# liangfu/dspnet

Hardware: AMD Instinct MI355X
Metric: training images/sec at 512x512 multitask (higher is better)
Workload: dtype f32; 1 GPU; resnet-50 multitask (det+depth+seg) 512x512, 8 det classes, 19 seg classes, N=6132 anchors, forward+backward+SGD; batch_per_gpu=32, global_batch=32, parallelism=dp1, f16x2_fallback_calls=0

## Files before the change

dspnet_amd/csrc/conv.hip:

```cpp
#include "dspn_common.h"
#include "bn_final_job.h"
#include "dspn_store.h"
#include "dspn_pieces.h"
#include "conv_geom.h"
#include <cstdlib>
#include "../../include/dspn_nn.h"

using dspn::st_t;
using dspn::kHalf;
using dspn::u32x4_t;

namespace {

using dspn::conv::f32x16;
using dspn::conv::bf16x8;
using dspn::pieces::bf16x4;
typedef __attribute__((address_space(3))) bf16x4 lds_bf16x4;

constexpr int kLdsRowH = kHalf ? 72 : 40;
__device__ __forceinline__ bf16x4 to_bf16x4(const float4 v) {
  bf16x4 r = {(__bf16)v.x, (__bf16)v.y, (__bf16)v.z, (__bf16)v.w};
  return r;
}

// ... 1563 lines not shown
    if (g.bn_sums) return DSPN_NT_(true, 3, false, 6);
    return g.stats ? DSPN_NT_(true, 3, false, 5) : DSPN_NT_(true, 3, false, 4);
  }
#endif
  if (g.bn_sums) return DSPN_NT_UB_(false, 2);
  if (g.in_scale) return g.stats ? DSPN_NT_UB_(true, 1) : DSPN_NT_UB_(true, 0);
  return g.stats ? DSPN_NT_UB_(false, 1) : DSPN_NT_UB_(false, 0);
#undef DSPN_NT_UB_
#undef DSPN_NT_
}

#ifdef DSPN_ABLATE
int g_debug_bits = 0;
#else
constexpr int g_debug_bits = 0;
#endif
static const int kNtBm[5] = {128, 128, 64, 256, 128}, kNtBn[5] = {128, 64, 64, 32, 256};
int nt_config(long long M, int Cout) {
  auto tiles = [&](int bm, int bn) { return ((M + bm - 1) / bm) * ((Cout + bn - 1) / bn); };
  int cfg;
  static const long long min_tiles = [] { const char *e = getenv("DSPN_NT_MINTILES"); return e ? atoll(e) : 256ll; }();
  if (Cout <= 32) cfg = tiles(256, 32) >= min_tiles ? 3 : 2;
  else cfg = (Cout > 64 && tiles(128, 128) >= min_tiles) ? 0 : 2;
  if (cfg == 0 && (Cout + 63) / 64 * 64 < (Cout + 127) / 128 * 128) cfg = 1;
  static const int cfg64 = [] { const char *e = getenv("DSPN_NT_CFG64"); return e ? atoi(e) : -1; }();
  if (cfg64 >= 0 && Cout > 32 && Cout <= 64 && tiles(kNtBm[cfg64], kNtBn[cfg64]) >= min_tiles) cfg = cfg64;
  if ((g_debug_bits >> 8) & 7) cfg = ((g_debug_bits >> 8) & 7) - 1;
  return cfg;
}
int dispatch_nt_impl(const st_t *in, const st_t *w, const float *bias, st_t *out, const ConvGeom &g_in,
                     hipStream_t s, SplitWs ws, const st_t *residual, bool *wide_used);
int dispatch_nt(const st_t *in, const st_t *w, const float *bias, st_t *out, const ConvGeom &g_in,
                hipStream_t s, SplitWs ws, const st_t *residual = nullptr) {
  bool wide = false;
  const int rc = dispatch_nt_impl(in, w, bias, out, g_in, s, ws, residual, &wide);
#ifndef DSPN_HALF
  if (!rc && g_in.bn_dy_absmax && !g_in.bn_sums && !wide) {
    if (!(g_in.dense && g_in.obs == (long long)g_in.Hg * g_in.Wg * g_in.ldc && g_in.ldc % 4 == 0))
      return dspn::fail(DSPN_ERR_ARG_, "conv2d_forward: the output magnitude block needs a dense output with ldc %% 4 == 0");
    return dspn_absmax_f32(out, (long long)g_in.N * g_in.Hg * g_in.Wg, g_in.ldc, nullptr, nullptr, 0,
                           reinterpret_cast<float *>(g_in.bn_dy_absmax), s);
  }
#endif
  return rc;
}
int dispatch_nt_impl(const st_t *in, const st_t *w, const float *bias, st_t *out, const ConvGeom &g_in,
                     hipStream_t s, SplitWs ws, const st_t *residual, bool *wide_used) {
  ConvGeom g = g_in;
  g.dbg = g_debug_bits;
  constexpr uintptr_t amask = 4 * sizeof(st_t) - 1;
  if (g.ldc % 4 == 0 && g.obs % 4 == 0 && (reinterpret_cast<uintptr_t>(out) & amask) == 0 &&
      (!residual || (reinterpret_cast<uintptr_t>(residual) & amask) == 0))
    g.flags |= 16;
  {
    const long long ib = (long long)sizeof(st_t) * g.N * g.Hin * g.Win * g.Cin,
                    wb = (long long)sizeof(st_t) * g.Cout * g.WTAPS * g.Cin;
    if (ib >= (1ll << 31) || wb >= (1ll << 31))
      return dspn::fail(DSPN_ERR_ARG_, "conv: tensors of 2 GiB or more are not supported by the buffer-addressed kernel");
    g.in_bytes = (unsigned)ib; g.w_bytes = (unsigned)wb;
  }
  const long long M = (long long)g.N * g.Hg * g.Wg;
  if (M <= 0) return 0;
  const bool pre = !kHalf && g.bf16 >= 2 && ((g.Cin / kEPC) & 7) == 0;
  if (pre) {
    if (!g.w_planes)
      return dspn::fail(DSPN_ERR_ARG_, "conv: the split math modes with a multiple of 32 input channels (%d) need the weight operand as piece planes (dspn_conv2d_weight_planes_f32)", g.Cin);
    w = static_cast<const st_t *>(g.w_planes);
    g.w_bytes = (unsigned)((g.bf16 == 3 ? 4ll : 6ll) * g.Cout * g.WTAPS * g.Cin);
  }
  auto tiles = [&](int bm, int bn) { return ((M + bm - 1) / bm) * ((g.Cout + bn - 1) / bn); };
  const int cfg = nt_config(M, g.Cout);
  const int *bm_ = kNtBm, *bn_ = kNtBn;
  const long long nblk = tiles(bm_[cfg], bn_[cfg]);
  const int nk = (g.TR * g.TS * (g.Cin / kEPC) + 7) >> 3;
  int splits = 1, per = nk;
  if (g.a_planes && !(pre && g.bf16 == 3 && !g.in_scale))
    return dspn::fail(DSPN_ERR_ARG_, "conv: a piece-plane operand needs DSPN_MATH_F32_F16X2, a multiple of 32 channels (%d) and no input affine", g.Cin);
  if (g.stats && (!g.dense || !(g.flags & 16) || g.Cout % 4 != 0))
    return dspn::fail(DSPN_ERR_ARG_, "conv2d_forward: output statistics need a dense, 16-byte aligned output with Cout %% 4 == 0");
  if (g.bn_sums && (g.in_scale || g.stats))
    return dspn::fail(DSPN_ERR_ARG_, "conv: BatchNorm-backward sums cannot be combined with an input affine or output statistics");
  if (g.bn_sums && (!(g.flags & 16) || g.Cout % 4 != 0))
    return dspn::fail(DSPN_ERR_ARG_, "conv2d_dgrad: BatchNorm sums need a 16-byte aligned dx with Cin %% 4 == 0");
  if (g.dense && nblk < 192 && nk >= 16 && ws.ptr && !g.stats && !g.bn_sums) {
    splits = (int)std::min<long long>((384 + nblk - 1) / nblk, nk / 8);
    splits = std::max(1, std::min(splits, 32));
    while (splits > 1 && sizeof(float) * (size_t)splits * M * g.Cout > ws.bytes) --splits;
    per = (nk + splits - 1) / splits;
    splits = (nk + per - 1) / per;
  }
  static const char *eight_env = getenv("DSPN_NT_8WAVE");
  const int eight_mode = eight_env ? atoi(eight_env) : -1;
  const bool one_tap = g.TR * g.TS == 1;
  const bool eight = eight_mode == 0 ? false : eight_mode == 1 ? true : (kHalf || g.bf16 >= 2) ? true
                     : ((!g.stats && !g.bn_sums) || (eight_mode == 2 && one_tap && g.bn_sums) || (eight_mode == 3 && one_tap));
  {
    bool wide_ok = splits == 1 && (cfg == 0 || (cfg == 2 && g.Cout > 32 && g.Cout <= 64)) && (g.flags & 16) && g.Cout % 4 == 0 &&
                   g.TR * g.TS > 0;
    if (kHalf) wide_ok = wide_ok && !g.in_scale && g.Cin % 64 == 0 && dspn::wide_tiles_mode() >= 2;
    else wide_ok = wide_ok && pre && g.bf16 == 3;
    if (wide_ok) {
      int shape = dspn::conv::wide_tile_choice(M, g.Cout, nk, (g.stats || g.bn_sums) ? 1 : 0);
      if (shape && !kHalf && !g.a_planes) shape = 10 + (shape == 1 ? 3 : shape);
      if (shape) { *wide_used = true; return dspn::conv::launch_wide(shape, in, w, bias, out, g, s, residual); }
    }
  }
  if (cfg == 0 && eight) return launch_nt<4, 2, 1, 2>(in, w, bias, out, g, s, splits, per, ws.ptr, residual);
  switch (cfg) {
    case 0: return launch_nt<2, 2, 2, 2>(in, w, bias, out, g, s, splits, per, ws.ptr, residual);
    case 1: return launch_nt<2, 2, 2, 1>(in, w, bias, out, g, s, splits, per, ws.ptr, residual);
    case 2: return launch_nt<2, 2, 1, 1>(in, w, bias, out, g, s, splits, per, ws.ptr, residual);
    default: return launch_nt<4, 1, 2, 1>(in, w, bias, out, g, s, splits, per, ws.ptr, residual);
  }
}

struct WgradPlan { int bm; int bn; int splits; int pps; };
constexpr int kPlanPK = 64;
static_assert(kPlanPK % kPK == 0, "split sizes must be whole k-steps");
WgradPlan wgrad_plan(long long P, int Cout, int J, long long x_bytes = 0, long long max_splits = 1 << 30) {
  WgradPlan p;
  p.bm = Cout <= 32 ? 32 : (Cout <= 64 ? 64 : 128);
  if (p.bm == 128 && (Cout + 63) / 64 * 64 < (Cout + 127) / 128 * 128) p.bm = 64;
  p.bn = (J <= 64 && p.bm == 128) ? 64 : 128;
  if (const char *e = getenv("DSPN_WG_TILE")) {
    const int t = atoi(e);
    p.bm = t == 0 ? 32 : (t == 1 ? 64 : 128);
    p.bn = t == 2 ? 64 : 128;
  }
  const long long tiles = (long long)((Cout + p.bm - 1) / p.bm) * ((J + p.bn - 1) / p.bn);
  const long long lds = 4ll * std::max(2 * kPK * (p.bm + p.bn), p.bm * (p.bn + 4));
  const long long slots = 256 * std::min<long long>(8, (160ll << 10) / lds);
  long long s_min = 1;
  if (x_bytes > 0) s_min = (x_bytes + (32ll << 20) - 1) / (32ll << 20);
  const long long s_max = std::max<long long>(1, std::min<long long>(std::min<long long>(P / 128, 1024), max_splits));
  s_min = std::min(s_min, s_max);
  const double flop_per_pix = 2.0 * p.bm * p.bn, slot_rate = 120e12 / (double)slots, ovh_pix = 160;
  double best = 1e30;
  long long splits = s_min;
  for (long long sp = s_min; sp <= s_max; ++sp) {
    const long long pps = ((P + sp - 1) / sp + kPlanPK - 1) / kPlanPK * kPlanPK;
    const long long real = (P + pps - 1) / pps;
    const long long rounds = (tiles * real + slots - 1) / slots;
    const double t = (double)rounds * ((double)pps + ovh_pix) * flop_per_pix / slot_rate +
                     (double)real * Cout * J * 8.0 / 4e12;
    if (t < best * 0.999) { best = t; splits = sp; }
    if (tiles * sp > 8 * slots) break;
  }
  if (const char *e = getenv("DSPN_WG_SPLITS")) splits = std::max<long long>(1, std::min<long long>(atoll(e), s_max));
  splits = std::min(splits, s_max);
  long long pps = ((P + splits - 1) / splits + kPlanPK - 1) / kPlanPK * kPlanPK;
  p.splits = (int)((P + pps - 1) / pps);
  p.pps = (int)pps;
  return p;
}

}

extern "C" {

#ifdef DSPN_ABLATE
#ifdef DSPN_HALF
int dspn_debug_set_bf16(int bits) { g_debug_bits = bits; return 0; }
#else
int dspn_debug_set(int bits) { g_debug_bits = bits; return 0; }
int dspn_debug_read_stamps(unsigned *host, int words, int clear) {
  if (hipMemcpyFromSymbol(host, HIP_SYMBOL(g_phase_stamps), sizeof(unsigned) * (size_t)std::min(words, 8192 * 8)) != hipSuccess) return 1;
  if (clear) { static unsigned z[8192 * 8]; (void)hipMemcpyToSymbol(HIP_SYMBOL(g_phase_stamps), z, sizeof(z)); }
  return 0;
}
#endif
#endif

#ifndef DSPN_HALF
size_t dspn_conv2d_split_workspace_bytes(long long out_pixels, int Cout) {
  if (out_pixels <= 0 || Cout <= 0) return 0;
  const long long capped = std::min<long long>(out_pixels * Cout, 192ll * 64 * 64 * 4);
  return sizeof(float) * 32 * (size_t)capped;
}
#endif

struct InAffine { const float *scale, *shift; int relu; };
struct OpScales { const float *a, *b; int a_planes = 0; };

static int conv2d_forward_one(int math, OpScales scales, const st_t *x, InAffine tf, float *stats, float *minmax, const st_t *w, const void *w_planes, const float *bias, const st_t *residual, st_t *y, int N,
                            int H, int W, int Cin, int Cout, int R, int S, int stride, int pad_h, int pad_w,
                            int dil, int Ho, int Wo, long long y_batch_stride, int y_ldc,
                            int relu, int accumulate, void *workspace, size_t workspace_bytes,
                            void *stream) {
  DSPN_REQUIRE(x && (w || w_planes) && y, "conv2d_forward: null pointer");
// ... 108 lines not shown
  hipLaunchKernelGGL(weight_transpose_kernel, dim3(blocks), dim3(256), 0, (hipStream_t)stream, w,
                     wt, static_cast<float *>(nullptr), Cout, taps, Cin, Cout_pad);
  return dspn::check_launch("weight_transpose");
}

int dspn_conv2d_weight_transpose_batch_f32(const void *table, int n, long long total_tiles, void *stream) {
  DSPN_REQUIRE(table && n > 0 && total_tiles > 0 && total_tiles < (1ll << 31), "weight_transpose_batch: bad argument");
  static_assert(sizeof(WtDesc) == 48, "table row layout: 2 pointers, 4 ints, 1 int64, 1 pointer (NULL here)");
  hipLaunchKernelGGL(weight_transpose_batch_kernel, dim3((unsigned)total_tiles), dim3(256), 0, (hipStream_t)stream,
                     static_cast<const WtDesc *>(table), n);
  return dspn::check_launch("weight_transpose_batch");
}
long long dspn_conv2d_weight_transpose_tiles(int Cout, int taps, int Cin, int Cout_pad) {
  if (Cout <= 0 || taps <= 0 || Cin <= 0 || Cout_pad < Cout) return 0;
  return (long long)((Cout_pad + 31) >> 5) * taps * ((Cin + 31) >> 5);
}

int dspn_conv2d_weight_planes_f32(const float *w, void *planes, void *planes_t, int Cout, int taps, int Cin, int cols_t,
                                  int pieces, const float *w_absmax, void *stream) {
  DSPN_REQUIRE(w && (planes || planes_t) && Cout > 0 && taps > 0 && Cin > 0 && Cin % 4 == 0, "weight_planes: bad argument");
  DSPN_REQUIRE(pieces == 3 || (pieces == 2 && w_absmax), "weight_planes: pieces is 3 (bf16) or 2 (fp16, with the weight's magnitude block)");
  DSPN_REQUIRE(!planes || Cin % 32 == 0, "weight_planes: the forward planes need Cin %% 32 == 0, got %d", Cin);
  DSPN_REQUIRE(!planes_t || (cols_t % 32 == 0 && cols_t >= Cout), "weight_planes: cols_t is the padded Cout, a multiple of 32");
  WpDesc e{w, static_cast<__bf16 *>(planes), static_cast<__bf16 *>(planes_t), Cout, taps, Cin, planes_t ? cols_t : 0, 0, w_absmax, pieces, 0};
  const long long tiles = weight_planes_tiles(Cout, taps, Cin, cols_t, planes_t != nullptr);
  DSPN_REQUIRE(tiles < (1ll << 31), "weight_planes: too many tiles");
  hipLaunchKernelGGL(weight_planes_kernel, dim3((unsigned)tiles), dim3(256), 0, (hipStream_t)stream, e);
  return dspn::check_launch("weight_planes");
}

long long dspn_conv2d_weight_planes_tiles(int Cout, int taps, int Cin, int cols_t, int with_transposed) {
  if (Cout <= 0 || taps <= 0 || Cin <= 0) return 0;
  return weight_planes_tiles(Cout, taps, Cin, cols_t, with_transposed != 0);
}

int dspn_absmax_f32(const float *x, long long rows, int C, const float *scale, const float *shift, int relu,
                    float *out_dev, void *stream) {
  DSPN_REQUIRE(x && out_dev && rows > 0 && C > 0 && C % 4 == 0, "absmax: bad argument (C must be a multiple of 4)");
  DSPN_REQUIRE((scale == nullptr) == (shift == nullptr), "absmax: scale and shift go together");
  const long long n4 = rows * (C / 4);
  const int blocks = (int)std::min<long long>((n4 + 255) / 256, 2048);
  hipLaunchKernelGGL(absmax_kernel, dim3(blocks), dim3(256), 0, (hipStream_t)stream, reinterpret_cast<const float4 *>(x), n4,
                     C / 4, reinterpret_cast<const float4 *>(scale), reinterpret_cast<const float4 *>(shift), relu,
                     reinterpret_cast<unsigned *>(out_dev));
  return dspn::check_launch("absmax");
}

int dspn_absmax_batch_f32(const void *table, int n, long long total_chunks, void *stream) {
  DSPN_REQUIRE(table && n > 0 && total_chunks > 0 && total_chunks < (1ll << 31), "absmax_batch: bad argument");
  static_assert(sizeof(AmDesc) == 32, "table row layout: 2 pointers, 2 int64");
  hipLaunchKernelGGL(absmax_batch_kernel, dim3((unsigned)total_chunks), dim3(256), 0, (hipStream_t)stream,
                     static_cast<const AmDesc *>(table), n);
  return dspn::check_launch("absmax_batch");
}

int dspn_conv2d_weight_planes_batch_f32(const void *table, int n, long long total_tiles, void *stream) {
  DSPN_REQUIRE(table && n > 0 && total_tiles > 0 && total_tiles < (1ll << 31), "weight_planes_batch: bad argument");
  static_assert(sizeof(WpDesc) == 64, "table row layout: 3 pointers, 4 ints, 1 int64, 1 pointer, 2 ints");
  hipLaunchKernelGGL(weight_planes_batch_kernel, dim3((unsigned)total_tiles), dim3(256), 0, (hipStream_t)stream,
                     static_cast<const WpDesc *>(table), n);
  return dspn::check_launch("weight_planes_batch");
}
#else
int dspn_conv2d_weight_prepare_bf16(const float *w, st_t *wh, st_t *wt, int Cout, int taps, int Cin,
                                    int Cout_pad, void *stream) {
  DSPN_REQUIRE(w && wt && Cout > 0 && taps > 0 && Cin > 0 && Cout_pad >= Cout && Cout_pad % kEPC == 0,
               "weight_prepare: bad argument");
  const long long total = (long long)Cin * taps * Cout_pad;
  const int blocks = (int)std::min<long long>((total + 255) / 256, 4096);
  hipLaunchKernelGGL(weight_transpose_kernel, dim3(blocks), dim3(256), 0, (hipStream_t)stream, w,
                     wt, wh, Cout, taps, Cin, Cout_pad);
  return dspn::check_launch("weight_prepare");
}

int dspn_conv2d_weight_prepare_batch_bf16(const void *table, int n, long long total_tiles, void *stream) {
  DSPN_REQUIRE(table && n > 0 && total_tiles > 0 && total_tiles < (1ll << 31), "weight_prepare_batch: bad argument");
  static_assert(sizeof(WtDesc) == 48, "table row layout: 2 pointers, 4 ints, 1 int64, 1 pointer");
  hipLaunchKernelGGL(weight_transpose_batch_kernel, dim3((unsigned)total_tiles), dim3(256), 0, (hipStream_t)stream,
                     static_cast<const WtDesc *>(table), n);
  return dspn::check_launch("weight_prepare_batch");
}
#endif

struct BnBwd { const st_t *x; const float *scale, *shift, *mean, *rstd; int relu; float *sums; float *dy_absmax; };

static int dgrad_tiles(int N, int H, int W, int Cin, int stride, int *per_class ) {
  int total = 0;
  for (int ph = 0; ph < (stride == 1 ? 1 : 2); ++ph)
    for (int pw = 0; pw < (stride == 1 ? 1 : 2); ++pw) {
      const long long hg = stride == 1 ? H : (H - ph + 1) / 2, wg = stride == 1 ? W : (W - pw + 1) / 2;
      const long long M = (long long)N * hg * wg;
      const int t = M > 0 ? (int)((M + kNtBm[nt_config(M, Cin)] - 1) / kNtBm[nt_config(M, Cin)]) : 0;
      if (per_class) per_class[ph * 2 + pw] = t;
      total += t;
    }
  return total;
}

static int conv2d_dgrad_one(int math, OpScales scales, const st_t *dy, const st_t *wt, const void *wt_planes, st_t *dx, int N, int H, int W,
                          int Cin, int ldy, int R, int S, int stride, int pad_h, int pad_w, int dil, int Ho,
                          int Wo, int dx_ldc, int accumulate, BnBwd bn, void *workspace, size_t workspace_bytes,
                          void *stream) {
  DSPN_REQUIRE(dy && (wt || wt_planes) && dx, "conv2d_dgrad: null pointer");
  DSPN_REQUIRE(ldy % kEPC == 0, "conv2d_dgrad: dy channel stride must be a multiple of %d", kEPC);
  DSPN_REQUIRE(stride == 1 || (stride == 2 && dil == 1), "conv2d_dgrad: stride 1, or stride 2 with dilation 1");
  DSPN_REQUIRE(N > 0 && H > 0 && W > 0 && Cin > 0 && R > 0 && S > 0, "conv2d_dgrad: bad geometry");
  ConvGeom g;
  memset(&g, 0, sizeof(g));
  g.N = N; g.Hin = Ho; g.Win = Wo; g.Cin = ldy; g.Cout = Cin;
  g.WTAPS = R * S; g.WS = S;
  g.ldc = dx_ldc > 0 ? dx_ldc : Cin;
  g.obs = (long long)H * W * g.ldc;
  g.OW = W;
  g.flags = accumulate ? 4 : 0;
  g.bf16 = kHalf ? 1 : math;
  g.w_planes = wt_planes;
  g.a_absmax = scales.a; g.b_absmax = scales.b;
  g.bn_x = bn.x; g.bn_scale = bn.scale; g.bn_shift = bn.shift; g.bn_mean = bn.mean; g.bn_rstd = bn.rstd;
  g.bn_relu = bn.relu; g.bn_sums = bn.sums; g.bn_tile_base = 0;
  g.bn_dy_absmax = (bn.sums && !kHalf && math == DSPN_MATH_F32_F16X2) ? reinterpret_cast<unsigned *>(bn.dy_absmax) : nullptr;
  g.a_planes = scales.a_planes;
  int class_tiles[4] = {0, 0, 0, 0};
  if (bn.sums) dgrad_tiles(N, H, W, Cin, stride, class_tiles);
  hipStream_t s = (hipStream_t)stream;
  const SplitWs sws{static_cast<float *>(workspace), workspace ? workspace_bytes : 0};
  if (stride == 1) {
    g.Hg = H; g.Wg = W; g.ish = 1; g.isw = 1; g.ioh = pad_h; g.iow = pad_w; g.idh = -dil; g.idw = -dil;
    g.TR = R; g.TS = S; g.wr0 = 0; g.wrs = 1; g.ws0 = 0; g.wss = 1;
    g.osh = 1; g.osw = 1; g.dense = 1;
    return dispatch_nt(dy, wt, nullptr, dx, g, s, sws);
  }
  for (int ph = 0; ph < 2; ++ph)
    for (int pw = 0; pw < 2; ++pw) {
      ConvGeom c = g;
      c.Hg = (H - ph + 1) / 2; c.Wg = (W - pw + 1) / 2;
      for (int q = 0; q < ph * 2 + pw; ++q) c.bn_tile_base += class_tiles[q];
      if (c.Hg <= 0 || c.Wg <= 0) continue;
      const int r0 = (ph + pad_h) & 1, s0 = (pw + pad_w) & 1;
      c.TR = r0 < R ? (R - r0 + 1) / 2 : 0;
      c.TS = s0 < S ? (S - s0 + 1) / 2 : 0;
      if (c.TR == 0 || c.TS == 0) {
        c.TR = 0; c.TS = 1;
        if (accumulate && !bn.sums) continue;
      }
      c.ish = 1; c.isw = 1; c.ioh = (ph + pad_h - r0) / 2; c.iow = (pw + pad_w - s0) / 2;
      c.idh = -1; c.idw = -1;
      c.wr0 = r0; c.wrs = 2; c.ws0 = s0; c.wss = 2;
      c.osh = 2; c.osw = 2; c.ooh = ph; c.oow = pw; c.dense = 0;
      const int rc = dispatch_nt(dy, wt, nullptr, dx, c, s, sws);
      if (rc) return rc;
    }
  return 0;
}

static int dgrad_bn_tiles(int N, int H, int W, int Cin, int stride) {
  if (N <= 0 || H <= 0 || W <= 0 || Cin <= 0 || Cin % 4 != 0 || (stride != 1 && stride != 2)) return 0;
  return dgrad_tiles(N, H, W, Cin, stride, nullptr);
}
#ifndef DSPN_HALF
int dspn_conv2d_dgrad_bn_tiles(int N, int H, int W, int Cin, int stride) { return dgrad_bn_tiles(N, H, W, Cin, stride); }
#endif

int DSPN_FN(dspn_conv2d_dgrad_bn)(const st_t *dy, const st_t *wt, const void *wt_planes, st_t *dx, int N, int H, int W,
                             int Cin, int ldy, int R, int S, int stride, int pad_h, int pad_w, int dil, int Ho,
                             int Wo, int dx_ldc, int accumulate,
                             const st_t *bn_x, const float *bn_scale, const float *bn_shift, const float *bn_mean,
                             const float *bn_rstd, int bn_relu, float *bn_sums, size_t bn_sums_bytes, float *bn_dy_absmax,
                             int math, const float *dy_absmax, const float *w_absmax, void *workspace, size_t workspace_bytes,
                             void *stream) {
  DSPN_REQUIRE(N > 0 && Ho > 0 && Wo > 0 && ldy > 0, "conv2d_dgrad: bad geometry");
  const int math_vouch = math & DSPN_MATH_UNSCALED_OK, dy_planes = (math & DSPN_MATH_DY_PLANES) ? 1 : 0;
  math &= ~(DSPN_MATH_UNSCALED_OK | DSPN_MATH_DY_PLANES);
  DSPN_REQUIRE(!dy_planes || (!dspn::kHalf && math == DSPN_MATH_F32_F16X2 && ldy % 32 == 0 && dy_absmax),
               "conv2d_dgrad: DSPN_MATH_DY_PLANES needs DSPN_MATH_F32_F16X2, ldy %% 32 == 0 and the block the planes were cut by (dy_absmax)");
  DSPN_REQUIRE(math >= DSPN_MATH_FP32 && math <= DSPN_MATH_F32_F16X2, "conv2d_dgrad: math is one of DSPN_MATH_*");
  DSPN_REQUIRE(dspn::kHalf || math != DSPN_MATH_F32_F16X2 || math_vouch || (dy_absmax && w_absmax),
               "conv2d_dgrad: DSPN_MATH_F32_F16X2 needs the magnitude block of both operands (dspn_absmax_f32); a caller who knows that every |operand| < 65504 passes math | DSPN_MATH_UNSCALED_OK");
  const int ldc = dx_ldc > 0 ? dx_ldc : Cin;
  const int nb = batch_chunk(N, (long long)sizeof(st_t) * Ho * Wo * ldy);
  if (bn_sums) {
    DSPN_REQUIRE(bn_x && bn_mean && bn_rstd && (!bn_relu || (bn_scale && bn_shift)), "conv2d_dgrad: BatchNorm operands missing");
    DSPN_REQUIRE(ldc == Cin && nb == N, "conv2d_dgrad: BatchNorm sums need a dense dx and dy below 2 GiB");
    const int tiles = dgrad_bn_tiles(N, H, W, Cin, stride);
    DSPN_REQUIRE(tiles > 0 && bn_sums_bytes >= sizeof(float) * 2 * (size_t)tiles * Cin,
                 "conv2d_dgrad: bn_sums needs dspn_conv2d_dgrad_bn_tiles() x 2 x Cin floats");
  }
  for (int n0 = 0; n0 < N; n0 += nb) {
    const int n = std::min(nb, N - n0);
    const int rc = conv2d_dgrad_one(math, OpScales{dy_absmax, w_absmax, dy_planes}, dy + (long long)n0 * Ho * Wo * ldy, wt, wt_planes, dx + (long long)n0 * H * W * ldc, n, H,
                                    W, Cin, ldy, R, S, stride, pad_h, pad_w, dil, Ho, Wo, dx_ldc, accumulate,
                                    BnBwd{bn_x, bn_scale, bn_shift, bn_mean, bn_rstd, bn_relu, bn_sums, bn_dy_absmax}, workspace,
                                    workspace_bytes, stream);
    if (rc) return rc;
  }
  return 0;
}

#ifndef DSPN_HALF
int dspn_conv2d_dgrad_f32(const float *dy, const float *wt, float *dx, int N, int H, int W,
                          int Cin, int ldy, int R, int S, int stride, int pad_h, int pad_w, int dil, int Ho,
                          int Wo, int dx_ldc, int accumulate, void *workspace, size_t workspace_bytes,
                          void *stream) {
  return dspn_conv2d_dgrad_bn_f32(dy, wt, nullptr, dx, N, H, W, Cin, ldy, R, S, stride, pad_h, pad_w, dil, Ho, Wo, dx_ldc,
                                  accumulate, nullptr, nullptr, nullptr, nullptr, nullptr, 0, nullptr, 0, nullptr, DSPN_MATH_FP32,
                                  nullptr, nullptr, workspace, workspace_bytes, stream);
}

size_t dspn_conv2d_input_sum_grad_workspace_bytes(int Ho, int Wo, int ldy, int R, int S) {
  return sizeof(float) * ((size_t)Ho * Wo * ldy + (size_t)R * S * 32 * ldy);
}
#endif

int DSPN_FN(dspn_conv2d_input_sum_grad)(const st_t *dy, const float *w, float *out, int N, int H, int W,
                                   int Cin, int Cout, int ldy, int R, int S, int stride, int pad_h, int pad_w, int dil,
                                   int Ho, int Wo, void *workspace, size_t workspace_bytes, void *stream) {
  DSPN_REQUIRE(dy && w && out && workspace, "conv2d_input_sum_grad: null pointer");
  DSPN_REQUIRE(ldy % 4 == 0 && Cin >= 1 && Cin <= 8, "conv2d_input_sum_grad: Cin <= 8, ldy % 4 == 0");
  if (workspace_bytes < sizeof(float) * ((size_t)Ho * Wo * ldy + (size_t)R * S * 32 * ldy))
    return dspn::fail(DSPN_ERR_WORKSPACE_, "conv2d_input_sum_grad: workspace too small");
  hipStream_t s = (hipStream_t)stream;
  float *p2 = static_cast<float *>(workspace);
  float *partial = p2 + (size_t)Ho * Wo * ldy;
  const long long per4 = (long long)Ho * Wo * ldy / 4;
  hipLaunchKernelGGL(batch_sum_kernel, dim3((int)std::min<long long>((per4 + 255) / 256, 8192)), dim3(256), 0, s,
                     dspn::CA4Ptr(dy), reinterpret_cast<float4 *>(p2), N, per4);
  SumGradGeom g{H, W, Ho, Wo, ldy, R, S, stride, stride, pad_h, pad_w, dil, dil, 32};
  hipLaunchKernelGGL(tap_sum_kernel, dim3(R * S, 32), dim3(256), 0, s, p2, partial, g);
  hipLaunchKernelGGL(sum_grad_final_kernel, dim3(1), dim3(1024), 0, s, partial, w, out, R * S, 32, ldy, Cout, Cin);
  return dspn::check_launch("conv2d_input_sum_grad");
}

#ifndef DSPN_HALF
size_t dspn_conv2d_wgrad_workspace_bytes(int N, int Ho, int Wo, int Cin, int Cout, int R, int S) {
  const long long P = (long long)N * Ho * Wo;
  const int J = R * S * Cin;
  if (P <= 0 || J <= 0 || Cout <= 0) return 0;
  size_t m = (size_t)wgrad_plan(P, Cout, J).splits;
  for (int stride = 1; stride <= 2; ++stride)
    m = std::max(m, (size_t)wgrad_plan(P, Cout, J, 4ll * P * Cin * stride * stride).splits);
  return sizeof(float) * m * Cout * J;
}
#endif

static int conv2d_wgrad_one(int math, OpScales scales, const st_t *x, InAffine tf, const st_t *dy, float *dw, int N, int H, int W, int Cin,
                          int Cout, int ldy, int R, int S, int stride, int pad_h, int pad_w, int dil, int Ho,
                          int Wo, int accumulate, void *workspace, size_t workspace_bytes,
                          void *stream) {
  DSPN_REQUIRE(x && dy && workspace, "conv2d_wgrad: null pointer");
  DSPN_REQUIRE(Cin % kEPC == 0 && ldy % kEPC == 0, "conv2d_wgrad: channel strides must be multiples of %d", kEPC);
  WgradGeom g;
  g.N = N; g.Hin = H; g.Win = W; g.Cin = Cin; g.Ho = Ho; g.Wo = Wo; g.Cout = Cout; g.ldy = ldy;
  g.sh = stride; g.sw = stride; g.ph = pad_h; g.pw = pad_w; g.dh = dil; g.dw = dil; g.R = R; g.S = S;
  g.in_scale = tf.scale; g.in_shift = tf.shift; g.in_relu = tf.relu;
  g.bf16 = kHalf ? 1 : math;
  g.dy_absmax = scales.a; g.x_absmax = scales.b;
  g.dy_planes = scales.a_planes & 1; g.x_planes = (scales.a_planes >> 1) & 1;
  {
    const long long xb = (long long)sizeof(st_t) * N * H * W * Cin, yb = (long long)sizeof(st_t) * N * Ho * Wo * ldy;
    if (xb >= (1ll << 31) || yb >= (1ll << 31))
      return dspn::fail(DSPN_ERR_ARG_, "conv2d_wgrad: tensors of 2 GiB or more are not supported");
    g.x_bytes = (unsigned)xb; g.dy_bytes = (unsigned)yb;
  }
  const long long P = (long long)N * Ho * Wo;
  const int J = R * S * Cin;
  const long long ws_splits = (long long)(workspace_bytes / (sizeof(float) * (size_t)Cout * J));
  if (ws_splits < 1)
    return dspn::fail(DSPN_ERR_WORKSPACE_, "conv2d_wgrad: workspace %zu < %zu (one slab)", workspace_bytes, sizeof(float) * (size_t)Cout * J);
  const WgradPlan plan = wgrad_plan(P, Cout, J, R * S > 1 ? 4ll * P * Cin * std::min(stride, 2) * std::min(stride, 2) : 0, ws_splits);
  const int BM = plan.bm, BN = plan.bn;
  const int kt = (Cout + BM - 1) / BM, jt = (J + BN - 1) / BN;
  const long long splits = plan.splits;
  g.pix_per_split = plan.pps;
  const size_t need = sizeof(float) * (size_t)splits * Cout * J;
  if (workspace_bytes < need)
    return dspn::fail(DSPN_ERR_WORKSPACE_, "conv2d_wgrad: workspace %zu < %zu", workspace_bytes, need);
  hipStream_t s = (hipStream_t)stream;
  float *slab = static_cast<float *>(workspace);
  g.job = dspn::BnFinalJob{};
  g.job_rows = dspn::bn_job_take(s, &g.job) ? (g.job.blocks + kt * jt - 1) / (kt * jt) : 0;
// ... 149 lines not shown
```

dspnet_amd/csrc/conv_geom.h:

```cpp
#pragma once
#include <hip/hip_runtime.h>

namespace dspn {
namespace conv {

typedef float f32x16 __attribute__((ext_vector_type(16)));
typedef __bf16 bf16x8 __attribute__((ext_vector_type(8)));

template <typename st_t>
struct ConvGeomT {
  int N, Hin, Win, Cin;
  int Hg, Wg;
  int ish, isw, ioh, iow, idh, idw;
  int TR, TS;
  int WTAPS, WS, wr0, wrs, ws0, wss;
  int Cout;
  long long obs;
  int OW, osh, osw, ooh, oow, ldc;
  int flags;
  int dense;
  int dbg;
  int bf16;
  unsigned in_bytes, w_bytes;
  const float *in_scale, *in_shift;
  float *stats;
  float *minmax;
  const st_t *bn_x;
  const float *bn_scale, *bn_shift, *bn_mean, *bn_rstd;
  float *bn_sums;
  int bn_relu, bn_tile_base;
  unsigned *bn_dy_absmax;
  const float *a_absmax, *b_absmax;
  int a_planes;
  const void *w_planes;
};

__device__ __forceinline__ int xcd_remap(int bid, int nblk) {
  const int q = nblk >> 3, r = nblk & 7, x = bid & 7;
  const int start = x < r ? x * (q + 1) : r * (q + 1) + (x - r) * q;
  return start + (bid >> 3);
}


int wide_tile_choice(long long M, int Cout, int nk, int fused_epilogue);
int launch_wide(int shape, const float *in, const float *w_planes, const float *bias, float *out, const ConvGeomT<float> &g,
                hipStream_t s, const float *residual);
int launch_wide(int shape, const __bf16 *in, const __bf16 *w, const float *bias, __bf16 *out, const ConvGeomT<__bf16> &g,
                hipStream_t s, const __bf16 *residual);

int launch_stem(const float *x, const float *w, float *y, int N, int H, int W, int Cin, int Cout, int Ho, int Wo,
                const float *x_absmax, const float *w_absmax, float *stats, float *minmax, hipStream_t s);

}
}
```

dspnet_amd/csrc/conv_wide.h:

```cpp

#ifdef DSPN_STAMPS
__device__ unsigned long long g_wide_stamps[1024 * 16];
struct WideStamps {
  unsigned long long last, sum[16];
  __device__ __forceinline__ void begin() { for (int i = 0; i < 16; ++i) sum[i] = 0; last = __builtin_readcyclecounter(); }
  __device__ __forceinline__ void mark(int i) { const unsigned long long t = __builtin_readcyclecounter(); sum[i] += t - last; last = t; }
  __device__ __forceinline__ void flush() {
    if (threadIdx.x == 0 && blockIdx.x < 1024) for (int i = 0; i < 16; ++i) g_wide_stamps[blockIdx.x * 16 + i] = sum[i];
  }
};
#define DSPN_STAMP_DECL WideStamps stamps_; stamps_.begin()
#define DSPN_STAMP(i) stamps_.mark(i)
#define DSPN_STAMP_FLUSH stamps_.flush()
#define DSPN_STAMP_ARG , stamps_
#define DSPN_STAMP_PARAM , WideStamps &stamps_
#else
#define DSPN_STAMP_DECL
#define DSPN_STAMP(i)
#define DSPN_STAMP_FLUSH
#define DSPN_STAMP_ARG
#define DSPN_STAMP_PARAM
#endif

inline bool xt_enabled() { return dspn::tile_spanning() != 0; }
// ... 150 lines not shown
            red2[((h * RPP + er0) * BN + c4 * 4 + e) * 2 + 1] = vmx[h][e];
          }
        }
      }
    }
    asm volatile("s_waitcnt lgkmcnt(0)" ::: "memory");
    __builtin_amdgcn_s_barrier();
    for (int hc = tid; hc < HALVES * BN; hc += NTHR) {
      const int h = hc / BN, col = hc - h * BN;
      const int lim = min(M - (m0 + h * SR), SR);
      if (n0 + col >= g.Cout || lim <= 0) continue;
      const float *rh = red + (size_t)h * RPP * BN * 2, *rh2 = red2 + (size_t)h * RPP * BN * 2;
      const float mref = rh[col * 2];
      float n = 0.f, sd = 0.f, sq = 0.f;
#pragma unroll 4
      for (int er = 0; er < RPP; ++er) {
        const int ne_i = lim > er ? (lim - er + RPP - 1) / RPP : 0;
        const float ne = (float)ne_i;
        const float d = ne_i > 0 ? rh[(er * BN + col) * 2] - mref : 0.f;
        const float m2e = ne_i > 0 ? rh[(er * BN + col) * 2 + 1] : 0.f;
        n += ne; sd += ne * d; sq += m2e + ne * d * d;
      }
      const float dm = sd / n;
      const long long mt_ = m0 / SR + h;
      g.stats[(mt_ * 2 + 0) * g.Cout + n0 + col] = mref + dm;
      g.stats[(mt_ * 2 + 1) * g.Cout + n0 + col] = fmaxf(sq - n * dm * dm, 0.f);
      if (mmx) {
        float mn = kInf, mx = -kInf;
        for (int er = 0; er < RPP && er < lim; ++er) { mn = fminf(mn, rh2[(er * BN + col) * 2]); mx = fmaxf(mx, rh2[(er * BN + col) * 2 + 1]); }
        g.minmax[(mt_ * 2 + 0) * g.Cout + n0 + col] = mn;
        g.minmax[(mt_ * 2 + 1) * g.Cout + n0 + col] = mx;
      }
    }
  }
  if constexpr (EPI == 2) {
    __builtin_amdgcn_s_barrier();
    float *red = reinterpret_cast<float *>(wsm);
    if (cvalid) {
#pragma unroll
      for (int h = 0; h < HALVES; ++h)
#pragma unroll
        for (int e = 0; e < 4; ++e) {
          red[((h * RPP + er0) * BN + c4 * 4 + e) * 2] = gs[h][e];
          red[((h * RPP + er0) * BN + c4 * 4 + e) * 2 + 1] = gss[h][e];
        }
    }
    asm volatile("s_waitcnt lgkmcnt(0)" ::: "memory");
    __builtin_amdgcn_s_barrier();
    for (int hc = tid; hc < HALVES * BN; hc += NTHR) {
      const int h = hc / BN, col = hc - h * BN;
      if (n0 + col >= g.Cout || m0 + h * SR >= M) continue;
      const float *rh = red + (size_t)h * RPP * BN * 2;
      float a = 0.f, b = 0.f;
      for (int er = 0; er < RPP; ++er) { a += rh[(er * BN + col) * 2]; b += rh[(er * BN + col) * 2 + 1]; }
      const long long mt_ = g.bn_tile_base + m0 / SR + h;
      g.bn_sums[(mt_ * 2 + 0) * g.Cout + n0 + col] = a;
      g.bn_sums[(mt_ * 2 + 1) * g.Cout + n0 + col] = b;
    }
    gmx_all = fmaxf(gmx_all, gmx);
  }
  if constexpr (EPI == 0) gmx_all = fmaxf(gmx_all, gmx);
  asm volatile("s_waitcnt lgkmcnt(0)" ::: "memory");
  __builtin_amdgcn_s_barrier();
  DSPN_STAMP(6);
}

#ifndef DSPN_HALF
template <int WAVES_M, int WAVES_N, int EPI, int RB = 16, int SR = 128, bool CLOSE = false>
__device__ __forceinline__ void direct_epilogue(const ConvGeom &g, char *exch, f32x16 (&acc)[2][2], const float inv_a, const float inv_b, const int m0,
                                                const int n0, const int M, const int tid, const int wave,
                                                const float *__restrict__ bias, float *__restrict__ out,
                                                const float *__restrict__ residual, float &gmx_all) {
  constexpr int TM = 2, TN = 2, BN = WAVES_N * 64, NTHR = WAVES_M * WAVES_N * 64, PARTS = WAVES_M * 2;
  constexpr int WRT = SR / 64, TILES = WAVES_M / WRT, PPT = WRT * 2;
  static_assert(SR == 64 || SR == 128, "statistics tiles of 64 or 128 rows");
  static_assert(WAVES_M % WRT == 0, "whole statistics tiles per output tile");
  const int lane = tid & 63, half = lane >> 5, lc = lane & 31;
  const int wr = wave / WAVES_N, wm = wr * 64, wn = (wave % WAVES_N) * 64;
  const bool has_bias = g.flags & 1, relu = g.flags & 2, accum = g.flags & 4, has_res = g.flags & 8;
  const float *addsrc = has_res ? residual : (accum ? out : nullptr);
  const unsigned obytes = (unsigned)M * (unsigned)g.ldc * 4u;
  const __amdgpu_buffer_rsrc_t rs_o = __builtin_amdgcn_make_buffer_rsrc(out, 0, obytes, 0x00020000);
  const __amdgpu_buffer_rsrc_t rs_a = __builtin_amdgcn_make_buffer_rsrc(const_cast<float *>(addsrc ? addsrc : out), 0, addsrc ? obytes : 0u, 0x00020000);
  const __amdgpu_buffer_rsrc_t rs_x = __builtin_amdgcn_make_buffer_rsrc(const_cast<float *>(EPI == 2 ? g.bn_x : out), 0, EPI == 2 ? obytes : 0u, 0x00020000);
  constexpr unsigned kOOB = 0x80000000u;
  constexpr float kInf = __builtin_huge_valf();
  int col[TN];
  unsigned cbyte[TN];
  bool cv[TN];
  float bv[TN], bsc[TN], bsh[TN], bmu[TN], brs[TN];
#pragma unroll
  for (int j = 0; j < TN; ++j) {
    col[j] = n0 + wn + j * 32 + lc;
    cv[j] = col[j] < g.Cout;
    cbyte[j] = cv[j] ? (unsigned)col[j] * 4u : kOOB;
    bv[j] = (has_bias && cv[j]) ? bias[col[j]] : 0.f;
    bsc[j] = bsh[j] = bmu[j] = brs[j] = 0.f;
    if (EPI == 2 && cv[j]) {
      bmu[j] = g.bn_mean[col[j]]; brs[j] = g.bn_rstd[col[j]];
      if (g.bn_relu) { bsc[j] = g.bn_scale[col[j]]; bsh[j] = g.bn_shift[col[j]]; }
    }
  }
  const int row0 = m0 + wm + 4 * half;
  const unsigned pitch = (unsigned)g.ldc * 4u;
  float sK[TN], s1[TN], s2[TN], vmn[TN], vmx[TN], gs[TN], gss[TN];
  int scnt = 0;
  float gmx = 0.f;
#pragma unroll
  for (int j = 0; j < TN; ++j) { sK[j] = 0.f; s1[j] = 0.f; s2[j] = 0.f; vmn[j] = kInf; vmx[j] = -kInf; gs[j] = 0.f; gss[j] = 0.f; }
  const bool both = has_res && accum;
  constexpr int NB = TM * 16 / RB;
  const bool need_rows = addsrc != nullptr || EPI == 2;
  if constexpr (EPI == 2) {
    float rq[2][RB][TN], xq[2][RB][TN], oq[2][RB][TN];
    auto request = [&](const int bb, const int s_) __attribute__((always_inline)) {
      const int i = bb / (16 / RB), r0 = (bb % (16 / RB)) * RB;
#pragma unroll
      for (int rr = 0; rr < RB; ++rr) {
        const int r = r0 + rr;
        const unsigned rb = (unsigned)(row0 + 32 * i + (r & 3) + 8 * (r >> 2)) * pitch;
#pragma unroll
        for (int j = 0; j < TN; ++j) {
          const unsigned off = rb + cbyte[j];
          rq[s_][rr][j] = addsrc ? __builtin_bit_cast(float, __builtin_amdgcn_raw_buffer_load_b32(rs_a, (int)off, 0, 0)) : 0.f;
          xq[s_][rr][j] = __builtin_bit_cast(float, __builtin_amdgcn_raw_buffer_load_b32(rs_x, (int)off, 0, 0));
          oq[s_][rr][j] = both ? __builtin_bit_cast(float, __builtin_amdgcn_raw_buffer_load_b32(rs_o, (int)off, 0, 0)) : 0.f;
        }
      }
    };
    request(0, 0);
#pragma unroll
    for (int bb = 0; bb < NB; ++bb) {
      const int i = bb / (16 / RB), r0 = (bb % (16 / RB)) * RB, s_ = bb & 1;
      if (bb + 1 < NB) request(bb + 1, s_ ^ 1);
#pragma unroll
      for (int rr = 0; rr < RB; ++rr) {
        const int r = r0 + rr;
        const unsigned rb = (unsigned)(row0 + 32 * i + (r & 3) + 8 * (r >> 2)) * pitch;
#pragma unroll
        for (int j = 0; j < TN; ++j) {
          float v = acc[i][j][r] * inv_a * inv_b + bv[j];
          v += rq[s_][rr][j];
          if (both) v += oq[s_][rr][j];
          if (relu) v = v > 0.f ? v : 0.f;
          __builtin_amdgcn_raw_buffer_store_b32(__builtin_bit_cast(unsigned, v), rs_o, (int)(rb + cbyte[j]), 0, 0);
          const float xv = xq[s_][rr][j];
          const float gd = (!g.bn_relu || fmaf(xv, bsc[j], bsh[j]) > 0.f) ? v : 0.f;
          gs[j] += gd;
          gss[j] += gd * ((xv - bmu[j]) * brs[j]);
          gmx = fmaxf(gmx, fabsf(v));
        }
      }
    }
#pragma unroll
    for (int j = 0; j < TN; ++j) { gs[j] = cv[j] ? gs[j] : 0.f; gss[j] = cv[j] ? gss[j] : 0.f; }
  } else {
    typedef float f32x2 __attribute__((ext_vector_type(2)));
    f32x2 s1p[TN], s2p[TN];
#pragma unroll
    for (int j = 0; j < TN; ++j) { s1p[j] = f32x2{0.f, 0.f}; s2p[j] = f32x2{0.f, 0.f}; }
    f32x2 rq[2][RB / 2][TN], oq[2][RB / 2][TN];
    auto request = [&](const int bb, const int s_) __attribute__((always_inline)) {
      const int i = bb / (16 / RB), r0 = (bb % (16 / RB)) * RB;
#pragma unroll
      for (int rr = 0; rr < RB; rr += 2) {
        const int r = r0 + rr;
        const unsigned rb = (unsigned)(row0 + 32 * i + (r & 3) + 8 * (r >> 2)) * pitch;
#pragma unroll
        for (int j = 0; j < TN; ++j) {
          const unsigned off = rb + cbyte[j];
          rq[s_][rr / 2][j] = f32x2{0.f, 0.f}; oq[s_][rr / 2][j] = f32x2{0.f, 0.f};
          if (addsrc) rq[s_][rr / 2][j] = f32x2{__builtin_bit_cast(float, __builtin_amdgcn_raw_buffer_load_b32(rs_a, (int)off, 0, 0)),
                                               __builtin_bit_cast(float, __builtin_amdgcn_raw_buffer_load_b32(rs_a, (int)(off + pitch), 0, 0))};
          if (both) oq[s_][rr / 2][j] = f32x2{__builtin_bit_cast(float, __builtin_amdgcn_raw_buffer_load_b32(rs_o, (int)off, 0, 0)),
                                             __builtin_bit_cast(float, __builtin_amdgcn_raw_buffer_load_b32(rs_o, (int)(off + pitch), 0, 0))};
        }
      }
    };
    if (need_rows) request(0, 0);
#pragma unroll
    for (int bb = 0; bb < NB; ++bb) {
      const int i = bb / (16 / RB), r0 = (bb % (16 / RB)) * RB, s_ = bb & 1;
      if (need_rows && bb + 1 < NB) request(bb + 1, s_ ^ 1);
#pragma unroll
      for (int rr = 0; rr < RB; rr += 2) {
        const int r = r0 + rr;
        const unsigned rb = (unsigned)(row0 + 32 * i + (r & 3) + 8 * (r >> 2)) * pitch;
#pragma unroll
        for (int j = 0; j < TN; ++j) {
          f32x2 t = f32x2{acc[i][j][r], acc[i][j][r + 1]} * inv_a * inv_b + bv[j];
          if (need_rows) t += rq[s_][rr / 2][j];
          else t += f32x2{0.f, 0.f};
          float v0 = t[0], v1 = t[1];
          if (both) { v0 += oq[s_][rr / 2][j][0]; v1 += oq[s_][rr / 2][j][1]; }
          if (relu) { v0 = v0 > 0.f ? v0 : 0.f; v1 = v1 > 0.f ? v1 : 0.f; }
          __builtin_amdgcn_raw_buffer_store_b32(__builtin_bit_cast(unsigned, v0), rs_o, (int)(rb + cbyte[j]), 0, 0);
          __builtin_amdgcn_raw_buffer_store_b32(__builtin_bit_cast(unsigned, v1), rs_o, (int)(rb + pitch + cbyte[j]), 0, 0);
          const f32x2 v = f32x2{v0, v1};
          if constexpr (EPI == 0) {
            if (g.bn_dy_absmax) gmx = fmaxf(fmaxf(gmx, fabsf(v0)), fabsf(v1));
          }
          if constexpr (EPI == 1) {
            if (bb == 0 && rr == 0) sK[j] = v0;
            const f32x2 d = v - sK[j];
            s1p[j] += d; s2p[j] += d * d;
            vmn[j] = fminf(fminf(vmn[j], v0), v1); vmx[j] = fmaxf(fmaxf(vmx[j], v0), v1);
          }
        }
      }
    }
    scnt = 32;
#pragma unroll
    for (int j = 0; j < TN; ++j) { s1[j] = s1p[j].x + s1p[j].y; s2[j] = s2p[j].x + s2p[j].y; }
  }
  if constexpr (EPI == 0) gmx_all = fmaxf(gmx_all, gmx);
  if constexpr (EPI == 2) gmx_all = fmaxf(gmx_all, gmx);
  if constexpr (EPI != 0) {
    float *red = reinterpret_cast<float *>(exch);
    float *red2 = red + PARTS * BN * 4;
    const bool mmx = EPI == 1 && g.minmax != nullptr;
    const int p = wr * 2 + half;
#pragma unroll
    for (int j = 0; j < TN; ++j) {
      float *q = red + (p * BN + wn + j * 32 + lc) * 4;
      if constexpr (EPI == 1) {
        const float inv_n = scnt > 0 ? 1.f / (float)scnt : 0.f;
        q[0] = (float)scnt; q[1] = sK[j] + s1[j] * inv_n; q[2] = s2[j] - s1[j] * s1[j] * inv_n;
        if (mmx) { float *q2 = red2 + (p * BN + wn + j * 32 + lc) * 2; q2[0] = vmn[j]; q2[1] = vmx[j]; }
      } else {
        q[0] = gs[j]; q[1] = gss[j];
      }
    }
    asm volatile("s_waitcnt lgkmcnt(0)" ::: "memory");
    __builtin_amdgcn_s_barrier();
    for (int hc = tid; hc < TILES * BN; hc += NTHR) {
      const int h = hc / BN, c = hc - h * BN;
      if (n0 + c >= g.Cout || m0 + h * SR >= M) continue;
      const long long mt_ = m0 / SR + h;
      if constexpr (EPI == 1) {
        float n = 0.f, mean = 0.f, m2 = 0.f, mn = kInf, mx = -kInf;
#pragma unroll
        for (int pq = 0; pq < PPT; ++pq) {
          const int pp = h * PPT + pq;
          const float *q = red + (pp * BN + c) * 4;
          const float nb = q[0];
          if (nb > 0.f) {
            const float d = q[1] - mean, nn = n + nb;
            mean += d * (nb / nn);
            m2 += q[2] + d * d * (n * nb / nn);
            n = nn;
            if (mmx) { mn = fminf(mn, red2[(pp * BN + c) * 2]); mx = fmaxf(mx, red2[(pp * BN + c) * 2 + 1]); }
          }
        }
        g.stats[(mt_ * 2 + 0) * g.Cout + n0 + c] = mean;
        g.stats[(mt_ * 2 + 1) * g.Cout + n0 + c] = fmaxf(m2, 0.f);
        if (mmx) {
          g.minmax[(mt_ * 2 + 0) * g.Cout + n0 + c] = mn;
          g.minmax[(mt_ * 2 + 1) * g.Cout + n0 + c] = mx;
        }
      } else {
        float a = 0.f, b = 0.f;
#pragma unroll
        for (int pq = 0; pq < PPT; ++pq) { a += red[((h * PPT + pq) * BN + c) * 4]; b += red[((h * PPT + pq) * BN + c) * 4 + 1]; }
        const long long t_ = g.bn_tile_base + mt_;
        g.bn_sums[(t_ * 2 + 0) * g.Cout + n0 + c] = a;
        g.bn_sums[(t_ * 2 + 1) * g.Cout + n0 + c] = b;
      }
    }
    if constexpr (CLOSE) {
      asm volatile("s_waitcnt lgkmcnt(0)" ::: "memory");
      __builtin_amdgcn_s_barrier();
    }
  }
}
#endif

template <int NWV>
__device__ __forceinline__ void wide_publish_absmax(const ConvGeom &g, char *wsm, float gmx_all, const int tid) {
  const int lane = tid & 63, wave = tid >> 6;
    if (g.bn_dy_absmax) {
#pragma unroll
      for (int o = 32; o >= 1; o >>= 1) gmx_all = fmaxf(gmx_all, __shfl_xor(gmx_all, o, 64));
      float *sm = reinterpret_cast<float *>(wsm);
      if (lane == 0) sm[wave] = gmx_all;
      asm volatile("s_waitcnt lgkmcnt(0)" ::: "memory");
      __builtin_amdgcn_s_barrier();
      if (tid == 0) {
        float m = sm[0];
        for (int q = 1; q < NWV; ++q) m = fmaxf(m, sm[q]);
        if (m > 0.f) atomicMax(g.bn_dy_absmax + (blockIdx.x & 63u), __float_as_uint(m));
      }
    }
}

template <int WAVES_M, int WAVES_N, int STAGES, int EPI, int SR = 128, bool XT = false>
__global__ __launch_bounds__(WAVES_M * WAVES_N * 64, 2) void conv_ntw_kernel(
    const st_t *__restrict__ in, const st_t *__restrict__ wgt, const float *__restrict__ bias,
    st_t *__restrict__ out, const ConvGeom g, const int m_tiles, const int n_tiles,
    const st_t *__restrict__ residual) {
  constexpr int TM = 2, TN = 2;
// ... 121 lines not shown
    bf16x8 fa[4][TM], fb[4][TN];
    constexpr int ORD[4] = {kHalf ? 0 : 2, 0, kHalf ? 1 : 3, kHalf ? 2 : 1};
    constexpr int ORDH[4] = {0, 1, 2, 3};
    if (dbg & 4) {
#pragma unroll
      for (int f = 0; f < 4; ++f) {
#pragma unroll
        for (int i = 0; i < TM; ++i) { fa[f][i] = bf16x8{}; asm volatile("" : "+v"(fa[f][i])); }
#pragma unroll
        for (int j = 0; j < TN; ++j) { fb[f][j] = bf16x8{}; asm volatile("" : "+v"(fb[f][j])); }
      }
    } else {
#pragma unroll
      for (int q = 0; q < 4; ++q) {
        const int f = kHalf ? ORDH[q] : ORD[q];
        const int fbq = kHalf ? f : (f ^ 2);
#pragma unroll
        for (int i = 0; i < TM; ++i) fa[f][i] = *reinterpret_cast<const bf16x8 *>(sa + i * 4096 + (foff ^ ((2 * f) << 4)));
#pragma unroll
        for (int j = 0; j < TN; ++j) fb[fbq][j] = *reinterpret_cast<const bf16x8 *>(sb + j * 4096 + (foff ^ ((2 * fbq) << 4)));
      }
    }
    __builtin_amdgcn_sched_barrier(0);
    constexpr int NMMA = NKK * NPROD * TM * TN;
    static_assert(NI <= NMMA, "at most one request per MFMA");
    constexpr int PA[3] = {1, 0, 0}, PB[3] = {0, 1, 0};
#pragma unroll
    for (int m = 0; m < NMMA; ++m) {
      const int kk = m / (NPROD * TM * TN), t3 = (m / (TM * TN)) % NPROD, i = (m / TN) % TM, j = m % TN;
      const int ia = kHalf ? kk : 2 * PA[t3] + kk, ib = kHalf ? kk : 2 * PB[t3] + kk;
      if (dbg & 2) { asm volatile("" :: "v"(fa[ia][i]), "v"(fb[ib][j])); }
      else if constexpr (kHalf)
        acc[i][j] = __builtin_amdgcn_mfma_f32_32x32x16_bf16(fa[ia][i], fb[ib][j], acc[i][j], 0, 0, 0);
      else
        acc[i][j] = __builtin_amdgcn_mfma_f32_32x32x16_f16(__builtin_bit_cast(f16x8, fa[ia][i]),
                                                           __builtin_bit_cast(f16x8, fb[ib][j]), acc[i][j], 0, 0, 0);
#pragma unroll
      for (int q = 0; q < NI; ++q)
        if (((q + 1) * NMMA) / NI - 1 == m) {
          issue_piece(q);
          __builtin_amdgcn_sched_barrier(0);
        }
    }
  };

  float gmx_all = 0.f;

  if constexpr (XT) {
    constexpr bool EXCH_IN_RING = NWV == 8 || BM == 256;
    int t = blockIdx.x;
    if (t < ntiles) {
      setup_tile(t);
#pragma unroll
      for (int j = 0; j < D; ++j) issue(j, true);
    }
    int slot = 0, islot = D % STAGES;
    bool more = false;
    DSPN_STAMP_DECL;
    for (; t < ntiles; t += gridDim.x) {
      const int m0 = ld_m0, n0 = ld_n0;
      const int tn = t + (int)gridDim.x;
      const bool first = t == (int)blockIdx.x;
      zero_acc();
      int last_slot = 0;
      for (int kt = 0; kt < nk; ++kt) {
        if (!first && kt < D) asm volatile("s_waitcnt vmcnt(63)" ::: "memory");
        else asm volatile("s_waitcnt vmcnt(%0)" ::"n"((D - 1) * NI) : "memory");
        __builtin_amdgcn_s_barrier();
        if (kt + D < nk) {
          issue_begin(islot, true);
        } else {
          if (kt + D == nk) { more = tn < ntiles; if (more) setup_tile(tn); }
          issue_begin(islot, more);
        }
        mma_step(slot);
        last_slot = slot;
        slot = slot + 1 == STAGES ? 0 : slot + 1;
        islot = islot + 1 == STAGES ? 0 : islot + 1;
      }
      DSPN_STAMP(2);
      char *exch = wsm + STAGES * STG;
      if constexpr (EXCH_IN_RING) {
        exch = wsm + last_slot * STG;
        if constexpr (EPI != 0) { asm volatile("s_waitcnt lgkmcnt(0)" ::: "memory"); __builtin_amdgcn_s_barrier(); }
      }
      if constexpr (!kHalf) direct_epilogue<WAVES_M, WAVES_N, EPI, (EPI == 2 ? 4 : 8), SR>(g, exch, acc, inv_a, inv_b, m0, n0, M, tid, wave, bias, out, residual, gmx_all);
      DSPN_STAMP(5);
    }
    DSPN_STAMP_FLUSH;
    asm volatile("s_waitcnt vmcnt(0)" ::: "memory");
    if constexpr (EPI != 1) {
      asm volatile("s_waitcnt lgkmcnt(0)" ::: "memory");
      __builtin_amdgcn_s_barrier();
      wide_publish_absmax<NWV>(g, wsm, gmx_all, tid);
    }
    return;
  }

  DSPN_STAMP_DECL;
  for (int t = blockIdx.x; t < ntiles; t += gridDim.x) {
    setup_tile(t);
    const int m0 = ld_m0, n0 = ld_n0;
#pragma unroll
    for (int j = 0; j < D; ++j) issue(j, j < nk);
    zero_acc();
    DSPN_STAMP(1);
    int slot = 0, islot = D % STAGES;
    for (int kt = 0; kt < nk; ++kt) {
      asm volatile("s_waitcnt vmcnt(%0)" ::"n"((D - 1) * NI) : "memory");
      if (!(dbg & 8)) __builtin_amdgcn_s_barrier();
      issue_begin(islot, kt + D < nk);
      mma_step(slot);
      slot = slot + 1 == STAGES ? 0 : slot + 1;
      islot = islot + 1 == STAGES ? 0 : islot + 1;
    }
    asm volatile("s_waitcnt vmcnt(0)" ::: "memory");
    asm volatile("s_waitcnt lgkmcnt(0)" ::: "memory");
    __builtin_amdgcn_s_barrier();
    DSPN_STAMP(2);
    if (dbg & 16) { if (acc[0][0][0] == 1.2345e33f) out[0] = (st_t)acc[TM - 1][TN - 1][5]; continue; }

    {
      constexpr int SLD = BN + 4;
      float *st = reinterpret_cast<float *>(wsm);
  #pragma unroll
      for (int i = 0; i < TM; ++i)
  #pragma unroll
        for (int j = 0; j < TN; ++j)
  #pragma unroll
          for (int r = 0; r < 16; ++r)
            st[(wm + i * 32 + (r & 3) + 8 * (r >> 2) + 4 * (lane >> 5)) * SLD + wn + j * 32 + (lane & 31)] = acc[i][j][r] * inv_a * inv_b;
    }
    DSPN_STAMP(3);
    wide_epilogue<BM, BN, NTHR, EPI, SR>(g, wsm, m0, n0, M, tid, bias, out, residual, gmx_all, NoStage() DSPN_STAMP_ARG);
  }
  DSPN_STAMP_FLUSH;
  if constexpr (EPI != 1) wide_publish_absmax<NWV>(g, wsm, gmx_all, tid);
}

#ifndef DSPN_HALF
typedef float ntv_f32x4_t __attribute__((ext_vector_type(4)));
template <int NEWER>
__device__ __forceinline__ void ntv_wait2(ntv_f32x4_t &a, ntv_f32x4_t &b) {
  asm volatile("s_waitcnt vmcnt(%2)" : "+v"(a), "+v"(b) : "n"(NEWER));
}
template <int NEWER>
__device__ __forceinline__ void ntv_wait4(ntv_f32x4_t &a, ntv_f32x4_t &b, ntv_f32x4_t &c, ntv_f32x4_t &d) {
  asm volatile("s_waitcnt vmcnt(%4)" : "+v"(a), "+v"(b), "+v"(c), "+v"(d) : "n"(NEWER));
}
template <int WAVES_M, int WAVES_N, bool INTF, int EPI, int SR = 128, int XT = 0>
__global__ __launch_bounds__(WAVES_M * WAVES_N * 64, 2) void conv_ntv_kernel(
    const float *__restrict__ in, const float *__restrict__ wgt, const float *__restrict__ bias,
    float *__restrict__ out, const ConvGeom g, const int m_tiles, const int n_tiles,
    const float *__restrict__ residual) {
  constexpr int TM = 2, TN = 2;
  constexpr int BM = WAVES_M * TM * 32, BN = WAVES_N * TN * 32;
  constexpr int NWV = WAVES_M * WAVES_N, NTHR = NWV * 64;
  constexpr int A_U = BM * 4 / NTHR;
  constexpr int B_NI = BN / (8 * NWV);
  static_assert((BM * 4) % NTHR == 0 && BN % (8 * NWV) == 0, "whole units / pieces per thread / wave");
  constexpr int STG = (BM + BN) * 128;
#ifdef DSPN_NTV_SHALLOW
  constexpr bool DEEP = false;
#else
  constexpr bool DEEP = A_U <= 2;
#endif
  constexpr int NSET = DEEP ? 2 : 1;
  constexpr int NA = A_U * 2 + (INTF ? 4 : 0);
  extern __shared__ __attribute__((aligned(1024))) char wsm[];
  const int tid = threadIdx.x, lane = tid & 63;
  const int wave = __builtin_amdgcn_readfirstlane(tid >> 6);
  const int ntiles = m_tiles * n_tiles;
  const int M = g.N * g.Hg * g.Wg;
  const int CB = g.Cin >> 5;
  const int nk = g.TR * g.TS * CB;
  const float sc_a = operand_scale(g.a_absmax), sc_b = operand_scale(g.b_absmax);
  const float inv_a = 1.f / sc_a, inv_b = 1.f / sc_b;
  const __amdgpu_buffer_rsrc_t rsrc_b = __builtin_amdgcn_make_buffer_rsrc(const_cast<float *>(wgt), 0, g.w_bytes, 0x00020000);
  constexpr unsigned kOOB = 0x80000000u;
  const bool in_relu = g.flags & 32;
  auto rsrc_words = [](const float *p, unsigned bytes) {
    const unsigned long long a = reinterpret_cast<unsigned long long>(p);
    return u32x4_t{(unsigned)__builtin_amdgcn_readfirstlane((int)(unsigned)a),
                   (unsigned)__builtin_amdgcn_readfirstlane((int)((unsigned)(a >> 32) & 0xffffu)),
                   (unsigned)__builtin_amdgcn_readfirstlane((int)bytes), 0x00020000u};
  };
  const u32x4_t rw_a = rsrc_words(in, g.in_bytes);
  const u32x4_t rw_sc = rsrc_words(g.in_scale, INTF ? (unsigned)g.Cin * 4u : 0u), rw_sh = rsrc_words(g.in_shift, INTF ? (unsigned)g.Cin * 4u : 0u);
  typedef ntv_f32x4_t f32x4_t;
  auto load16 = [](const u32x4_t rw, const unsigned voff) __attribute__((always_inline)) {
    f32x4_t r;
    asm volatile("buffer_load_dwordx4 %0, %1, %2, 0 offen" : "=v"(r) : "v"(voff), "s"(rw));
    return r;
  };

  const int aq = tid & 3;
  int a_lds[A_U];
#pragma unroll
  for (int j = 0; j < A_U; ++j) {
    const int r = (tid + j * NTHR) >> 2, line = r >> 1;
    a_lds[j] = line * 256 + (((((r & 1) << 3) | aq) ^ (line & 7)) << 4);
  }
  int b_row[B_NI], b_cb[B_NI];
#pragma unroll
  for (int i = 0; i < B_NI; ++i) {
    const int line = 4 * (wave * B_NI + i) + (lane >> 4), sl = (lane & 15) ^ (line & 7);
    b_row[i] = 2 * line + (sl >> 3); b_cb[i] = (sl & 7) * 16;
  }
  int a_ih0[A_U], a_iw0[A_U], a_boff[A_U], b_boff[B_NI];
  int l_tr = 0, l_ts = 0, l_cb = 0;
  int lb_tr = 0, lb_ts = 0, lb_cb = 0;
  f32x4_t ra[NSET][A_U][2];
  f32x4_t tsc[NSET][2], tsh[NSET][2];
  unsigned a_mask[NSET] = {};
  u32x4_t pa[A_U][2];

  const int wm = (wave / WAVES_N) * (TM * 32), wn = (wave % WAVES_N) * (TN * 32);
// ... 274 lines not shown
  auto kern = conv_ntv_kernel<WAVES_M, WAVES_N, INTF, EPI, SR, XT>;
  static dspn::KernelDeviceState st;
  const bool first = !st.slots[0] && !st.slots[1];
  const int dev = dspn::ensure_persistent_grid(reinterpret_cast<const void *>(kern), WAVES_M * WAVES_N * 64, lds, st, "conv_ntv");
  if (dev < 0) return dev;
  const int slots = st.slots[dev], slots_per_cu = st.slots_per_cu[dev], slots_cus = st.cus[dev];
  if (first && getenv("DSPN_DEBUG_PRINT"))
    fprintf(stderr, "[dspn] conv_ntv<%d,%d,intf=%d,epi=%d,xt=%d>: %zu B LDS, occupancy %d/CU x %d CUs -> grid %d\n", WAVES_M, WAVES_N,
            (int)INTF, EPI, (int)XT, lds, slots_per_cu, slots_cus, slots);
  const int reserved = dspn::reserved_cus();
  const int avail = reserved > 0 ? std::max(8, slots_per_cu * std::max(8, slots_cus - reserved) / 8 * 8) : slots;
  const int grid_x = (int)std::min<long long>((long long)mt * nt, avail);
  {
    dspn::ProfScope prof(0, s);
    hipLaunchKernelGGL(kern, dim3(grid_x), dim3(WAVES_M * WAVES_N * 64), lds, s, in, w, bias, out, g, mt, nt, residual);
  }
  return dspn::check_launch("conv_ntv");
}
template <int WAVES_M, int WAVES_N, int SR = 128>
int launch_ntv(const float *in, const float *w, const float *bias, float *out, const ConvGeom &g, hipStream_t s, const float *residual) {
#define DSPN_NTV_(T, X) \
  (g.bn_sums ? launch_ntv_impl<WAVES_M, WAVES_N, T, 2, SR, X>(in, w, bias, out, g, s, residual) \
   : g.stats ? launch_ntv_impl<WAVES_M, WAVES_N, T, 1, SR, X>(in, w, bias, out, g, s, residual) \
             : launch_ntv_impl<WAVES_M, WAVES_N, T, 0, SR, X>(in, w, bias, out, g, s, residual))
  if constexpr (WAVES_M == 2 && WAVES_N == 2 && SR == 128) {
    const int nk = g.TR * g.TS * (g.Cin / 32);
    const long long tiles = (((long long)g.N * g.Hg * g.Wg + 127) / 128) * ((g.Cout + 127) / 128);
    if (dspn::tile_spanning() >= 2 && nk >= 2 && nk <= 8 && nk % 2 == 0 && tiles >= 2048 && xt_output_ok(g))
      return g.in_scale ? DSPN_NTV_(true, 1) : DSPN_NTV_(false, 1);
    static const bool direct_only = [] { const char *e = getenv("DSPN_NTV_DIRECT"); return !e || atoi(e) != 0; }();
    if (direct_only && xt_enabled() && nk >= 2 && xt_output_ok(g))
      return g.in_scale ? DSPN_NTV_(true, 2) : DSPN_NTV_(false, 2);
  }
  if constexpr (WAVES_M == 2 && WAVES_N == 4 && SR == 128) {
    static const bool direct8 = [] { const char *e = getenv("DSPN_NTV_DIRECT8"); return !e || atoi(e) != 0; }();
    const int nk = g.TR * g.TS * (g.Cin / 32);
    if (direct8 && xt_enabled() && nk >= 2 && xt_output_ok(g))
      return g.in_scale ? DSPN_NTV_(true, 2) : DSPN_NTV_(false, 2);
  }
  if constexpr (WAVES_M == 4 && WAVES_N == 1 && SR == 64) {
    const int nk = g.TR * g.TS * (g.Cin / 32);
    if (xt_c64_enabled() && xt_enabled() && nk >= 2 && xt_output_ok(g, 256))
      return g.in_scale ? DSPN_NTV_(true, 2) : DSPN_NTV_(false, 2);
  }
  return g.in_scale ? DSPN_NTV_(true, 0) : DSPN_NTV_(false, 0);
#undef DSPN_NTV_
}
#endif

template <int WAVES_M, int WAVES_N, int STAGES, int EPI, int SR, bool XT = false>
int launch_ntw_impl(const st_t *in, const st_t *w, const float *bias, st_t *out, const ConvGeom &g, hipStream_t s,
                    const st_t *residual) {
  constexpr int BM = WAVES_M * 64, BN = WAVES_N * 64;
  const long long M = (long long)g.N * g.Hg * g.Wg;
  const int mt = (int)((M + BM - 1) / BM), nt = (g.Cout + BN - 1) / BN;
  const size_t lds = XT ? (size_t)STAGES * (BM + BN) * 128 + ((WAVES_M * WAVES_N == 8 || BM == 256) ? 0 : sizeof(float) * 4 * BN * 6)
                        : std::max<size_t>((size_t)STAGES * (BM + BN) * 128, sizeof(float) * BM * (BN + 4));
  auto kern = conv_ntw_kernel<WAVES_M, WAVES_N, STAGES, EPI, SR, XT>;
  static dspn::KernelDeviceState st;
  const bool first = !st.slots[0] && !st.slots[1];
  const int dev = dspn::ensure_persistent_grid(reinterpret_cast<const void *>(kern), WAVES_M * WAVES_N * 64, lds, st, "conv_ntw");
  if (dev < 0) return dev;
  const int slots = st.slots[dev], slots_per_cu = st.slots_per_cu[dev], slots_cus = st.cus[dev];
  if (first && getenv("DSPN_DEBUG_PRINT"))
    fprintf(stderr, "[dspn] conv_ntw<%d,%d,stages=%d,epi=%d,xt=%d>: %zu B LDS, occupancy %d/CU x %d CUs -> grid %d\n", WAVES_M, WAVES_N,
            STAGES, EPI, (int)XT, lds, slots_per_cu, slots_cus, slots);
  const int reserved = dspn::reserved_cus();
  const int avail = reserved > 0 ? std::max(8, slots_per_cu * std::max(8, slots_cus - reserved) / 8 * 8) : slots;
  const int grid_x = (int)std::min<long long>((long long)mt * nt, avail);
  {
    dspn::ProfScope prof(0, s);
    hipLaunchKernelGGL(kern, dim3(grid_x), dim3(WAVES_M * WAVES_N * 64), lds, s, in, w, bias, out, g, mt, nt, residual);
  }
  return dspn::check_launch("conv_ntw");
}

template <int WAVES_M, int WAVES_N, int STAGES, int SR = 128>
int launch_ntw(const st_t *in, const st_t *w, const float *bias, st_t *out, const ConvGeom &g, hipStream_t s, const st_t *residual) {
#ifndef DSPN_HALF
  if constexpr ((WAVES_M == 2 && SR == 128) || (WAVES_M == 4 && WAVES_N == 1 && SR == 64)) {
    const int nk = g.TR * g.TS * (g.Cin / 32);
    if (xt_enabled() && nk >= STAGES && xt_output_ok(g, WAVES_M * 64) &&
        (WAVES_M == 4 ? xt_c64_enabled() : (WAVES_N == 2 || xt_wide8_enabled()))) {
      if (g.bn_sums) return launch_ntw_impl<WAVES_M, WAVES_N, STAGES, 2, SR, true>(in, w, bias, out, g, s, residual);
      if (g.stats) return launch_ntw_impl<WAVES_M, WAVES_N, STAGES, 1, SR, true>(in, w, bias, out, g, s, residual);
      return launch_ntw_impl<WAVES_M, WAVES_N, STAGES, 0, SR, true>(in, w, bias, out, g, s, residual);
    }
  }
#endif
  if (g.bn_sums) return launch_ntw_impl<WAVES_M, WAVES_N, STAGES, 2, SR>(in, w, bias, out, g, s, residual);
  if (g.stats) return launch_ntw_impl<WAVES_M, WAVES_N, STAGES, 1, SR>(in, w, bias, out, g, s, residual);
  return launch_ntw_impl<WAVES_M, WAVES_N, STAGES, 0, SR>(in, w, bias, out, g, s, residual);
}
```

dspnet_amd/csrc/dspn_common.h:

```cpp
#pragma once
#include <hip/hip_runtime.h>
#include <cstdarg>
#include <cstdio>
#include <cstring>

#define DSPN_OK_ 0
#define DSPN_ERR_ARG_ (-1)
#define DSPN_ERR_WORKSPACE_ (-2)
#define DSPN_ERR_LAUNCH_ (-3)

namespace dspn {

char *last_error_buf();

inline int fail(int code, const char *fmt, ...) {
  va_list ap;
  va_start(ap, fmt);
  vsnprintf(last_error_buf(), 512, fmt, ap);
  va_end(ap);
  return code;
}

inline int check_launch(const char *what) {
  hipError_t e = hipGetLastError();
  if (e != hipSuccess) return fail(DSPN_ERR_LAUNCH_, "%s: %s", what, hipGetErrorString(e));
  return 0;
}

bool prof_enabled();
void prof_begin(int family, hipStream_t s);
void prof_end(hipStream_t s);
struct ProfScope {
  hipStream_t s; bool on;
  ProfScope(int family, hipStream_t st) : s(st), on(prof_enabled()) { if (on) prof_begin(family, st); }
  ~ProfScope() { if (on) prof_end(s); }
};

int reserved_cus();
int wide_tiles_mode();
int tile_spanning();
int sampler_batched();

constexpr int kMaxDevices = 32;
struct KernelDeviceState {
  bool ready[kMaxDevices] = {};
  int slots[kMaxDevices] = {}, slots_per_cu[kMaxDevices] = {}, cus[kMaxDevices] = {};
};
inline int ensure_dynamic_lds(const void *kern, size_t bytes, KernelDeviceState &st, const char *what) {
  int dev = 0;
  if (hipGetDevice(&dev) != hipSuccess || dev < 0 || dev >= kMaxDevices)
    return fail(DSPN_ERR_LAUNCH_, "%s: no current device (or an index past %d)", what, kMaxDevices - 1);
  if (st.ready[dev]) return dev;
  if (bytes > 0) {
    const hipError_t e = hipFuncSetAttribute(kern, hipFuncAttributeMaxDynamicSharedMemorySize, (int)bytes);
    if (e != hipSuccess)
      return fail(DSPN_ERR_LAUNCH_, "%s: %zu bytes of dynamic LDS rejected on device %d (%s)", what, bytes, dev, hipGetErrorString(e));
  }
  st.ready[dev] = true;
  return dev;
}
inline int ensure_persistent_grid(const void *kern, int threads, size_t lds, KernelDeviceState &st, const char *what) {
  int dev = 0;
  if (hipGetDevice(&dev) != hipSuccess || dev < 0 || dev >= kMaxDevices)
    return fail(DSPN_ERR_LAUNCH_, "%s: no current device (or an index past %d)", what, kMaxDevices - 1);
  if (st.slots[dev]) return dev;
  const int d2 = ensure_dynamic_lds(kern, lds, st, what);
  if (d2 < 0) return d2;
  int per_cu = 0, cus = 0;
  (void)hipOccupancyMaxActiveBlocksPerMultiprocessor(&per_cu, kern, threads, lds);
  (void)hipDeviceGetAttribute(&cus, hipDeviceAttributeMultiprocessorCount, dev);
  if (per_cu < 1)
    return fail(DSPN_ERR_LAUNCH_, "%s: the kernel does not fit a compute unit of device %d (%d threads, %zu bytes of LDS)", what, dev, threads, lds);
  st.slots_per_cu[dev] = per_cu; st.cus[dev] = cus > 0 ? cus : 1;
  st.slots[dev] = per_cu * st.cus[dev] / 8 * 8 > 8 ? per_cu * st.cus[dev] / 8 * 8 : 8;
  return dev;
}

inline size_t align_up(size_t v, size_t a) { return (v + a - 1) / a * a; }
inline int cdiv(long a, long b) { return (int)((a + b - 1) / b); }

}

#define DSPN_REQUIRE(cond, ...) \
  do { if (!(cond)) return dspn::fail(DSPN_ERR_ARG_, __VA_ARGS__); } while (0)
```

dspnet_amd/csrc/nn.hip:

```cpp
#include "dspn_common.h"
#include "bn_final_job.h"
#include "dspn_store.h"
#include "dspn_pieces.h"
#include "../../include/dspn_nn.h"

using dspn::st_t;
using dspn::A1Ptr;
using dspn::A4Ptr;
using dspn::CA1Ptr;
using dspn::CA4Ptr;

#pragma clang fp contract(fast)

namespace {

constexpr int kT = 256;
inline int slab_rows_for(long long rows) {
  const long long want = (rows + 1023) / 1024;
  return (int)std::min<long long>(512, std::max<long long>(32, (want + 7) / 8 * 8));
}

inline int grid_for(long long n, int per_block = kT, int cap = 8192) {
  long long b = (n + per_block - 1) / per_block;
  return (int)std::max<long long>(1, std::min<long long>(b, cap));
// ... 472 lines not shown
                 const Co &k0, const Co &k1) __attribute__((always_inline)) {
    dspn::pieces::bf16x4 p0, p1, q0, q1;
    dspn::pieces::split2h(grad(x0, g0, k0), s, p0, p1);
    dspn::pieces::split2h(grad(x1, g1, k1), s, q0, q1);
    if (__builtin_expect(nf, 0)) { dspn::pieces::repair_inf(p0, p1); dspn::pieces::repair_inf(q0, q1); }
    planes[i] = hi ? plane_pack(p1, q1) : plane_pack(p0, q0);
  };
  const long long cstride = (long long)gridDim.x * (U * 256);
  long long base = blockIdx.x * (long long)(U * 256) + threadIdx.x;
  if (fixed_c) {
    const int c = (int)(base % C4);
    const PlaneChunk pc = plane_chunk(c);
    const Co k0 = coefs(pc.ca), k1 = coefs(pc.ca + 1);
    const int d = pc.ca - c;
    for (; base + (U - 1) * 256 < n4; base += cstride) {
      float4 x0[U], g0[U], x1[U], g1[U];
#pragma unroll
      for (int u = 0; u < U; ++u) {
        const long long a = base + u * 256 + d;
        x0[u] = x[a]; g0[u] = dy[a]; x1[u] = x[a + 1]; g1[u] = dy[a + 1];
      }
#pragma unroll
      for (int u = 0; u < U; ++u) one(base + u * 256, pc.hi, x0[u], g0[u], x1[u], g1[u], k0, k1);
    }
    for (int u = 0; u < U; ++u) {
      const long long i = base + u * 256;
      if (i < n4) one(i, pc.hi, x[i + d], dy[i + d], x[i + d + 1], dy[i + d + 1], k0, k1);
    }
  } else {
    for (; base < n4; base += cstride) {
#pragma unroll
      for (int u = 0; u < U; ++u) {
        const long long i = base + u * 256;
        if (i >= n4) break;
        const int c = (int)(i % C4);
        const PlaneChunk pc = plane_chunk(c);
        const long long a = i - c + pc.ca;
        one(i, pc.hi, x[a], dy[a], x[a + 1], dy[a + 1], coefs(pc.ca), coefs(pc.ca + 1));
      }
    }
  }
}

__global__ __launch_bounds__(256) void bn_bwd_apply_pool_kernel(const float4 *__restrict__ x, const float4 *__restrict__ scale,
                                    const float4 *__restrict__ shift, const float4 *__restrict__ coef, float4 *__restrict__ dx,
                                    long long n4, int C4, int relu, unsigned *__restrict__ absmax, const PoolGrad pool) {
  float mx = 0.f;
  for (long long i = blockIdx.x * (long long)blockDim.x + threadIdx.x; i < n4; i += (long long)gridDim.x * blockDim.x) {
    const unsigned row = (unsigned)i / (unsigned)C4;
    const int c4 = (int)((unsigned)i - row * (unsigned)C4);
    const float4 xv = x[i];
    float4 g = pool_grad_at(pool, row, c4, C4);
    if (relu) {
      const float4 sa = scale[c4], sb = shift[c4];
      g.x = fmaf(xv.x, sa.x, sb.x) > 0.f ? g.x : 0.f; g.y = fmaf(xv.y, sa.y, sb.y) > 0.f ? g.y : 0.f;
      g.z = fmaf(xv.z, sa.z, sb.z) > 0.f ? g.z : 0.f; g.w = fmaf(xv.w, sa.w, sb.w) > 0.f ? g.w : 0.f;
    }
    const float4 a = coef[c4], c1 = coef[C4 + c4], c0 = coef[2 * C4 + c4];
    const float4 o = make_float4(a.x * g.x + c1.x * xv.x + c0.x, a.y * g.y + c1.y * xv.y + c0.y,
                                 a.z * g.z + c1.z * xv.z + c0.z, a.w * g.w + c1.w * xv.w + c0.w);
    dx[i] = o;
    mx = fmaxf(mx, fmaxf(fmaxf(fabsf(o.x), fabsf(o.y)), fmaxf(fabsf(o.z), fabsf(o.w))));
  }
  if (absmax) {
    __shared__ float sm[4];
#pragma unroll
    for (int o = 32; o >= 1; o >>= 1) mx = fmaxf(mx, __shfl_xor(mx, o, 64));
    if ((threadIdx.x & 63) == 0) sm[threadIdx.x >> 6] = mx;
    __syncthreads();
    if (threadIdx.x == 0) {
      for (int w = 1; w < 4; ++w) mx = fmaxf(mx, sm[w]);
      if (mx > 0.f) atomicMax(absmax + (blockIdx.x & 63), __float_as_uint(mx));
    }
  }
}

template <int U>
__global__ __launch_bounds__(256) void bn_bwd_apply_kernel(const CA4Ptr x, const float4 *__restrict__ scale,
                                    const float4 *__restrict__ shift, const CA4Ptr dy,
                                    const float4 *__restrict__ coef, const A4Ptr dx,
                                    long long n4, int C4, int relu, int accumulate, unsigned *__restrict__ absmax,
                                    int fixed_c) {
  float mx = 0.f;
  auto one = [&](const float4 xv, float4 g, const float4 d, const float4 sa, const float4 sb, const float4 a,
                 const float4 c1, const float4 c0) __attribute__((always_inline)) {
    if (relu) {
      g.x = fmaf(xv.x, sa.x, sb.x) > 0.f ? g.x : 0.f; g.y = fmaf(xv.y, sa.y, sb.y) > 0.f ? g.y : 0.f;
      g.z = fmaf(xv.z, sa.z, sb.z) > 0.f ? g.z : 0.f; g.w = fmaf(xv.w, sa.w, sb.w) > 0.f ? g.w : 0.f;
    }
    float4 o = make_float4(a.x * g.x + c1.x * xv.x + c0.x, a.y * g.y + c1.y * xv.y + c0.y,
                           a.z * g.z + c1.z * xv.z + c0.z, a.w * g.w + c1.w * xv.w + c0.w);
    if (accumulate) { o.x += d.x; o.y += d.y; o.z += d.z; o.w += d.w; }
    mx = fmaxf(mx, fmaxf(fmaxf(fabsf(o.x), fabsf(o.y)), fmaxf(fabsf(o.z), fabsf(o.w))));
    return o;
  };
  const float4 zero = make_float4(0.f, 0.f, 0.f, 0.f);
  const long long cstride = (long long)gridDim.x * (U * 256);
  long long base = blockIdx.x * (long long)(U * 256) + threadIdx.x;
  if (fixed_c) {
    const int c4 = (int)(base % C4);
    const float4 sa = relu ? scale[c4] : zero, sb = relu ? shift[c4] : zero;
    const float4 a = coef[c4], c1 = coef[C4 + c4], c0 = coef[2 * C4 + c4];
    for (; base + (U - 1) * 256 < n4; base += cstride) {
      float4 xv[U], g[U], d[U];
#pragma unroll
      for (int u = 0; u < U; ++u) { xv[u] = x[base + u * 256]; g[u] = dy[base + u * 256]; }
#pragma unroll
      for (int u = 0; u < U; ++u) d[u] = accumulate ? (float4)dx[base + u * 256] : zero;
#pragma unroll
      for (int u = 0; u < U; ++u) dx[base + u * 256] = one(xv[u], g[u], d[u], sa, sb, a, c1, c0);
    }
    for (int u = 0; u < U; ++u) {
      const long long j = base + u * 256;
      if (j < n4) dx[j] = one(x[j], dy[j], accumulate ? (float4)dx[j] : zero, sa, sb, a, c1, c0);
    }
  } else {
    for (; base < n4; base += cstride) {
#pragma unroll
      for (int u = 0; u < U; ++u) {
        const long long j = base + u * 256;
        if (j >= n4) break;
        const int c4 = (int)(j % C4);
        dx[j] = one(x[j], dy[j], accumulate ? (float4)dx[j] : zero, relu ? scale[c4] : zero, relu ? shift[c4] : zero, coef[c4],
                    coef[C4 + c4], coef[2 * C4 + c4]);
      }
    }
  }
  if (absmax) {
    __shared__ float sm[kT / 64];
#pragma unroll
    for (int o = 32; o >= 1; o >>= 1) mx = fmaxf(mx, __shfl_xor(mx, o, 64));
    if ((threadIdx.x & 63) == 0) sm[threadIdx.x >> 6] = mx;
    __syncthreads();
    if (threadIdx.x == 0) {
      for (int w = 1; w < kT / 64; ++w) mx = fmaxf(mx, sm[w]);
      unsigned *o = absmax + (blockIdx.x & 63);
      if (mx > 0.f && __float_as_uint(mx) > __builtin_nontemporal_load(o)) atomicMax(o, __float_as_uint(mx));
    }
  }
}

#ifdef DSPN_HALF
__global__ void bn_apply8_kernel(const dspn::u32x4_t *__restrict__ x, const float4 *__restrict__ scale,
                                 const float4 *__restrict__ shift, dspn::u32x4_t *__restrict__ y, long long n8, int C8,
                                 int relu) {
  for (long long i = blockIdx.x * (long long)blockDim.x + threadIdx.x; i < n8;
       i += (long long)gridDim.x * blockDim.x) {
    const int c8 = (int)(i % C8);
    const dspn::u32x4_t xw = x[i];
    dspn::u32x4_t ow;
#pragma unroll
    for (int h = 0; h < 2; ++h) {
      const dspn::u32x2_t xh = {xw[2 * h], xw[2 * h + 1]};
      const float4 v = dspn::widen4(xh), a = scale[c8 * 2 + h], b = shift[c8 * 2 + h];
      float4 o = make_float4(fmaf(v.x, a.x, b.x), fmaf(v.y, a.y, b.y), fmaf(v.z, a.z, b.z), fmaf(v.w, a.w, b.w));
      if (relu) {
        o.x = o.x > 0.f ? o.x : 0.f; o.y = o.y > 0.f ? o.y : 0.f;
        o.z = o.z > 0.f ? o.z : 0.f; o.w = o.w > 0.f ? o.w : 0.f;
      }
      const dspn::u32x2_t on = dspn::narrow4(o);
      ow[2 * h] = on[0]; ow[2 * h + 1] = on[1];
    }
    y[i] = ow;
  }
}
template <int U>
__global__ __launch_bounds__(256) void bn_bwd_apply8_kernel(const dspn::u32x4_t *__restrict__ x, const float4 *__restrict__ scale,
                                     const float4 *__restrict__ shift, const dspn::u32x4_t *__restrict__ dy,
                                     const float4 *__restrict__ coef, dspn::u32x4_t *__restrict__ dx,
                                     long long n8, int C8, int relu, int accumulate, int fixed_c) {
  const int C4 = C8 * 2;
  const float4 zero = make_float4(0.f, 0.f, 0.f, 0.f);
  auto one = [&](const dspn::u32x4_t xw, const dspn::u32x4_t gw, const dspn::u32x4_t dw, const float4 (&sa)[2],
                 const float4 (&sb)[2], const float4 (&a)[2], const float4 (&c1)[2], const float4 (&c0)[2])
// ... 1574 lines not shown
```

dspnet_amd/engine.py:

```python
import math

import numpy as np
import torch

from . import functional as fn


FUSE_BATCHNORM = True
COMMUTE_RESIZE_CONV = True
import os as _os
MATERIALISE_MULTITAP_INPUT_BF16 = _os.environ.get("DSPN_MAT3X3", "1") != "0"


_SHARED_STREAMS = {}


def shared_stream(device, kind, priority=0):
    key = (str(device), kind)
    ent = _SHARED_STREAMS.get(key)
    if ent is None:
        ent = _SHARED_STREAMS[key] = (torch.cuda.Stream(device=device, priority=priority), priority)
    assert ent[1] == priority, "shared stream %r of %s was created with priority %d, asked for %d" % (kind, device, ent[1], priority)
    return ent[0]

# ... 263 lines not shown
            if rs and all(ok for _, ok in rs):
                n.defer_apply = True
                continue
            n.defer_apply = False
            n.out.affine_src = None
            n.out.data = fn.zeros(*n.out.shape, device=self.device, dtype=n.out.dtype)
            for c in n.conv_consumers:
                c.x_raw, c.in_affine = c.x, None
            n.mat_consumers = list(n.conv_consumers)
            n.conv_consumers = []

    def _plan_bn_backward_fusion(self):
        readers = {}
        for m in self.nodes:
            for k, v in vars(m).items():
                if k == "out":
                    continue
                for t in (v if isinstance(v, (list, tuple)) else [v]):
                    if isinstance(t, Tensor):
                        readers.setdefault(id(t), set()).add(id(m))
        for n in self.nodes:
            if not isinstance(n, BatchNorm) or not n.out.requires_grad:
                continue
            cons = n.conv_consumers if n.defer_apply else n.mat_consumers
            if not cons or (not n.defer_apply and readers.get(id(n.out), set()) != {id(c) for c in cons}):
                continue
            last = min(cons, key=self.nodes.index)
            if last.stride not in (1, 2) or (last.stride == 2 and last.dil != 1) or last.x.shape[3] % 4 != 0:
                continue
            tiles = fn.conv_dgrad_bn_tiles(last.x.shape, last.stride)
            if tiles <= 0:
                continue
            n.bwd_sums = (fn.zeros(tiles, 2, last.x.shape[3], device=self.device), tiles)
            last.bn_bwd_node = n

    def _plan_gradient_magnitudes(self):
        first_reader, readers = {}, {}
        for idx, m in enumerate(self.nodes):
            for k, v in vars(m).items():
                if k == "out":
                    continue
                for t in (v if isinstance(v, (list, tuple)) else [v]):
                    if isinstance(t, Tensor):
                        first_reader.setdefault(id(t), idx)
                        readers.setdefault(id(t), set()).add(idx)
        for idx, n in enumerate(self.nodes):
            if isinstance(n, BatchNorm):
                n.completes_x_grad = first_reader.get(id(n.x)) == idx
        for idx, n in enumerate(self.nodes):
            r = getattr(n, "residual", None)
            if isinstance(n, Conv) and n.am_dy is not None and r is not None and r.requires_grad:
                prod = getattr(r, "producer", None)
                if (isinstance(prod, Conv) and prod.am_dy is not None and prod.out is r and readers.get(id(r)) == {idx}
                        and not prod.relu and prod.b is None):
                    prod.am_dy = n.am_dy

    def _plan_gradient_planes(self):
        if self.math != "f16x2" or self.device.type != "cuda":
            return
        readers = {}
        for idx, m in enumerate(self.nodes):
            for k, v in vars(m).items():
                if k in ("out", "x_raw"):
                    continue
                for t in (v if isinstance(v, (list, tuple)) else [v]):
                    if isinstance(t, Tensor):
                        readers.setdefault(id(t), set()).add(idx)
        gatherer = {id(n.bn_bwd_node): n for n in self.nodes if isinstance(n, Conv) and getattr(n, "bn_bwd_node", None) is not None}
        for idx, n in enumerate(self.nodes):
            if not isinstance(n, BatchNorm) or n.bwd_sums is None or id(n) not in gatherer:
                continue
            prod, x = getattr(n.x, "producer", None), n.x
            if not (isinstance(prod, Conv) and prod.out is x and readers.get(id(x)) == {idx} and x.requires_grad
                    and x.dtype == torch.float32 and n.completes_x_grad and n.tile_stats is not None):
                continue
            if (prod.tap_expand or prod.relu or prod.b is not None or prod.residual is not None or prod.input_sum_grad is not None
                    or prod.am_dy is None or x.shape[3] != prod.cout or prod.cout % 32 != 0 or prod.out_minmax is None
                    or gatherer[id(n)].math != "f16x2"):
                continue
            n.dx_planes = True
            n.x_ext = fn.zeros(2, x.shape[3], device=self.device)
            n.am_dyin = self.new_scalar(backward=True)

    def _plan_input_planes(self):
        if self.math != "f16x2" or self.device.type != "cuda":
            return
        for n in self.nodes:
            if not isinstance(n, BatchNorm) or n.defer_apply is not True or n.tile_stats is None:
                continue
            x = n.x
            if (x.dtype != torch.float32 or x.shape[3] % 32 != 0 or x.data is None
                    or getattr(getattr(x, "producer", None), "out_minmax", None) is None):
                continue
            cons = [c for c in n.conv_consumers if c.math == "f16x2" and c.wp is not None and c.x_raw is x]
            reads = sum(c.w.shape[1] * c.w.shape[2] * ((c.cout + 127) // 128) for c in cons)
            if reads < X_PLANES_MIN_READS:
                continue
            n.planes = fn.zeros(*x.shape, device=self.device)
            for c in cons:
                c.x_planes_bn = n

    def finalize(self, seed=0):
        self._resolve_auto_deferred()
        self._plan_side_sync()
        if _os.environ.get("DSPN_X_PLANES", "1") != "0":
            self._plan_input_planes()
        self._plan_bn_backward_fusion()
        self._plan_gradient_magnitudes()
        if _os.environ.get("DSPN_DY_PLANES", "1") != "0":
            self._plan_gradient_planes()
        self._wt_pairs_nodes = [n for n in self.nodes if isinstance(n, Conv) and (n.wt is not None or n.wh is not None)]
        off = 0
        for p in self.param_order:
            p.offset = off
            off += (p.size + 3) // 4 * 4
        self.arena = torch.zeros(off, dtype=torch.float32, device=self.device)
        self.grad_arena = torch.zeros_like(self.arena)
        self.mom_arena = torch.zeros_like(self.arena)
        rng = np.random.Generator(np.random.PCG64(seed))
        host = np.zeros(off, np.float32)
        for p in self.param_order:
            host[p.offset:p.offset + p.size] = np.asarray(p.init(rng, p.shape), np.float32).reshape(-1)
        self.arena.copy_(torch.from_numpy(host))
        for p in self.param_order:
            p.data = self.arena[p.offset:p.offset + p.size].view(p.shape)
            p.grad = self.grad_arena[p.offset:p.offset + p.size].view(p.shape)
        if self._wt_pairs_nodes and self.device.type == "cuda":
            for n in self._wt_pairs_nodes:
                if n.wt is None:
                    n.wt = fn.zeros(n.w.shape[3], n.w.shape[1], n.w.shape[2], n.out.shape[3], device=self.device,
                                    dtype=n.wh.dtype)
            pairs = [n for n in self._wt_pairs_nodes if n.wtp is None or n.wh is not None]
            if pairs:
                self.wt_table = fn.weight_transpose_table([(n.w.data, n.wt, n.wh) for n in pairs], self.device)
                self.half_operands = self.wt_table[3]
        if self.device.type == "cuda":
            if self.math == "f16x2" and self._nscal:
                self.scalars = torch.zeros(self._nscal * fn.ABSMAX_SLOTS, dtype=torch.float32, device=self.device)
                self.scalars_min = torch.full((self._nscal,), float("inf"), dtype=torch.float32, device=self.device)
                wnodes = [n for n in self.nodes if getattr(n, "am_w", None) is not None and getattr(n, "w", None) is not None]
                pairs = [(n.w.data, self.scalar(n.am_w)) for n in wnodes]
                self._am_table_slots = {n.am_w for n in wnodes}
                if pairs:
                    self.am_table = fn.absmax_table(pairs, self.device)
                    if self.guard["enabled"]:
                        self.wmin_table = fn.absmin_rows_table(
                            [(n.w.data.view(n.w.shape[0], -1), self.scalars_min[n.am_w:n.am_w + 1]) for n in wnodes], self.device)
            planes = [(n.w.data, n.wp, n.wtp) + ((self.scalar(n.am_w),) if self.math == "f16x2" else ())
                      for n in self.nodes if isinstance(n, Conv) and (n.wp is not None or n.wtp is not None)]
            if planes:
                self.wp_table = fn.weight_planes_table(planes, self.device)
        if self.device.type == "cuda":
            for n in self.nodes:
                if isinstance(n, Conv):
                    n.alloc_slabs()
        return self

    def flush_slabs(self, key="all", convs=None, beside=False):
        if key not in self.slab_tables:
            nodes = [n for n in (convs if convs is not None else self.nodes) if isinstance(n, Conv) and n.slabs is not None]
            table = fn.slab_reduce_table([(n.slabs, n.w.grad, False) for n in nodes], self.device) if nodes else None
            self.slab_tables[key] = (nodes, table)
        nodes, table = self.slab_tables[key]
        st = self.__dict__.get("_wg")
        beside = beside and st is not None and st["last"] is not None
        if not beside:
            self.wgrad_beside_join()
        if not nodes:
            return
        ran = nodes if all(n.slabs_fresh for n in nodes) else [n for n in nodes if n.slabs_fresh]
        if ran:
            args = table if ran is nodes else fn.slab_reduce_table([(n.slabs, n.w.grad, False) for n in ran], self.device)
            if beside:
                main, side = torch.cuda.current_stream(self.device), st["stream"]
                ev = self._wg_event()
                ev.record(main)
                side.wait_event(ev)
                with torch.cuda.stream(side):
                    fn.slab_reduce_batch(*args)
                    done = self._wg_event()
                    done.record(side)
                st["last"] = done
            else:
                fn.slab_reduce_batch(*args)
        for n in nodes:
            n.slabs_fresh = False

    def load_params(self, values):
        for k, v in values.items():
            self.params[k].data.copy_(torch.from_numpy(np.ascontiguousarray(v, np.float32)).view(self.params[k].shape))


    def _node_tensors(self, n):
# ... 331 lines not shown
def deconv_bilinear_init(channels):
    def f(rng, shape):
        k_p, r, s, c_p = shape
        factor = (r + 1) // 2
        center = factor - 1 if r % 2 == 1 else factor - 0.5
        og = np.ogrid[:r, :s]
        filt = (1 - abs(og[0] - center) / factor) * (1 - abs(og[1] - center) / factor)
        w = np.zeros(shape, np.float32)
        for i in range(channels):
            w[i, :, :, i] = filt
        return w
    return f


def init_affine_identity(rng, shape):
    return np.array([1, 0, 0, 0, 1, 0], np.float32)


def affine_matrix_param(g, name="affine_matrix"):
    p = g.param(name, (6,), init_affine_identity)
    p.logical, p.kind = (1, 6), "raw"
    return p


class InputNCHW(Node):

    def __init__(self, g, src, name="data_nhwc"):
        self.src = src
        N, C, H, W = src.shape
        self.out = g.tensor((N, H, W, fn.padc(C)), name, requires_grad=False)
        self.out.channels = C

    def forward(self):
        fn.nchw_to_nhwc(self.src.data, out=self.out.data)


FUSE_MAXPOOL_BACKWARD = _os.environ.get("DSPN_FUSE_POOL_BWD", "1") != "0"
X_PLANES_MIN_READS = int(_os.environ.get("DSPN_X_PLANES_MIN_READS", "6"))


class BatchNorm(Node):

    def __init__(self, g, x, name, fix_gamma=False, eps=2e-5, relu=False, beta_grad_from_consumer=False,
                 defer_apply=False):
        C = x.shape[-1]
        if not FUSE_BATCHNORM:
            defer_apply = False
        self.x, self.eps, self.relu = x, eps, relu
        self.gamma = None if fix_gamma else g.param(name + "_gamma", (C,), init_ones)
        self.beta = g.param(name + "_beta", (C,), init_zeros)
        for p in (self.gamma, self.beta):
            if p is not None:
                p.logical = (x.channels or C,)
        g.bn_names.append((name, x.channels or C, bool(fix_gamma)))
        g.bn_nodes[name] = self
        self.channels = x.channels or C
        self.momentum, self.use_global_stats = float(g.bn_momentum), bool(g.bn_global)
        self.moving_mean = torch.zeros(C, dtype=torch.float32, device=g.device)
        self.moving_var = torch.ones(C, dtype=torch.float32, device=g.device)
        self.mean = fn.zeros(C, device=g.device)
        self.rstd = fn.zeros(C, device=g.device)
        self.scale = fn.zeros(C, device=g.device)
        self.shift = fn.zeros(C, device=g.device)
        self.defer_apply = defer_apply
        self.tile_stats = (x.producer.enable_out_stats()
                           if FUSE_BATCHNORM and getattr(x, "producer", None) is not None else None)
        self.out = g.tensor(x.shape, name + ("_relu" if relu else "_out"), requires_grad=not beta_grad_from_consumer,
                            virtual=bool(defer_apply))
        if defer_apply:
            self.out.affine_src = (x, self.scale, self.shift, relu)
        self.out.bn_node = self
        self.am_out = g.new_scalar() if (g.math == "f16x2" and self.out.dtype == torch.float32) else None
        self.out.am_slot = self.am_out
        self.conv_consumers = []
        self.mat_consumers = []
        self.bwd_sums = None
        self.bwd_sums_ready = False
        self.dx_planes, self.x_ext, self.am_dyin = False, None, None
        self.planes, self.planes_ready = None, False
        self.pool_grad = None
        self._g = g
        self.completes_x_grad = False
        self._pending = None

    def _moving(self):
        if self.use_global_stats:
            mode = fn.BN_GLOBAL
        elif self._g.bn_track:
            mode = fn.BN_TRACK
        else:
            return None
        return fn.bn_moving(self.moving_mean, self.moving_var, self.momentum, mode, self.channels)

    def forward(self):
        moving = self._moving()
        if self.tile_stats is not None:
            buf, tiles, tile_rows = self.tile_stats
            rows = int(np.prod(self.x.shape[:-1]))
            g, mm, am = self._g, getattr(self.x.producer, "out_minmax", None), None
            slot = g._am_x.get((id(self.x), id(self.scale))) if (mm is not None and g.scalars is not None) else None
            if slot is not None:
                am = g.scalar(slot)
                g._am_done.add(slot)
            fn.bn_stats_from_tiles(buf, tiles, tile_rows, rows, self.x.shape[-1], self.eps,
                                   None if self.gamma is None else self.gamma.data, self.beta.data,
                                   self.mean, self.rstd, self.scale, self.shift,
                                   tile_minmax=mm if am is not None else None, relu=self.relu, out_absmax=am,
                                   out_absmin=None if am is None else g.scalars_min[slot:slot + 1],
                                   out_chan_minmax=self.x_ext if am is not None else None, moving=moving)
            self.planes_ready = self.planes is not None and am is not None
            if self.planes_ready:
                fn.bn_apply_planes(self.x.data, self.scale, self.shift, am, relu=self.relu, out=self.planes)
        else:
            fn.bn_stats(self.x.data, self.eps, None if self.gamma is None else self.gamma.data, self.beta.data,
                        self.mean, self.rstd, self.scale, self.shift, moving=moving)
        if not self.defer_apply:
            am = self._g.scalar(self.am_out)
            fn.bn_apply(self.x.data, self.scale, self.shift, relu=self.relu, out=self.out.data, out_absmax=am)
            if am is not None:
                self._g._am_done.add(self.am_out)

    def _x_ext_valid(self):
        g = self._g
        slot = g._am_x.get((id(self.x), id(self.scale)))
        return slot is not None and slot in g._am_done

    def finalize_beside(self):
        g = self._g
        if (not FINALIZE_BESIDE or g.device.type != "cuda" or not self.bwd_sums_ready or self.pool_grad is not None
                or not self.out._gw or self._pending is not None):
            return False
        self.backward(beside=True)
        return self._pending is not None

    def _from_sums(self, beside, args, kw):
        if not beside:
            fn.bn_backward_from_sums(*args, **kw)
            return
        fn.bn_backward_from_sums(*args, phase=1, park=True, **kw)
        self._pending = (args, kw)

    def backward(self, beside=False):
        if self._pending is not None:
            args, kw = self._pending
            self._pending = None
            fn.bn_backward_from_sums(*args, phase=2, **kw)
            return
        if not self.out._gw:
            return
        am = None
        if self.x.requires_grad:
            dx, acc = self.x.grad_target()
            prod, g = getattr(self.x, "producer", None), self._g
            if (isinstance(prod, Conv) and prod.am_dy is not None and g.scalars is not None and dx.dtype == torch.float32
                    and self.completes_x_grad):
                am = g.scalar(prod.am_dy)
                g._am_done.add(prod.am_dy)
        else:
            dx, acc = (self.out.grad if self.pool_grad is None else self.out.own_grad()), False
        if self.pool_grad is not None:
            argmax, dyp, k, s, p = self.pool_grad
            self.pool_grad = None
            if not acc:
                fn.bn_backward_maxpool(self.x.data, self.scale, self.shift, dyp, argmax, k, s, p, self.mean, self.rstd,
                                       None if self.gamma is None else self.gamma.data, relu=self.relu, dx=dx,
                                       dgamma=None if self.gamma is None else self.gamma.grad, dbeta=self.beta.grad, dx_absmax=am)
                return
            fn.maxpool_backward_argmax(argmax, dyp, self.out.shape, k, s, p, dx=self.out.own_grad())
            self.out.grad = self.out.own_grad()
        if (self.bwd_sums_ready and self.dx_planes and am is not None and not acc and self._x_ext_valid()
                and not getattr(prod, "guard_fb", False)):
            self.bwd_sums_ready = False
            self._from_sums(beside, (self.x.data, self.scale, self.shift, self.out.grad, self.mean, self.rstd,
                                     None if self.gamma is None else self.gamma.data, self.bwd_sums[0], self.bwd_sums[1]),
                            dict(relu=self.relu, dx=dx, dgamma=None if self.gamma is None else self.gamma.grad,
                                 dbeta=self.beta.grad, accumulate=False, dx_absmax=am,
                                 dy_absmax=self._g.scalar(self.am_dyin), x_chan_minmax=self.x_ext, dx_planes=True,
                                 dx_absmin=g.scalars_min[prod.am_dy:prod.am_dy + 1] if g.guard["enabled"] else None))
            self.x.grad_planes = True
            return
        if self.bwd_sums_ready:
            self.bwd_sums_ready = False
            self._from_sums(beside, (self.x.data, self.scale, self.shift, self.out.grad, self.mean, self.rstd,
                                     None if self.gamma is None else self.gamma.data, self.bwd_sums[0], self.bwd_sums[1]),
                            dict(relu=self.relu, dx=dx, dgamma=None if self.gamma is None else self.gamma.grad,
                                 dbeta=self.beta.grad, accumulate=acc, dx_absmax=am))
            return
        assert not beside, "finalize_beside() without the data gradient's sums"
        fn.bn_backward(self.x.data, self.scale, self.shift, self.out.grad, self.mean, self.rstd,
                       None if self.gamma is None else self.gamma.data, relu=self.relu, dx=dx,
                       dgamma=None if self.gamma is None else self.gamma.grad, dbeta=self.beta.grad,
                       accumulate=acc, dx_absmax=am)


WGRAD_SIDE = int(_os.environ.get("DSPN_WGRAD_SIDE", "1"))
WGRAD_SIDE_MIN_US = float(_os.environ.get("DSPN_WGRAD_SIDE_MIN_US", "30"))

FINALIZE_BESIDE = _os.environ.get("DSPN_FINALIZE_BESIDE", "1") != "0"

FUSE_CONV_MAGNITUDES = _os.environ.get("DSPN_CONV_MAGNITUDES", "1") != "0"


def xa_unavailable(conv):
    return conv.out.data is None or conv.out.data.shape[-1] % 4 != 0


class Conv(Node):

    def __init__(self, g, x, name, num_filter, kernel, stride=1, pad=0, dilate=1, no_bias=True, relu=False,
                 init="xavier", cin_logical=None, cout_phys=None, input_sum_grad=None, residual=None, out_name=None,
                 tap_expand=False):
        N, H, W, Cin = x.shape
        kh, kw = fn._hw(kernel)
        ph, pw = fn._hw(pad)
        self.x, self.stride, self.pad, self.dil, self.relu = x, stride, (ph, pw), dilate, relu
        self.x_raw, self.in_affine = x, None
        if x.affine_src is not None:
            raw, sc, sh, arelu = x.affine_src
            self.x_raw, self.in_affine = raw, (sc, sh, arelu)
            assert not tap_expand
            x.bn_node.conv_consumers.append(self)
        elif getattr(x, "bn_node", None) is not None and not tap_expand:
            x.bn_node.mat_consumers.append(self)
        self.cout = num_filter
        self.input_sum_grad = input_sum_grad
        cin_meta = cin_logical if cin_logical is not None else (x.channels or Cin)
        cin_logical = Cin if cin_logical is None else cin_logical
        self.w = g.param(name + "_weight", (num_filter, kh, kw, Cin), conv_weight_init(init, cin_logical))
        self.b = None if no_bias else g.param(name + "_bias", (num_filter,), init_zeros)
        self.w.logical, self.w.kind = (num_filter, cin_meta, kh, kw), "conv"
        if self.b is not None:
            self.b.logical = (num_filter,)
        Ho, Wo = fn.conv_out_size(H, kh, stride, ph, dilate), fn.conv_out_size(W, kw, stride, pw, dilate)
        ldc = fn.padc(num_filter) if cout_phys is None else cout_phys
        self.out = g.tensor((N, Ho, Wo, ldc), out_name or (name + "_out"))
        self.out.channels = num_filter
        self.out.producer = self
        self.slabs, self.slabs_fresh = None, False
        self.out_stats = None
        self.out_minmax = None
        self._g = g
        self.residual = residual
        assert residual is None or residual.shape == self.out.shape
        half = self.out.dtype == torch.bfloat16
        self.wt_shape = (Cin, kh, kw, ldc)
        planes_t = g.device.type == "cuda" and x.requires_grad and fn.needs_planes(self.out.dtype, ldc, g.math)
        self.wt = None if (not x.requires_grad or planes_t) else fn.zeros(Cin, kh, kw, ldc, device=g.device, dtype=self.out.dtype)
        self.wh = fn.zeros(num_filter, kh, kw, Cin, device=g.device, dtype=torch.bfloat16) if half else None
        self.math = g.math
        self.am_x = self.am_dy = self.am_w = None
        if g.math == "f16x2" and self.out.dtype == torch.float32:
            key = (id(self.x_raw), None if self.in_affine is None else id(self.in_affine[0]))
            if key not in g._am_x:
                g._am_x[key] = g.new_scalar()
            self.am_x, self.am_dy, self.am_w = g._am_x[key], g.new_scalar(backward=True), g.new_scalar()
        self.am_out = g.new_scalar() if (self.am_x is not None and not tap_expand) else None
        if self.am_out is not None:
            self.out.am_slot = self.am_out
        if self.am_x is not None and self.in_affine is None:
            g.want_magnitude(self.x_raw)
        self.x_planes_bn = None
        self.guard_fb = False
        self.wp = self.wtp = None
        if g.device.type == "cuda":
            npc = fn.plane_pieces(g.math)
            if fn.needs_planes(self.out.dtype, Cin, g.math):
                self.wp = fn.zeros(num_filter, kh * kw, Cin // 32, npc, 32, device=g.device, dtype=torch.bfloat16)
            if x.requires_grad and fn.needs_planes(self.out.dtype, ldc, g.math):
                self.wtp = fn.zeros(Cin, kh * kw, ldc // 32, npc, 32, device=g.device, dtype=torch.bfloat16)
        self.tap_expand = bool(tap_expand) and kh * kw > 1
        if self.tap_expand:
            assert stride == 1 and dilate == 1 and not relu and residual is None
            assert (Ho, Wo) == (H, W), "tap expansion needs a 'same' convolution"
            self.z = fn.act_zeros(N, H, W, fn.padc(num_filter * kh * kw), device=g.device)
        self.flops_fwd = 2.0 * cin_logical * num_filter * kh * kw * Ho * Wo * N
        self.flops_bwd = self.flops_fwd * (2 if x.requires_grad else 1)

    def alloc_slabs(self):
        cout, kh, kw, cin = self.w.shape
        wshape = (cout * kh * kw, 1, 1, cin) if self.tap_expand else self.w.shape
        xs = self.x.shape
        splits = fn.conv2d_wgrad_splits(xs, self.z.shape if self.tap_expand else self.out.shape, wshape,
                                        1 if self.tap_expand else self.stride)
        if splits > 0 and self.w.data.numel() % 4 == 0:
            self.slabs = fn.zeros(splits, self.w.data.numel(), device=self._g.device)

    def wop(self):
        return self.w.data if self.wh is None else self.wh

    def enable_out_stats(self):
        if self.tap_expand or self.out.shape[3] != self.cout or self.cout % 4 != 0:
            return None
        if self.out_stats is None:
            rows = self.out.shape[0] * self.out.shape[1] * self.out.shape[2]
            tiles, tile_rows = fn.conv_stats_layout(rows, self.cout)
            if tiles == 0:
                return None
            self.out_stats = (fn.zeros(tiles, 2, self.cout, device=self._g.device), tiles, tile_rows)
            if self.math == "f16x2" and self.out.dtype == torch.float32:
                self.out_minmax = fn.zeros(tiles, 2, self.cout, device=self._g.device)
        return self.out_stats

    def _magnitudes(self, which):
        g = self._g
        if self.am_x is None or g.scalars is None:
            return None
        if which == "x" and self.am_x not in g._am_done:
            src = self.x_raw
            while src.alias_of is not None:
                src = src.alias_of
            prod = getattr(src, "producer", None)
            table = getattr(prod, "out_minmax", None) if getattr(prod, "out", None) is src else None
            if table is not None:
                fn.absmax(table.view(-1, table.shape[-1]), self.in_affine, out=g.scalar(self.am_x))
            elif src.am_slot is not None and src.am_slot in g._am_done:
                if self.in_affine is None:
                    return g.scalar(src.am_slot)
                fn.absmax_affine_bound(self.in_affine[0], self.in_affine[1], g.scalar(src.am_slot), g.scalar(self.am_x))
            else:
                fn.absmax(self.x_raw.data, self.in_affine, out=g.scalar(self.am_x))
            g._am_done.add(self.am_x)
        return g.scalar({"x": self.am_x, "dy": self.am_dy, "w": self.am_w}[which])

    def forward(self):
        xa, wa = self._magnitudes("x"), self._magnitudes("w")
        if self.tap_expand:
            cout, kh, kw, cin = self.w.shape
            fn.conv2d_forward(self.x.data, self.wop().view(cout * kh * kw, 1, 1, cin), None, 1, 0, 1, out=self.z,
                              w_planes=self.wp, math=self.math,
                              x_absmax=xa, w_absmax=wa)
            fn.tap_sum(self.z, None if self.b is None else self.b.data, cout, kh, kw, self.pad, out=self.out.data)
            return
        if self.guard_fb:
            return self._forward_fallback()
        xp = self._x_planes()
        oa = self._out_magnitude()
        fn.conv2d_forward(self.x_raw.data if xp is None else xp, self.wop(), None if self.b is None else self.b.data, self.stride,
                          self.pad, self.dil, relu=self.relu, out=self.out.data,
                          residual=None if self.residual is None else self.residual.data,
                          in_affine=self.in_affine if xp is None else None,
                          out_stats=None if self.out_stats is None else self.out_stats[0], w_planes=self.wp,
                          math=self.math, x_absmax=xa, w_absmax=wa, out_minmax=self.out_minmax, x_planes=xp is not None,
                          out_absmax=oa)
        if oa is not None:
            self._g._am_done.add(self.am_out)

    def _out_magnitude(self):
        g = self._g
        if (not FUSE_CONV_MAGNITUDES or self.am_out is None or g.scalars is None or self.out_stats is not None
                or self.am_out not in g._am_wanted or xa_unavailable(self)):
            return None
        return g.scalar(self.am_out)

    def _x_planes(self):
        bn = self.x_planes_bn
        if self.guard_fb:
            return None
        return bn.planes if (bn is not None and bn.planes_ready and self.am_x in self._g._am_done) else None

    def _w3(self, transposed):
        cols = self.wt_shape[3] if transposed else self.w.shape[3]
        if cols % 32 != 0:
            return None
        return fn.weight_planes(self.w.data, transposed=transposed, cols=cols, math="bf16x3")

    def _forward_fallback(self):
        fn.conv2d_forward(self.x_raw.data, self.wop(), None if self.b is None else self.b.data, self.stride, self.pad, self.dil,
                          relu=self.relu, out=self.out.data, residual=None if self.residual is None else self.residual.data,
                          in_affine=self.in_affine, out_stats=None if self.out_stats is None else self.out_stats[0],
                          w_planes=self._w3(False), math="bf16x3")
        if self.out_minmax is not None:
            fn.tile_minmax(self.out.data, self.out_stats[2], self.out_minmax)
        oa = self._out_magnitude()
        if oa is not None:
            fn.absmax(self.out.data, out=oa)
            self._g._am_done.add(self.am_out)
        self._g.guard["calls"] += 1
        self._g.guard["calls_total"] += 1

    def backward(self):
        if not self.out._gw:
            return
        dy = self.out.grad
        planes = self.out.grad_planes
        if self.relu and self.b is not None:
            dya0 = None
            if (FUSE_CONV_MAGNITUDES and self.am_dy is not None and self._g.scalars is not None
                    and self.am_dy not in self._g._am_done and dy.dtype == torch.float32):
                dya0 = self._g.scalar(self.am_dy)
            fn.relu_backward_colsum(self.out.data, dy, self.cout, dx=dy, out=self.b.grad, dx_absmax=dya0)
            if dya0 is not None:
                self._g._am_done.add(self.am_dy)
        elif self.relu:
            fn.relu_backward(self.out.data, dy, dx=dy)
        if self.residual is not None and self.residual.requires_grad:
            self.residual.give_grad(dy)
        if self.b is not None and not self.relu:
            fn.colsum(dy, self.cout, out=self.b.grad)
        xa, dya, wa = self._magnitudes("x"), self._magnitudes("dy"), self._magnitudes("w")
        if dya is not None and self.am_dy not in self._g._am_done:
            fn.absmax(dy, out=dya)
            self._g._am_done.add(self.am_dy)
        bn = getattr(self, "bn_bwd_node", None) if self.x.requires_grad else None
        early = (bn is not None and FINALIZE_BESIDE and not self.guard_fb and self._g.device.type == "cuda"
                 and bn.pool_grad is None)
        if (WGRAD_SIDE and self._g.wgrad_side_allowed and self._g.device.type == "cuda" and (bn is not None or self._g.batchnorm_chain()) and self._wgrad_worth_a_stream()
                and self._g.wgrad_beside(self, dy, planes, xa, dya)):
            early = False
            if self.input_sum_grad is not None:
                fn.conv2d_input_sum_grad(dy, self.w.data, self.x.shape, self.stride, self.pad, self.dil,
                                         out=self.input_sum_grad.grad)
            if self.x.requires_grad:
                self._data_gradient(dy, planes, dya, wa)
            return
        if early:
            self._data_gradient(dy, planes, dya, wa)
            bn.finalize_beside()
        self._weight_gradient(dy, planes, xa, dya)
        if self.input_sum_grad is not None:
            fn.conv2d_input_sum_grad(dy, self.w.data, self.x.shape, self.stride, self.pad, self.dil,
                                     out=self.input_sum_grad.grad)
        if self.x.requires_grad and not early:
            self._data_gradient(dy, planes, dya, wa)

    def _wgrad_worth_a_stream(self):
        w = getattr(self, "_wg_worth", None)
        if w is None:
            P = float(np.prod(self.out.shape[:-1]))
            cout, kh, kw, cin = self.w.shape
            esz = 4.0 if self.out.dtype == torch.float32 else 2.0
            est = max(2.0 * P * cout * kh * kw * cin / 2.5e14, esz * (P * cout + float(np.prod(self.x.shape))) / 4e12)
            w = self._wg_worth = est * 1e6 >= WGRAD_SIDE_MIN_US
        return w

    def _weight_gradient(self, dy, planes, xa, dya):
        if self.tap_expand:
            cout, kh, kw, cin = self.w.shape
            fn.tap_spread(dy, cout, kh, kw, self.pad, out=self.z)
            if self.slabs is not None:
                fn.conv2d_wgrad_slabs(self.x.data, self.z, (cout * kh * kw, 1, 1, cin), self.slabs, 1, 0, 1, math=self.math,
                                      x_absmax=xa)
            else:
                fn.conv2d_wgrad(self.x.data, self.z, (cout * kh * kw, 1, 1, cin), 1, 0, 1,
                                out=self.w.grad.view(cout * kh * kw, 1, 1, cin), math=self.math, x_absmax=xa)
        elif self.guard_fb:
            assert not planes, "a convolution on the guard's fallback got its gradient as piece planes"
            if self.slabs is not None:
                fn.conv2d_wgrad_slabs(self.x_raw.data, dy, self.w.shape, self.slabs, self.stride, self.pad, self.dil,
                                      in_affine=self.in_affine, math="bf16x3")
            else:
                fn.conv2d_wgrad(self.x_raw.data, dy, self.w.shape, self.stride, self.pad, self.dil, out=self.w.grad,
                                in_affine=self.in_affine, math="bf16x3")
            self._g.guard["calls"] += 1
            self._g.guard["calls_total"] += 1
        elif self.slabs is not None:
            xp = self._x_planes()
            fn.conv2d_wgrad_slabs(self.x_raw.data if xp is None else xp, dy, self.w.shape, self.slabs, self.stride, self.pad,
                                  self.dil, in_affine=self.in_affine if xp is None else None, math=self.math, x_absmax=xa,
                                  dy_absmax=dya, dy_planes=planes, x_planes=xp is not None)
        else:
            xp = self._x_planes()
            fn.conv2d_wgrad(self.x_raw.data if xp is None else xp, dy, self.w.shape, self.stride, self.pad, self.dil,
                            out=self.w.grad, in_affine=self.in_affine if xp is None else None, math=self.math, x_absmax=xa,
                            dy_absmax=dya, dy_planes=planes, x_planes=xp is not None)
        self.slabs_fresh = self.slabs is not None

    def _data_gradient(self, dy, planes, dya, wa):
        if self.wtp is not None and self._g.wp_table is None:
            fn.weight_planes(self.w.data, transposed=True, cols=self.wtp.shape[2] * 32, out=self.wtp, math=self.math,
                             w_absmax=wa)
        elif self.wtp is None and not self._g.wt_batched:
            fn.weight_transpose(self.w.data, out=self.wt, copy=self.wh)
        dx, acc = self.x.grad_target()
        bn = getattr(self, "bn_bwd_node", None)
        bn_bwd, bn_dya = None, None
        if bn is not None:
            bn_bwd = (bn.x.data, bn.scale, bn.shift, bn.mean, bn.rstd, bn.relu, bn.bwd_sums[0])
            bn.bwd_sums_ready = True
            if bn.dx_planes:
                bn_dya = self._g.scalar(bn.am_dyin)
        if self.guard_fb:
            w3 = self._w3(True)
            fn.conv2d_dgrad(dy, self.wt if w3 is None else None, self.x.shape, self.stride, self.pad, self.dil, out=dx,
                            accumulate=acc, bn_bwd=bn_bwd, wt_planes=w3, math="bf16x3", wt_shape=self.wt_shape)
            if bn_dya is not None:
                fn.absmax(dx, out=bn_dya)
            self._g.guard["calls"] += 1
            self._g.guard["calls_total"] += 1
            return
        fn.conv2d_dgrad(dy, self.wt, self.x.shape, self.stride, self.pad, self.dil, out=dx, accumulate=acc,
                        bn_bwd=bn_bwd, wt_planes=self.wtp, math=self.math, dy_absmax=dya, w_absmax=wa,
                        bn_dy_absmax=bn_dya, dy_planes=planes, wt_shape=self.wt_shape)


class BilinearConcatConv(Node):

    def __init__(self, g, inputs, name, num_filter, kernel, pad, target_hw, theta, init="maxdim"):
        N = inputs[0].shape[0]
        kh, kw = fn._hw(kernel)
        self.pad = fn._hw(pad)
        assert (kh - 1) // 2 == self.pad[0] and (kw - 1) // 2 == self.pad[1], "needs a 'same' convolution"
        Ht, Wt = target_hw
        self.inputs = inputs
        self.theta = theta
        self.offsets = np.cumsum([0] + [t.shape[3] for t in inputs]).tolist()
        Cin = self.offsets[-1]
        self.cout, self.kh, self.kw = num_filter, kh, kw
        self.w = g.param(name + "_weight", (num_filter, kh, kw, Cin), conv_weight_init(init, Cin))
        self.w.logical, self.w.kind = (num_filter, Cin, kh, kw), "conv"
        T = num_filter * kh * kw
        Tp = fn.padc(T)
        self.T = T
        half = fn.ACT_DTYPE == torch.bfloat16
        self.z = fn.act_zeros(N, Ht, Wt, Tp, device=g.device)
        self.zc, self.wc, self.wct, self.dwc, self.wch, self.wcp = [], [], [], [], [], []
        self.math = g.math
        self._g = g
        f16 = g.math == "f16x2"
        self.am = [(g.new_scalar(), g.new_scalar(), g.new_scalar(backward=True)) if f16 else (None, None, None) for _ in inputs]
        self.am_w = g.new_scalar() if f16 else None
        for t in inputs:
            self.zc.append(fn.act_zeros(N, t.shape[1], t.shape[2], Tp, device=g.device))
            self.wc.append(fn.zeros(T, 1, 1, t.shape[3], device=g.device))
            self.wct.append(fn.act_zeros(t.shape[3], 1, 1, Tp, device=g.device))
            self.wch.append(fn.act_zeros(T, 1, 1, t.shape[3], device=g.device) if half else None)
            self.dwc.append(fn.zeros(T, 1, 1, t.shape[3], device=g.device))
            self.wcp.append(fn.zeros(T, 1, t.shape[3] // 32, fn.plane_pieces(g.math), 32, device=g.device, dtype=torch.bfloat16)
                            if g.device.type == "cuda" and fn.needs_planes(self.zc[-1].dtype, t.shape[3], g.math) else None)
        self.sources = None
        self.tpart = None
        self.out = g.tensor((N, Ht, Wt, fn.padc(num_filter)), name + "_out")
        self.out.channels = num_filter
        self.flops_fwd = sum(2.0 * t.shape[3] * T * t.shape[1] * t.shape[2] * N for t in inputs)
        self.flops_bwd = self.flops_fwd + sum(2.0 * t.shape[3] * T * t.shape[1] * t.shape[2] * N
                                              for t in inputs if t.requires_grad)
        self.flops_direct = 2.0 * Cin * T * Ht * Wt * N

    def _gather_weights(self):
        w2d = self.w.data
        Cin = self.offsets[-1]
        for c, t in enumerate(self.inputs):
            fn.copy_block(w2d, self.wc[c], 1, self.T, t.shape[3], 0, Cin, self.offsets[c], 0, t.shape[3], 0)

    def forward(self):
        self._gather_weights()
        for c, t in enumerate(self.inputs):
            if self.wch[c] is not None:
                fn.weight_transpose(self.wc[c], out=self.wct[c], copy=self.wch[c])
            xa, wa = self._g.magnitude(self.am[c][0], t.data, src=t), self._g.scalar(self.am_w)
            if self.wcp[c] is not None:
                fn.weight_planes(self.wc[c], out=self.wcp[c], math=self.math, w_absmax=wa)
            fn.conv2d_forward(t.data, self.wc[c] if self.wch[c] is None else self.wch[c], None, 1, 0, 1, out=self.zc[c],
                              w_planes=self.wcp[c], math=self.math, x_absmax=xa, w_absmax=wa)
        if self.sources is None:
            self.sources = fn.SamplerSources([(z, 0) for z in self.zc])
        fn.affine_sampler_forward(self.sources, self.theta.data, self.z)
        fn.tap_sum(self.z, None, self.cout, self.kh, self.kw, self.pad, out=self.out.data)
# ... 239 lines not shown
```

dspnet_amd/functional.py:

```python
import ctypes
import os

import torch

from . import _lib
from ._lib import check

_c = ctypes
_vp = _c.c_void_p
_i = _c.c_int
_ll = _c.c_longlong
_f = _c.c_float
_sz = _c.c_size_t

_lib.register({
    "dspn_conv2d_split_workspace_bytes": (_sz, [_ll, _i]),
    "dspn_conv2d_forward_f32": (_i, [_vp, _vp, _vp, _vp, _vp, _i, _i, _i, _i, _i, _i, _i, _i, _i, _i, _i, _i, _i,
                                     _ll, _i, _i, _i, _vp, _sz, _vp]),
    "dspn_conv2d_forward_bn_f32": (_i, [_vp, _vp, _vp, _i, _vp, _vp, _vp, _vp, _vp, _i, _i, _i, _i, _i, _i, _i, _i, _i, _i, _i, _i,
                                        _i, _ll, _i, _i, _i, _vp, _sz, _vp, _i, _vp, _vp, _vp, _sz, _vp]),
    "dspn_absmax_f32": (_i, [_vp, _ll, _i, _vp, _vp, _i, _vp, _vp]),
    "dspn_absmax_batch_f32": (_i, [_vp, _i, _ll, _vp]),
    "dspn_conv2d_weight_planes_f32": (_i, [_vp, _vp, _vp, _i, _i, _i, _i, _i, _vp, _vp]),
    "dspn_conv2d_weight_planes_tiles": (_ll, [_i, _i, _i, _i, _i]),
    "dspn_conv2d_weight_planes_batch_f32": (_i, [_vp, _i, _ll, _vp]),
    "dspn_conv2d_stats_layout": (_i, [_ll, _i, _c.POINTER(_c.c_int)]),
    "dspn_bn_stats_from_tiles_f32": (_i, [_vp, _i, _i, _ll, _i, _f, _vp, _vp, _vp, _vp, _vp, _vp, _vp, _i, _vp, _vp, _vp, _vp, _sz, _vp]),
    "dspn_bn_tiles_workspace_bytes": (_sz, [_i, _i]),
    "dspn_conv2d_wgrad_bn_f32": (_i, [_vp, _vp, _vp, _i, _vp, _vp, _i, _i, _i, _i, _i, _i, _i, _i, _i, _i, _i, _i, _i, _i,
                                      _i, _i, _vp, _vp, _vp, _sz, _vp]),
    "dspn_conv2d_wgrad_splits": (_i, [_i, _i, _i, _i, _i, _i, _i, _i]),
    "dspn_conv2d_wgrad_slabs_f32": (_i, [_vp, _vp, _vp, _i, _vp, _vp, _sz, _i, _i, _i, _i, _i, _i, _i, _i, _i, _i, _i, _i,
                                         _i, _i, _i, _vp, _vp, _vp]),
    "dspn_conv2d_slab_reduce_batch_f32": (_i, [_vp, _i, _ll, _vp]),
    "dspn_conv2d_weight_transpose_batch_f32": (_i, [_vp, _i, _ll, _vp]),
    "dspn_conv2d_weight_transpose_tiles": (_ll, [_i, _i, _i, _i]),
    "dspn_conv2d_weight_transpose_f32": (_i, [_vp, _vp, _i, _i, _i, _i, _vp]),
    "dspn_conv2d_dgrad_f32": (_i, [_vp, _vp, _vp, _i, _i, _i, _i, _i, _i, _i, _i, _i, _i, _i, _i, _i, _i, _i, _vp,
                                   _sz, _vp]),
    "dspn_conv2d_dgrad_bn_tiles": (_i, [_i, _i, _i, _i, _i]),
    "dspn_conv2d_dgrad_bn_f32": (_i, [_vp, _vp, _vp, _vp, _i, _i, _i, _i, _i, _i, _i, _i, _i, _i, _i, _i, _i, _i, _i,
                                      _vp, _vp, _vp, _vp, _vp, _i, _vp, _sz, _vp, _i, _vp, _vp, _vp, _sz, _vp]),
    "dspn_bn_backward_from_sums_f32": (_i, [_vp, _vp, _vp, _vp, _vp, _vp, _vp, _vp, _i, _vp, _vp, _vp, _ll, _i, _i, _i,
                                            _vp, _vp, _vp, _vp, _i, _vp, _sz, _vp]),
    "dspn_absmin_rows_batch_f32": (_i, [_vp, _i, _ll, _vp]),
    "dspn_tile_minmax_f32": (_i, [_vp, _ll, _i, _i, _vp, _vp]),
    "dspn_conv2d_input_sum_grad_workspace_bytes": (_sz, [_i, _i, _i, _i, _i]),
    "dspn_conv2d_input_sum_grad_f32": (_i, [_vp, _vp, _vp, _i, _i, _i, _i, _i, _i, _i, _i, _i, _i, _i, _i, _i, _i,
                                            _vp, _sz, _vp]),
    "dspn_conv2d_wgrad_workspace_bytes": (_sz, [_i, _i, _i, _i, _i, _i, _i]),
    "dspn_conv2d_wgrad_f32": (_i, [_vp, _vp, _vp, _i, _i, _i, _i, _i, _i, _i, _i, _i, _i, _i, _i, _i, _i, _i,
                                   _vp, _sz, _vp]),
    "dspn_bn_workspace_bytes": (_sz, [_ll, _i]),
    "dspn_bn_stats_f32": (_i, [_vp, _ll, _i, _f, _vp, _vp, _vp, _vp, _vp, _vp, _vp, _sz, _vp]),
    "dspn_bn_apply_f32": (_i, [_vp, _vp, _vp, _vp, _ll, _i, _i, _vp, _vp]),
    "dspn_bn_apply_planes_f32": (_i, [_vp, _vp, _vp, _vp, _ll, _i, _i, _vp, _vp]),
    "dspn_absmax_affine_bound_f32": (_i, [_vp, _vp, _i, _vp, _vp, _vp]),
    "dspn_bn_backward_f32": (_i, [_vp, _vp, _vp, _vp, _vp, _vp, _vp, _vp, _vp, _vp, _ll, _i, _i, _i, _vp, _vp, _sz,
                                  _vp]),
    "dspn_add_f32": (_i, [_vp, _vp, _vp, _ll, _vp]),
    "dspn_relu_backward_f32": (_i, [_vp, _vp, _vp, _ll, _i, _vp]),
    "dspn_fill_f32": (_i, [_vp, _f, _ll, _vp]),
    "dspn_relu_backward_colsum_f32": (_i, [_vp, _vp, _vp, _ll, _i, _i, _vp, _vp, _vp, _sz, _vp]),
    "dspn_colsum_workspace_bytes": (_sz, [_ll, _i]),
    "dspn_colsum_f32": (_i, [_vp, _ll, _i, _i, _vp, _vp, _sz, _vp]),
    "dspn_nchw_to_nhwc_f32": (_i, [_vp, _vp, _i, _i, _i, _i, _i, _vp]),
    "dspn_nhwc_to_nchw_f32": (_i, [_vp, _vp, _i, _i, _i, _i, _i, _vp]),
    "dspn_copy_block_f32": (_i, [_vp, _vp, _i, _ll, _i, _ll, _i, _i, _ll, _i, _i, _i, _vp]),
    "dspn_copy_block_batch_f32": (_i, [_vp, _i, _ll, _vp]),
    "dspn_transpose_bnc_f32": (_i, [_vp, _vp, _i, _i, _i, _vp]),
    "dspn_avgpool2d_forward_f32": (_i, [_vp, _vp, _i, _i, _i, _i, _i, _i, _i, _i, _i, _vp]),
    "dspn_avgpool2d_backward_f32": (_i, [_vp, _vp, _i, _i, _i, _i, _i, _i, _i, _i, _i, _i, _vp]),
    "dspn_bilinear_backward_workspace_bytes": (_sz, [_i, _i, _i, _i]),
    "dspn_bilinear_backward_ws_f32": (_i, [_vp, _vp, _i, _i, _i, _i, _i, _i, _i, _i, _vp, _sz, _vp]),
    "dspn_seg_counts_f32": (_i, [_vp, _vp, _ll, _i, _i, _vp, _vp]),
    "dspn_seg_upsample_argmax_f32": (_i, [_vp, _vp, _i, _i, _i, _i, _i, _i, _i, _vp]),
    "dspn_tap_sum_f32": (_i, [_vp, _vp, _vp, _i, _i, _i, _i, _i, _i, _i, _i, _i, _i, _vp]),
    "dspn_tap_spread_f32": (_i, [_vp, _vp, _i, _i, _i, _i, _i, _i, _i, _i, _i, _i, _vp]),
    "dspn_maxpool_forward_f32": (_i, [_vp, _vp, _vp, _i, _i, _i, _i, _i, _i, _i, _i, _i, _vp]),
    "dspn_maxpool_forward_bn_f32": (_i, [_vp, _vp, _vp, _i, _vp, _vp, _i, _i, _i, _i, _i, _i, _i, _i, _i, _vp, _vp]),
    "dspn_maxpool_backward_argmax_f32": (_i, [_vp, _vp, _vp, _i, _i, _i, _i, _i, _i, _i, _i, _i, _vp]),
    "dspn_bn_backward_maxpool_f32": (_i, [_vp, _vp, _vp, _vp, _vp, _i, _i, _i, _i, _i, _i, _i, _i, _i, _vp, _vp, _vp, _vp, _vp,
                                          _vp, _i, _vp, _vp, _sz, _vp]),
    "dspn_maxpool_backward_f32": (_i, [_vp, _vp, _vp, _vp, _i, _i, _i, _i, _i, _i, _i, _i, _i, _vp]),
    "dspn_avgpool_forward_f32": (_i, [_vp, _vp, _i, _i, _i, _i, _i, _i, _i, _vp]),
    "dspn_avgpool_backward_f32": (_i, [_vp, _vp, _i, _i, _i, _i, _i, _i, _i, _i, _vp]),
    "dspn_bilinear_forward_f32": (_i, [_vp, _vp, _i, _i, _i, _i, _i, _i, _i, _i, _vp]),
    "dspn_bilinear_forward_acc_f32": (_i, [_vp, _vp, _i, _i, _i, _i, _i, _i, _i, _i, _vp]),
    "dspn_bilinear_backward_f32": (_i, [_vp, _vp, _i, _i, _i, _i, _i, _i, _i, _i, _vp]),
    "dspn_affine_sampler_forward_f32": (_i, [_vp, _vp, _vp, _vp, _vp, _i, _vp, _vp, _i, _i, _i, _i, _vp]),
    "dspn_affine_sampler_backward_data_f32": (_i, [_vp, _vp, _vp, _i, _i, _i, _i, _i, _i, _i, _i, _i, _vp]),
    "dspn_affine_sampler_theta_workspace_bytes": (_sz, [_i, _i, _i]),
    "dspn_affine_sampler_backward_theta_f32": (_i, [_vp, _vp, _vp, _vp, _vp, _i, _vp, _vp, _i, _i, _i, _i, _vp, _i,
                                                    _vp, _sz, _vp]),
    "dspn_affine_sampler_backward_data_theta_f32": (_i, [_vp, _vp, _vp, _vp, _i, _i, _i, _i, _i, _i, _i, _i, _i, _vp, _sz, _vp,
                                                         _vp, _sz, _vp]),
    "dspn_affine_sampler_theta_rows": (_ll, [_i, _i, _i, _i]),
    "dspn_affine_sampler_backward_workspace_bytes": (_sz, [_i, _i, _i, _i, _i]),
    "dspn_affine_sampler_theta_reduce_workspace_bytes": (_sz, [_ll]),
    "dspn_affine_sampler_theta_reduce": (_i, [_vp, _ll, _vp, _i, _vp, _sz, _vp]),
    "dspn_softmax_output_f32": (_i, [_vp, _vp, _vp, _vp, _ll, _i, _i, _f, _f, _vp, _vp]),
    "dspn_count_f32": (_i, [_vp, _ll, _i, _f, _vp, _vp]),
    "dspn_smooth_l1_forward_f32": (_i, [_vp, _vp, _vp, _vp, _ll, _vp]),
    "dspn_smooth_l1_backward_f32": (_i, [_vp, _vp, _vp, _vp, _ll, _f, _vp, _vp]),
    "dspn_cross_entropy_sum_f32": (_i, [_vp, _vp, _ll, _i, _i, _f, _f, _vp, _vp]),
    "dspn_sum_f32": (_i, [_vp, _ll, _vp, _vp]),
    "dspn_sgd_momentum_f32": (_i, [_vp, _vp, _vp, _ll, _f, _f, _f, _f, _vp]),
})


for _name in ("dspn_conv2d_forward_bn", "dspn_conv2d_dgrad_bn", "dspn_conv2d_wgrad_bn", "dspn_conv2d_wgrad_slabs",
              "dspn_conv2d_input_sum_grad", "dspn_bn_stats", "dspn_bn_apply", "dspn_bn_backward",
              "dspn_bn_backward_from_sums", "dspn_add", "dspn_relu_backward", "dspn_relu_backward_colsum", "dspn_colsum",
              "dspn_nchw_to_nhwc", "dspn_copy_block", "dspn_tap_sum", "dspn_tap_spread", "dspn_maxpool_forward", "dspn_maxpool_forward_bn",
              "dspn_maxpool_backward_argmax", "dspn_maxpool_backward", "dspn_avgpool_forward", "dspn_avgpool_backward",
              "dspn_avgpool2d_forward", "dspn_avgpool2d_backward", "dspn_softmax_output", "dspn_affine_sampler_forward",
              "dspn_affine_sampler_backward_data", "dspn_affine_sampler_backward_theta",
              "dspn_affine_sampler_backward_data_theta"):
    _lib.register({_name + "_bf16": _lib.SIGNATURES[_name + "_f32"]})
_lib.register({
    "dspn_conv2d_weight_prepare_bf16": (_i, [_vp, _vp, _vp, _i, _i, _i, _i, _vp]),
    "dspn_conv2d_weight_prepare_batch_bf16": (_i, [_vp, _i, _ll, _vp]),
    "dspn_copy_block_bf16_f32": _lib.SIGNATURES["dspn_copy_block_f32"],
    "dspn_copy_block_f32_bf16": _lib.SIGNATURES["dspn_copy_block_f32"],
})
# ... 258 lines not shown
    assert not x_planes or (math == 3 and x.dtype == torch.float32 and x_absmax is not None and in_affine is None)
    assert out_minmax is None or (out_stats is not None and out_minmax.numel() == out_stats.numel())
    assert out_absmax is None or (out_stats is None and math == 3 and x.dtype == torch.float32 and out_absmax.numel() == ABSMAX_SLOTS)
    if math == 3 and x.dtype == torch.float32:
        assert w_planes is None or w_absmax is not None, "f16x2 planes come with the magnitude block they were cut by"
        x_absmax = absmax(x, in_affine) if x_absmax is None else x_absmax
        w_absmax = absmax(w) if w_absmax is None else w_absmax
    else:
        x_absmax = w_absmax = None
    if needs_planes(x.dtype, Cin, math):
        if w_planes is None:
            w_planes = weight_planes(w, math=math, w_absmax=w_absmax)
    else:
        w_planes = None
    ph, pw = _hw(pad)
    Ho, Wo = conv_out_size(H, R, stride, ph, dil), conv_out_size(W, S, stride, pw, dil)
    if out is None:
        ldc = padc(Cout, x.dtype)
        out = (zeros if ldc != Cout else empty)(N, Ho, Wo, ldc, device=x.device, dtype=x.dtype)
    ldc = out.shape[3]
    assert w.dtype == x.dtype == out.dtype, (x.dtype, w.dtype, out.dtype)
    ws = workspace(L().dspn_conv2d_split_workspace_bytes(N * Ho * Wo, Cout), x.device, "split")
    assert residual is None or (residual.shape == out.shape and residual.dtype == out.dtype)
    sc, sh, arelu = in_affine if in_affine is not None else (None, None, False)
    check(_f("dspn_conv2d_forward_bn", x)(ptr(x), ptr(sc), ptr(sh), int(arelu), ptr(w), ptr(w_planes), ptr(bias),
                                         ptr(residual), ptr(out),
                                         N, H, W, Cin, Cout, R, S, stride, ph, pw, dil, Ho, Wo, 0, ldc, int(relu),
                                         int(accumulate), ptr(out_stats), 0 if out_stats is None else out_stats.numel() * 4,
                                         ptr(out_minmax if out_absmax is None else out_absmax),
                                         math | (MATH_X_PLANES if x_planes else 0), ptr(x_absmax),
                                         ptr(w_absmax), ptr(ws), ws.numel(), stream()),
          "conv2d_forward")
    return out


def weight_transpose_table(triples, device):
    import numpy as np
    rows = np.zeros(len(triples), dtype=[("w", "<u8"), ("wt", "<u8"), ("K", "<i4"), ("T", "<i4"), ("C", "<i4"),
                                         ("Kp", "<i4"), ("begin", "<i8"), ("wh", "<u8")])
    total = 0
    half = triples[0][1].dtype == torch.bfloat16
    for i, (w, wt, wh) in enumerate(triples):
        Cout, R, S, Cin = w.shape
        assert w.dtype == torch.float32 and wt.shape[:3] == (Cin, R, S) and w.is_contiguous() and wt.is_contiguous()
        assert (wt.dtype == torch.bfloat16) == half and (wh is None or (half and wh.shape == w.shape))
        rows[i] = (w.data_ptr(), wt.data_ptr(), Cout, R * S, Cin, wt.shape[3], total, 0 if wh is None else wh.data_ptr())
        total += int(L().dspn_conv2d_weight_transpose_tiles(Cout, R * S, Cin, wt.shape[3]))
    assert rows.dtype.itemsize == 48
    table = torch.from_numpy(rows.view(np.uint8).copy()).to(device)
    return table, len(triples), total, half


def weight_transpose_batch(table, n, total, half=False):
    f = L().dspn_conv2d_weight_prepare_batch_bf16 if half else L().dspn_conv2d_weight_transpose_batch_f32
    check(f(ptr(table), n, total, stream()), "weight_transpose_batch")


def weight_transpose(w, out=None, dtype=None, copy=None):
    Cout, R, S, Cin = w.shape
    dtype = out.dtype if out is not None else (dtype or torch.float32)
    Kp = padc(Cout, dtype) if out is None else out.shape[3]
    if out is None:
        out = empty(Cin, R, S, Kp, device=w.device, dtype=dtype)
    if dtype == torch.bfloat16:
        check(L().dspn_conv2d_weight_prepare_bf16(ptr(w), ptr(copy), ptr(out), Cout, R * S, Cin, Kp, stream()),
              "weight_prepare")
    else:
        check(L().dspn_conv2d_weight_transpose_f32(ptr(w), ptr(out), Cout, R * S, Cin, Kp, stream()),
              "weight_transpose")
    return out


def weight_cast(w):
    return w.to(torch.bfloat16)


def conv_dgrad_bn_tiles(x_shape, stride):
    N, H, W, C = x_shape
    return L().dspn_conv2d_dgrad_bn_tiles(N, H, W, C, stride)


MATH_DY_PLANES = 0x200
MATH_X_PLANES = 0x400


def conv2d_dgrad(dy, wt, x_shape, stride=1, pad=0, dil=1, out=None, accumulate=False, bn_bwd=None, wt_planes=None,
                 math=None, dy_absmax=None, w_absmax=None, bn_dy_absmax=None, dy_planes=False, wt_shape=None):
    N, H, W, Cx = x_shape
    Cin, R, S, ldy = wt.shape if wt is not None else wt_shape
    assert dy.shape[3] == ldy, (dy.shape, (Cin, R, S, ldy))
    assert wt is not None or wt_planes is not None
    math = _math_code(math)
    if math == 3 and dy.dtype == torch.float32:
        assert wt_planes is None or w_absmax is not None, "f16x2 planes come with the magnitude block they were cut by"
        assert not dy_planes or dy_absmax is not None, "piece-plane gradients come with the magnitude block they were cut by"
        dy_absmax = absmax(dy) if dy_absmax is None else dy_absmax
        w_absmax = absmax(wt) if w_absmax is None else w_absmax
    else:
        dy_absmax = w_absmax = None
    if needs_planes(dy.dtype, ldy, math):
        if wt_planes is None:
            wt_planes = weight_planes(wt, math=math, w_absmax=w_absmax)
    else:
        wt_planes = None
    Ho, Wo = dy.shape[1], dy.shape[2]
    if out is None:
        out = (zeros if Cx != Cin else empty)(N, H, W, Cx, device=dy.device, dtype=dy.dtype)
    assert (wt is None or wt.dtype == dy.dtype) and dy.dtype == out.dtype, (dy.dtype, out.dtype)
    ws = workspace(L().dspn_conv2d_split_workspace_bytes(N * H * W, Cin), dy.device, "split")
    ph, pw = _hw(pad)
    bx, bsc, bsh, bmu, brs, brelu, bsums = bn_bwd if bn_bwd is not None else (None, None, None, None, None, False, None)
    check(_f("dspn_conv2d_dgrad_bn", dy)(ptr(dy), ptr(wt), ptr(wt_planes), ptr(out), N, H, W, Cin, ldy, R, S, stride, ph, pw,
                                       dil, Ho, Wo, out.shape[3], int(accumulate), ptr(bx), ptr(bsc), ptr(bsh), ptr(bmu),
                                       ptr(brs), int(brelu), ptr(bsums), 0 if bsums is None else bsums.numel() * 4,
                                       ptr(bn_dy_absmax), math | (MATH_DY_PLANES if dy_planes else 0), ptr(dy_absmax),
                                       ptr(w_absmax), ptr(ws), ws.numel(), stream()), "conv2d_dgrad")
    return out


def _wgrad_absmax(x, dy, in_affine, math, x_absmax, dy_absmax):
    if math == 3 and x.dtype == torch.float32:
        return (absmax(x, in_affine) if x_absmax is None else x_absmax, absmax(dy) if dy_absmax is None else dy_absmax)
    return None, None


def conv2d_wgrad(x, dy, w_shape, stride=1, pad=0, dil=1, out=None, accumulate=False, in_affine=None, math=None,
                 x_absmax=None, dy_absmax=None, dy_planes=False, x_planes=False):
    N, H, W, Cin = x.shape
    Cout, R, S, Cw = w_shape
    assert Cw == Cin
    Ho, Wo, ldy = dy.shape[1], dy.shape[2], dy.shape[3]
    if out is None:
        out = empty(Cout, R, S, Cin, device=x.device)
    nbytes = L().dspn_conv2d_wgrad_workspace_bytes(N, Ho, Wo, Cin, Cout, R, S)
    ws = workspace(nbytes, x.device, "wgrad")
    ph, pw = _hw(pad)
    sc, sh, arelu = in_affine if in_affine is not None else (None, None, False)
    assert x.dtype == dy.dtype and out.dtype == torch.float32
    math = _math_code(math)
    assert not x_planes or (x_absmax is not None and in_affine is None)
    x_absmax, dy_absmax = _wgrad_absmax(x, dy, in_affine, math, x_absmax, dy_absmax)
    check(_f("dspn_conv2d_wgrad_bn", x)(ptr(x), ptr(sc), ptr(sh), int(arelu), ptr(dy), ptr(out), N, H, W, Cin, Cout, ldy,
                                       R, S, stride, ph, pw, dil, Ho, Wo, int(accumulate),
                                       math | (MATH_DY_PLANES if dy_planes else 0) | (MATH_X_PLANES if x_planes else 0),
                                       ptr(x_absmax), ptr(dy_absmax), ptr(ws), ws.numel(), stream()), "conv2d_wgrad")
    return out


def tap_sum(z, bias, cout, R, S, pad, out):
    N, H, W, ldz = z.shape
    ph, pw = _hw(pad)
    assert z.dtype == out.dtype
    check(_f("dspn_tap_sum", z)(ptr(z), ptr(bias), ptr(out), N, H, W, cout, out.shape[3], ldz, R, S, ph, pw, stream()),
          "tap_sum")
    return out


def tap_spread(dy, cout, R, S, pad, out):
    N, H, W, ldy = dy.shape
    ph, pw = _hw(pad)
    assert dy.dtype == out.dtype
    check(_f("dspn_tap_spread", dy)(ptr(dy), ptr(out), N, H, W, cout, ldy, out.shape[3], R, S, ph, pw, stream()),
          "tap_spread")
    return out


def conv2d_wgrad_splits(x_shape, dy_shape, w_shape, stride):
    N, H, W, Cin = x_shape
    Cout, R, S, _ = w_shape
    return L().dspn_conv2d_wgrad_splits(N, dy_shape[1], dy_shape[2], Cin, Cout, R, S, stride)


def conv2d_wgrad_slabs(x, dy, w_shape, slabs, stride=1, pad=0, dil=1, in_affine=None, math=None, x_absmax=None,
                       dy_absmax=None, dy_planes=False, x_planes=False):
    N, H, W, Cin = x.shape
    Cout, R, S, Cw = w_shape
    assert Cw == Cin
    ph, pw = _hw(pad)
    sc, sh, arelu = in_affine if in_affine is not None else (None, None, False)
    assert x.dtype == dy.dtype and slabs.dtype == torch.float32
    math = _math_code(math)
    assert not x_planes or (x_absmax is not None and in_affine is None)
    x_absmax, dy_absmax = _wgrad_absmax(x, dy, in_affine, math, x_absmax, dy_absmax)
    check(_f("dspn_conv2d_wgrad_slabs", x)(ptr(x), ptr(sc), ptr(sh), int(arelu), ptr(dy), ptr(slabs), slabs.numel() * 4,
                                          N, H, W, Cin, Cout, dy.shape[3], R, S, stride, ph, pw, dil, dy.shape[1],
                                          dy.shape[2],
                                          math | (MATH_DY_PLANES if dy_planes else 0) | (MATH_X_PLANES if x_planes else 0),
                                          ptr(x_absmax), ptr(dy_absmax), stream()), "conv2d_wgrad_slabs")


def slab_reduce_table(entries, device):
    import numpy as np
    rows = np.zeros(len(entries), dtype=[("slab", "<u8"), ("dw", "<u8"), ("n4", "<i8"), ("splits", "<i4"),
                                         ("acc", "<i4"), ("begin", "<i8")])
    total = 0
    for i, (slabs, dw, acc) in enumerate(entries):
        assert dw.numel() % 4 == 0 and slabs.numel() == slabs.shape[0] * dw.numel()
        rows[i] = (slabs.data_ptr(), dw.data_ptr(), dw.numel() // 4, slabs.shape[0], int(acc), total)
        total += dw.numel() // 4
    assert rows.dtype.itemsize == 40
    return torch.from_numpy(rows.view(np.uint8).copy()).to(device), len(entries), total

# ... 10 lines not shown
    ws = workspace(L().dspn_conv2d_input_sum_grad_workspace_bytes(Ho, Wo, ldy, R, S), dy.device, "sumgrad")
    ph, pw = _hw(pad)
    check(_f("dspn_conv2d_input_sum_grad", dy)(ptr(dy), ptr(w), ptr(out), N, H, W, Cin, Cout, ldy, R, S, stride,
                                             ph, pw, dil, Ho, Wo, ptr(ws), ws.numel(), stream()),
          "conv2d_input_sum_grad")
    return out


def _rows(x):
    return x.numel() // x.shape[-1]


def bn_stats(x, eps, gamma, beta, mean=None, rstd=None, scale=None, shift=None, moving=None):
    C = x.shape[-1]
    rows = _rows(x)
    mean = empty(C, device=x.device) if mean is None else mean
    rstd = empty(C, device=x.device) if rstd is None else rstd
    scale = empty(C, device=x.device) if scale is None else scale
    shift = empty(C, device=x.device) if shift is None else shift
    ws = workspace(L().dspn_bn_workspace_bytes(rows, C), x.device, "bn")
    args = (ptr(x), rows, C, eps, ptr(gamma), ptr(beta), ptr(mean), ptr(rstd), ptr(scale), ptr(shift), ptr(ws), ws.numel())
    if moving is None:
        check(_f("dspn_bn_stats", x)(*args, stream()), "bn_stats")
    else:
        check(_f("dspn_bn_stats_ex", x)(*args, moving, stream()), "bn_stats_ex")
    return mean, rstd, scale, shift


def bn_apply(x, scale, shift, relu=False, out=None, out_absmax=None):
    out = torch.empty_like(x) if out is None else out
    assert out.dtype == x.dtype and (out_absmax is None or out_absmax.numel() == ABSMAX_SLOTS)
    check(_f("dspn_bn_apply", x)(ptr(x), ptr(scale), ptr(shift), ptr(out), _rows(x), x.shape[-1], int(relu),
                                ptr(out_absmax if x.dtype == torch.float32 else None), stream()), "bn_apply")
    return out


def bn_apply_planes(x, scale, shift, y_absmax, relu=False, out=None):
    out = torch.empty_like(x) if out is None else out
    assert x.dtype == out.dtype == torch.float32 and x.shape[-1] % 32 == 0 and y_absmax.numel() == ABSMAX_SLOTS
    check(L().dspn_bn_apply_planes_f32(ptr(x), ptr(scale), ptr(shift), ptr(out), _rows(x), x.shape[-1], int(relu),
                                       ptr(y_absmax), stream()), "bn_apply_planes")
    return out


def absmax_affine_bound(scale, shift, x_absmax, out):
    assert scale.numel() == shift.numel() and x_absmax.numel() == out.numel() == ABSMAX_SLOTS
    check(L().dspn_absmax_affine_bound_f32(ptr(scale), ptr(shift), scale.numel(), ptr(x_absmax), ptr(out), stream()),
          "absmax_affine_bound")
    return out


def bn_backward(x, scale, shift, dy, mean, rstd, gamma, relu=False, dx=None, dgamma=None, dbeta=None,
                accumulate=False, dx_absmax=None):
    C = x.shape[-1]
    rows = _rows(x)
    dx = torch.empty_like(x) if dx is None else dx
    dbeta = empty(C, device=x.device) if dbeta is None else dbeta
    if gamma is not None and dgamma is None:
        dgamma = empty(C, device=x.device)
    ws = workspace(L().dspn_bn_workspace_bytes(rows, C), x.device, "bn")
    assert dy.dtype == x.dtype == dx.dtype
    check(_f("dspn_bn_backward", x)(ptr(x), ptr(scale), ptr(shift), ptr(dy), ptr(mean), ptr(rstd), ptr(gamma), ptr(dx),
                                   ptr(dgamma), ptr(dbeta), rows, C, int(relu), int(accumulate), ptr(dx_absmax), ptr(ws),
                                   ws.numel(), stream()), "bn_backward")
    return dx, dgamma, dbeta


def bn_backward_maxpool(x, scale, shift, dy_pool, argmax, k, stride, pad, mean, rstd, gamma, relu=False, dx=None, dgamma=None,
                        dbeta=None, dx_absmax=None):
    N, H, W, C = x.shape
    assert x.dtype == dy_pool.dtype == torch.float32 and argmax.dtype == torch.uint8 and argmax.shape == dy_pool.shape
    dx = torch.empty_like(x) if dx is None else dx
    dbeta = empty(C, device=x.device) if dbeta is None else dbeta
    if gamma is not None and dgamma is None:
        dgamma = empty(C, device=x.device)
    ws = workspace(L().dspn_bn_workspace_bytes(N * H * W, C), x.device, "bn")
    check(L().dspn_bn_backward_maxpool_f32(ptr(x), ptr(scale), ptr(shift), ptr(dy_pool), ptr(argmax), N, H, W, C, k, stride, pad,
                                           dy_pool.shape[1], dy_pool.shape[2], ptr(mean), ptr(rstd), ptr(gamma), ptr(dx),
                                           ptr(dgamma), ptr(dbeta), int(relu), ptr(dx_absmax), ptr(ws), ws.numel(), stream()),
          "bn_backward_maxpool")
    return dx, dgamma, dbeta


def bn_backward_from_sums(x, scale, shift, dy, mean, rstd, gamma, sums, tiles, relu=False, dx=None, dgamma=None,
                          dbeta=None, accumulate=False, dx_absmax=None, dy_absmax=None, x_chan_minmax=None, dx_planes=False,
                          dx_absmin=None, phase=0, park=False):
    assert phase in (0, 1, 2) and (not park or phase == 1)
    C = x.shape[-1]
    rows = _rows(x)
    dx = torch.empty_like(x) if dx is None else dx
    dbeta = empty(C, device=x.device) if dbeta is None else dbeta
    if gamma is not None and dgamma is None:
        dgamma = empty(C, device=x.device)
    ws = workspace(12 * C + L().dspn_bn_tiles_workspace_bytes(tiles, C), x.device, "bn")
    assert dy.dtype == x.dtype == dx.dtype
    check(_f("dspn_bn_backward_from_sums", x)(ptr(x), ptr(scale), ptr(shift), ptr(dy), ptr(mean), ptr(rstd), ptr(gamma),
                                             ptr(sums), tiles, ptr(dx), ptr(dgamma), ptr(dbeta), rows, C, int(relu),
                                             int(accumulate), ptr(dx_absmax), ptr(dx_absmin), ptr(dy_absmax), ptr(x_chan_minmax),
                                             int(bool(dx_planes)) | (phase << 1) | (8 if park else 0), ptr(ws), ws.numel(), stream()),
          "bn_backward_from_sums")
    return dx, dgamma, dbeta


def add(a, b, out=None):
    out = torch.empty_like(a) if out is None else out
    assert a.dtype == b.dtype == out.dtype
    check(_f("dspn_add", a)(ptr(a), ptr(b), ptr(out), a.numel(), stream()), "add")
    return out


def relu_backward(y, dy, dx=None, accumulate=False):
    dx = torch.empty_like(y) if dx is None else dx
    assert y.dtype == dy.dtype == dx.dtype
    check(_f("dspn_relu_backward", y)(ptr(y), ptr(dy), ptr(dx), y.numel(), int(accumulate), stream()),
          "relu_backward")
    return dx


def relu_backward_colsum(y, dy, C, dx=None, out=None, dx_absmax=None):
    dx = dy if dx is None else dx
    ld = y.shape[-1]
    rows = _rows(y)
    out = empty(C, device=y.device) if out is None else out
    ws = workspace(L().dspn_colsum_workspace_bytes(rows, C), y.device, "colsum")
    assert y.dtype == dy.dtype == dx.dtype
    assert dx_absmax is None or (y.dtype == torch.float32 and dx_absmax.numel() == ABSMAX_SLOTS)
    check(_f("dspn_relu_backward_colsum", y)(ptr(y), ptr(dy), ptr(dx), rows, C, ld, ptr(out), ptr(dx_absmax), ptr(ws), ws.numel(),
                                             stream()), "relu_backward_colsum")
    return dx, out


def fill(t, v):
    check(L().dspn_fill_f32(ptr(t), float(v), t.numel(), stream()), "fill")
    return t


def colsum(a, C, out=None):
    ld = a.shape[-1]
    rows = _rows(a)
    out = empty(C, device=a.device) if out is None else out
    ws = workspace(L().dspn_colsum_workspace_bytes(rows, C), a.device, "colsum")
    check(_f("dspn_colsum", a)(ptr(a), rows, C, ld, ptr(out), ptr(ws), ws.numel(), stream()), "colsum")
    return out


def nchw_to_nhwc(src, Cp=None, out=None):
    N, C, H, W = src.shape
    Cp = (pad4(C) if out is None else out.shape[3]) if Cp is None else Cp
    out = empty(N, H, W, Cp, device=src.device) if out is None else out
    assert src.dtype == torch.float32
    check(_f("dspn_nchw_to_nhwc", out)(ptr(src), ptr(out), N, C, H, W, Cp, stream()), "nchw_to_nhwc")
    return out


def nhwc_to_nchw(src, C=None, out=None):
    N, H, W, Cp = src.shape
    C = Cp if C is None else C
    out = empty(N, C, H, W, device=src.device) if out is None else out
    check(L().dspn_nhwc_to_nchw_f32(ptr(src), ptr(out), N, C, H, W, Cp, stream()), "nhwc_to_nchw")
    return out


def copy_block_table(entries, device):
    import numpy as np
    rows = np.zeros(len(entries), dtype=[("src", "<u8"), ("dst", "<u8"), ("rps", "<i8"), ("sss", "<i8"), ("dss", "<i8"),
                                         ("C", "<i4"), ("lds", "<i4"), ("soff", "<i4"), ("ldd", "<i4"), ("doff", "<i4"),
                                         ("acc", "<i4"), ("begin", "<i8")])
    assert rows.dtype.itemsize == 72
    total = 0
    for i, (src, dst, samples, rps, C, sss, lds, soff, dss, ldd, doff, acc) in enumerate(entries):
        assert src.dtype == dst.dtype == torch.float32 and samples > 0 and rps > 0 and C > 0
        rows[i] = (src.data_ptr(), dst.data_ptr(), rps, sss, dss, C, lds, soff, ldd, doff, int(bool(acc)), total)
        total += samples * rps * C
    return torch.from_numpy(rows.view(np.uint8).copy()).to(device), len(entries), total


def copy_block_batch(table, n, total):
# ... 259 lines not shown
```

include/dspn_nn.h:

```cpp
#ifndef DSPN_NN_H_
#define DSPN_NN_H_

#include <stddef.h>

#ifdef __cplusplus
extern "C" {
#endif


size_t dspn_conv2d_split_workspace_bytes(long long out_pixels, int Cout);
#define DSPN_MATH_FP32 0
#define DSPN_MATH_BF16 1
#define DSPN_MATH_F32_BF16X3 2
#define DSPN_MATH_F32_F16X2 3
#define DSPN_MATH_UNSCALED_OK 0x100
#define DSPN_MATH_DY_PLANES 0x200
#define DSPN_MATH_X_PLANES 0x400

int dspn_conv2d_forward_f32(const float *x, const float *w, const float *bias, const float *residual, float *y,
                            int N, int H, int W, int Cin, int Cout, int R, int S,
                            int stride, int pad_h, int pad_w, int dil, int Ho, int Wo,
                            long long y_batch_stride, int y_ldc, int relu, int accumulate,
                            void *workspace, size_t workspace_bytes, void *stream);

int dspn_conv2d_forward_bn_f32(const float *x, const float *in_scale, const float *in_shift, int in_relu,
                               const float *w, const void *w_planes, const float *bias, const float *residual, float *y,
                               int N, int H, int W, int Cin, int Cout, int R, int S,
                               int stride, int pad_h, int pad_w, int dil, int Ho, int Wo,
                               long long y_batch_stride, int y_ldc, int relu, int accumulate,
                               float *out_stats, size_t out_stats_bytes, float *out_minmax, int math,
                               const float *x_absmax, const float *w_absmax,
                               void *workspace, size_t workspace_bytes, void *stream);
int dspn_conv2d_stats_layout(long long out_pixels, int Cout, int *tile_rows);

int dspn_conv2d_weight_planes_f32(const float *w, void *planes, void *planes_t, int Cout, int taps, int Cin, int cols_t,
                                  int pieces, const float *w_absmax, void *stream);
long long dspn_conv2d_weight_planes_tiles(int Cout, int taps, int Cin, int cols_t, int with_transposed);
int dspn_conv2d_weight_planes_batch_f32(const void *table, int n, long long total_tiles, void *stream);

int dspn_conv2d_weight_transpose_f32(const float *w, float *wt, int Cout, int taps, int Cin,
                                     int Cout_pad, void *stream);
long long dspn_conv2d_weight_transpose_tiles(int Cout, int taps, int Cin, int Cout_pad);
int dspn_conv2d_weight_transpose_batch_f32(const void *table, int n, long long total_tiles, void *stream);

int dspn_conv2d_dgrad_f32(const float *dy, const float *wt, float *dx,
                          int N, int H, int W, int Cin, int ldy, int R, int S,
                          int stride, int pad_h, int pad_w, int dil, int Ho, int Wo, int dx_ldc,
                          int accumulate, void *workspace, size_t workspace_bytes, void *stream);
int dspn_conv2d_dgrad_bn_tiles(int N, int H, int W, int Cin, int stride);
int dspn_conv2d_dgrad_bn_f32(const float *dy, const float *wt, const void *wt_planes, float *dx, int N, int H, int W, int Cin, int ldy,
                             int R, int S, int stride, int pad_h, int pad_w, int dil, int Ho, int Wo, int dx_ldc,
                             int accumulate, const float *bn_x, const float *bn_scale, const float *bn_shift,
                             const float *bn_mean, const float *bn_rstd, int bn_relu, float *bn_sums,
                             size_t bn_sums_bytes, float *bn_dy_absmax, int math, const float *dy_absmax, const float *w_absmax,
                             void *workspace, size_t workspace_bytes, void *stream);

size_t dspn_conv2d_input_sum_grad_workspace_bytes(int Ho, int Wo, int ldy, int R, int S);
int dspn_conv2d_input_sum_grad_f32(const float *dy, const float *w, float *out, int N, int H, int W,
                                   int Cin, int Cout, int ldy, int R, int S, int stride, int pad_h, int pad_w, int dil,
                                   int Ho, int Wo, void *workspace, size_t workspace_bytes, void *stream);

size_t dspn_conv2d_wgrad_workspace_bytes(int N, int Ho, int Wo, int Cin, int Cout, int R, int S);

int dspn_conv2d_wgrad_f32(const float *x, const float *dy, float *dw,
                          int N, int H, int W, int Cin, int Cout, int ldy, int R, int S,
                          int stride, int pad_h, int pad_w, int dil, int Ho, int Wo, int accumulate,
                          void *workspace, size_t workspace_bytes, void *stream);
int dspn_conv2d_wgrad_bn_f32(const float *x, const float *in_scale, const float *in_shift, int in_relu,
                             const float *dy, float *dw, int N, int H, int W, int Cin, int Cout, int ldy,
                             int R, int S, int stride, int pad_h, int pad_w, int dil, int Ho, int Wo,
                             int accumulate, int math, const float *x_absmax, const float *dy_absmax,
                             void *workspace, size_t workspace_bytes, void *stream);

int dspn_conv2d_wgrad_splits(int N, int Ho, int Wo, int Cin, int Cout, int R, int S, int stride);
int dspn_conv2d_wgrad_slabs_f32(const float *x, const float *in_scale, const float *in_shift, int in_relu,
                                const float *dy, float *slabs, size_t slabs_bytes, int N, int H, int W, int Cin,
                                int Cout, int ldy, int R, int S, int stride, int pad_h, int pad_w, int dil, int Ho,
                                int Wo, int math, const float *x_absmax, const float *dy_absmax, void *stream);
int dspn_conv2d_slab_reduce_batch_f32(const void *table, int n, long long total4, void *stream);

#define DSPN_ABSMAX_SLOTS 64
int dspn_absmax_f32(const float *x, long long rows, int C, const float *scale, const float *shift, int relu,
                    float *out_dev, void *stream);
int dspn_absmin_rows_batch_f32(const void *table, int n, long long total_rows, void *stream);
int dspn_tile_minmax_f32(const float *x, long long rows, int C, int tile_rows, float *minmax, void *stream);
int dspn_absmax_batch_f32(const void *table, int n, long long total_chunks, void *stream);
int dspn_absmax_affine_bound_f32(const float *scale, const float *shift, int C, const float *x_absmax_dev, float *out_dev,
                                 void *stream);

#ifdef DSPN_BF16_ELEMENT
typedef DSPN_BF16_ELEMENT dspn_bf16;
#else
typedef unsigned short dspn_bf16;
#endif
int dspn_conv2d_forward_bn_bf16(const dspn_bf16 *x, const float *in_scale, const float *in_shift, int in_relu,
                                const dspn_bf16 *w, const void *w_planes_unused, const float *bias, const dspn_bf16 *residual, dspn_bf16 *y,
                                int N, int H, int W, int Cin, int Cout, int R, int S,
                                int stride, int pad_h, int pad_w, int dil, int Ho, int Wo,
                                long long y_batch_stride, int y_ldc, int relu, int accumulate,
                                float *out_stats, size_t out_stats_bytes, float *out_minmax_unused, int math,
                                const float *absmax_unused_a, const float *absmax_unused_b,
                                void *workspace, size_t workspace_bytes, void *stream);
int dspn_conv2d_dgrad_bn_bf16(const dspn_bf16 *dy, const dspn_bf16 *wt, const void *wt_planes_unused, dspn_bf16 *dx, int N, int H, int W, int Cin,
                              int ldy, int R, int S, int stride, int pad_h, int pad_w, int dil, int Ho, int Wo,
                              int dx_ldc, int accumulate, const dspn_bf16 *bn_x, const float *bn_scale,
                              const float *bn_shift, const float *bn_mean, const float *bn_rstd, int bn_relu,
                              float *bn_sums, size_t bn_sums_bytes, float *bn_dy_absmax_unused, int math,
                              const float *absmax_unused_a, const float *absmax_unused_b, void *workspace,
                              size_t workspace_bytes, void *stream);
int dspn_conv2d_wgrad_bn_bf16(const dspn_bf16 *x, const float *in_scale, const float *in_shift, int in_relu,
                              const dspn_bf16 *dy, float *dw, int N, int H, int W, int Cin, int Cout, int ldy,
                              int R, int S, int stride, int pad_h, int pad_w, int dil, int Ho, int Wo,
                              int accumulate, int math, const float *absmax_unused_a, const float *absmax_unused_b,
                              void *workspace, size_t workspace_bytes, void *stream);
int dspn_conv2d_wgrad_slabs_bf16(const dspn_bf16 *x, const float *in_scale, const float *in_shift, int in_relu,
                                 const dspn_bf16 *dy, float *slabs, size_t slabs_bytes, int N, int H, int W, int Cin,
                                 int Cout, int ldy, int R, int S, int stride, int pad_h, int pad_w, int dil, int Ho,
                                 int Wo, int math, const float *absmax_unused_a, const float *absmax_unused_b, void *stream);
int dspn_conv2d_input_sum_grad_bf16(const dspn_bf16 *dy, const float *w, float *out, int N, int H, int W,
                                    int Cin, int Cout, int ldy, int R, int S, int stride, int pad_h, int pad_w, int dil,
                                    int Ho, int Wo, void *workspace, size_t workspace_bytes, void *stream);
int dspn_conv2d_weight_prepare_bf16(const float *w, dspn_bf16 *wh, dspn_bf16 *wt, int Cout, int taps, int Cin,
                                    int Cout_pad, void *stream);
int dspn_conv2d_weight_prepare_batch_bf16(const void *table, int n, long long total_tiles, void *stream);


size_t dspn_bn_workspace_bytes(long long rows, int C);

int dspn_bn_stats_f32(const float *x, long long rows, int C, float eps, const float *gamma,
                      const float *beta, float *mean, float *rstd, float *scale, float *shift,
                      void *workspace, size_t workspace_bytes, void *stream);

int dspn_bn_stats_from_tiles_f32(const float *tile_stats, int tiles, int tile_rows, long long rows, int C, float eps,
                                 const float *gamma, const float *beta, float *mean, float *rstd, float *scale,
                                 float *shift, const float *tile_minmax, int relu, float *out_absmax, float *out_absmin,
                                 float *out_chan_minmax, void *workspace, size_t workspace_bytes, void *stream);
size_t dspn_bn_tiles_workspace_bytes(int tiles, int C);

// ... 204 lines not shown
```

Measured before the change: 974.0 images/s.

## Recompute conv dgrad to fuse BatchNorm backward apply and skip dx round-trip

Adds a recompute path for a conv dgrad that feeds a BatchNorm backward. A first dgrad pass computes only the BN reduction sums without storing dx. A small kernel then turns those sums into per-channel coefficients, and a second dgrad pass applies the BN backward elementwise in its epilogue and writes the final input gradient. This trades a second GEMM for removing the write and re-read of the intermediate activation gradient and a separate BN-apply kernel. It only applies to plane-fed, stride-1 wide-family layers and falls back otherwise.

```diff
diff --git a/dspnet_amd/csrc/conv.hip b/dspnet_amd/csrc/conv.hip
--- a/dspnet_amd/csrc/conv.hip
+++ b/dspnet_amd/csrc/conv.hip
@@ -1669,7 +1669,7 @@
     return dspn::fail(DSPN_ERR_ARG_, "conv: BatchNorm-backward sums cannot be combined with an input affine or output statistics");
   if (g.bn_sums && (!(g.flags & 16) || g.Cout % 4 != 0))
     return dspn::fail(DSPN_ERR_ARG_, "conv2d_dgrad: BatchNorm sums need a 16-byte aligned dx with Cin %% 4 == 0");
-  if (g.dense && nblk < 192 && nk >= 16 && ws.ptr && !g.stats && !g.bn_sums) {
+  if (g.dense && nblk < 192 && nk >= 16 && ws.ptr && !g.stats && !g.bn_sums && !g.bn_mode) {
     splits = (int)std::min<long long>((384 + nblk - 1) / nblk, nk / 8);
     splits = std::max(1, std::min(splits, 32));
     while (splits > 1 && sizeof(float) * (size_t)splits * M * g.Cout > ws.bytes) --splits;
@@ -1687,11 +1687,14 @@
     if (kHalf) wide_ok = wide_ok && !g.in_scale && g.Cin % 64 == 0 && dspn::wide_tiles_mode() >= 2;
     else wide_ok = wide_ok && pre && g.bf16 == 3;
     if (wide_ok) {
-      int shape = dspn::conv::wide_tile_choice(M, g.Cout, nk, (g.stats || g.bn_sums) ? 1 : 0);
+      int shape = dspn::conv::wide_tile_choice(M, g.Cout, nk, (g.stats || g.bn_sums || g.bn_mode) ? 1 : 0);
       if (shape && !kHalf && !g.a_planes) shape = 10 + (shape == 1 ? 3 : shape);
-      if (shape) { *wide_used = true; return dspn::conv::launch_wide(shape, in, w, bias, out, g, s, residual); }
-    }
-  }
+      if (shape && (!g.bn_mode || shape <= 4)) { *wide_used = true; return dspn::conv::launch_wide(shape, in, w, bias, out, g, s, residual); }
+    }
+  }
+  if (g.bn_mode)
+    return dspn::fail(DSPN_ERR_ARG_, "conv2d_dgrad: the recomputed BatchNorm backward (bn_mode %d) needs a plane-fed layer of the wide "
+                      "family (dy as piece planes, a dense 16-byte aligned dx, no split-K)", g.bn_mode);
   if (cfg == 0 && eight) return launch_nt<4, 2, 1, 2>(in, w, bias, out, g, s, splits, per, ws.ptr, residual);
   switch (cfg) {
     case 0: return launch_nt<2, 2, 2, 2>(in, w, bias, out, g, s, splits, per, ws.ptr, residual);
@@ -1966,7 +1969,7 @@
 }
 #endif
 
-struct BnBwd { const st_t *x; const float *scale, *shift, *mean, *rstd; int relu; float *sums; float *dy_absmax; };
+struct BnBwd { const st_t *x; const float *scale, *shift, *mean, *rstd; int relu; float *sums; float *dy_absmax; int mode = 0; const float *coef = nullptr; };
 
 static int dgrad_tiles(int N, int H, int W, int Cin, int stride, int *per_class ) {
   int total = 0;
@@ -2002,7 +2005,8 @@
   g.a_absmax = scales.a; g.b_absmax = scales.b;
   g.bn_x = bn.x; g.bn_scale = bn.scale; g.bn_shift = bn.shift; g.bn_mean = bn.mean; g.bn_rstd = bn.rstd;
   g.bn_relu = bn.relu; g.bn_sums = bn.sums; g.bn_tile_base = 0;
-  g.bn_dy_absmax = (bn.sums && !kHalf && math == DSPN_MATH_F32_F16X2) ? reinterpret_cast<unsigned *>(bn.dy_absmax) : nullptr;
+  g.bn_dy_absmax = ((bn.sums || bn.mode == 2) && !kHalf && math == DSPN_MATH_F32_F16X2) ? reinterpret_cast<unsigned *>(bn.dy_absmax) : nullptr;
+  g.bn_mode = bn.mode; g.bn_coef = bn.coef;
   g.a_planes = scales.a_planes;
   int class_tiles[4] = {0, 0, 0, 0};
   if (bn.sums) dgrad_tiles(N, H, W, Cin, stride, class_tiles);
@@ -2054,7 +2058,11 @@
                              void *stream) {
   DSPN_REQUIRE(N > 0 && Ho > 0 && Wo > 0 && ldy > 0, "conv2d_dgrad: bad geometry");
   const int math_vouch = math & DSPN_MATH_UNSCALED_OK, dy_planes = (math & DSPN_MATH_DY_PLANES) ? 1 : 0;
-  math &= ~(DSPN_MATH_UNSCALED_OK | DSPN_MATH_DY_PLANES);
+  const int no_store = (math & DSPN_MATH_NO_STORE) ? 1 : 0;
+  math &= ~(DSPN_MATH_UNSCALED_OK | DSPN_MATH_DY_PLANES | DSPN_MATH_NO_STORE);
+  DSPN_REQUIRE(!no_store || (!dspn::kHalf && bn_sums && dy_planes && math == DSPN_MATH_F32_F16X2 && !accumulate && !bn_dy_absmax && stride == 1),
+               "conv2d_dgrad: DSPN_MATH_NO_STORE needs bn_sums, DSPN_MATH_F32_F16X2 with DSPN_MATH_DY_PLANES, stride 1, no accumulation "
+               "and no bn_dy_absmax (nothing is stored)");
   DSPN_REQUIRE(!dy_planes || (!dspn::kHalf && math == DSPN_MATH_F32_F16X2 && ldy % 32 == 0 && dy_absmax),
                "conv2d_dgrad: DSPN_MATH_DY_PLANES needs DSPN_MATH_F32_F16X2, ldy %% 32 == 0 and the block the planes were cut by (dy_absmax)");
   DSPN_REQUIRE(math >= DSPN_MATH_FP32 && math <= DSPN_MATH_F32_F16X2, "conv2d_dgrad: math is one of DSPN_MATH_*");
@@ -2073,12 +2081,33 @@
     const int n = std::min(nb, N - n0);
     const int rc = conv2d_dgrad_one(math, OpScales{dy_absmax, w_absmax, dy_planes}, dy + (long long)n0 * Ho * Wo * ldy, wt, wt_planes, dx + (long long)n0 * H * W * ldc, n, H,
                                     W, Cin, ldy, R, S, stride, pad_h, pad_w, dil, Ho, Wo, dx_ldc, accumulate,
-                                    BnBwd{bn_x, bn_scale, bn_shift, bn_mean, bn_rstd, bn_relu, bn_sums, bn_dy_absmax}, workspace,
+                                    BnBwd{bn_x, bn_scale, bn_shift, bn_mean, bn_rstd, bn_relu, bn_sums, bn_dy_absmax, no_store}, workspace,
                                     workspace_bytes, stream);
     if (rc) return rc;
   }
   return 0;
 }
+
+#ifndef DSPN_HALF
+int dspn_conv2d_dgrad_bn_apply_f32(const float *dy, const float *wt, const void *wt_planes, float *dx, int N, int H, int W, int Cin,
+                                   int ldy, int R, int S, int stride, int pad_h, int pad_w, int dil, int Ho, int Wo, int dx_ldc,
+                                   int accumulate, const float *bn_x, const float *bn_scale, const float *bn_shift, int bn_relu,
+                                   const float *coef, float *dx_absmax, int math, const float *dy_absmax, const float *w_absmax,
+                                   void *workspace, size_t workspace_bytes, void *stream) {
+  DSPN_REQUIRE(N > 0 && H > 0 && W > 0 && Ho > 0 && Wo > 0 && ldy > 0 && Cin > 0 && Cin % 4 == 0, "conv2d_dgrad_bn_apply: bad geometry");
+  DSPN_REQUIRE(dy && wt_planes && dx && bn_x && coef && (!bn_relu || (bn_scale && bn_shift)) && dy_absmax && w_absmax,
+               "conv2d_dgrad_bn_apply: null pointer (dy planes, wt_planes, dx, bn_x, coef, the ReLU's scale / shift, both magnitude blocks)");
+  DSPN_REQUIRE((math & ~DSPN_MATH_DY_PLANES) == DSPN_MATH_F32_F16X2 && (math & DSPN_MATH_DY_PLANES) && ldy % 32 == 0,
+               "conv2d_dgrad_bn_apply: DSPN_MATH_F32_F16X2 | DSPN_MATH_DY_PLANES with ldy %% 32 == 0 only");
+  DSPN_REQUIRE(stride == 1 && (dx_ldc <= 0 || dx_ldc == Cin), "conv2d_dgrad_bn_apply: stride 1 and a dense dx only");
+  DSPN_REQUIRE(static_cast<const void *>(dx) != static_cast<const void *>(bn_x), "conv2d_dgrad_bn_apply: dx must not be bn_x");
+  DSPN_REQUIRE(batch_chunk(N, (long long)sizeof(float) * Ho * Wo * ldy) == N, "conv2d_dgrad_bn_apply: dy of 2 GiB or more");
+  return conv2d_dgrad_one(DSPN_MATH_F32_F16X2, OpScales{dy_absmax, w_absmax, 1}, dy, wt, wt_planes, dx, N, H, W, Cin, ldy, R, S, stride,
+                          pad_h, pad_w, dil, Ho, Wo, dx_ldc, accumulate,
+                          BnBwd{bn_x, bn_scale, bn_shift, nullptr, nullptr, bn_relu, nullptr, dx_absmax, 2, coef}, workspace,
+                          workspace_bytes, stream);
+}
+#endif
 
 #ifndef DSPN_HALF
 int dspn_conv2d_dgrad_f32(const float *dy, const float *wt, float *dx, int N, int H, int W,
diff --git a/dspnet_amd/csrc/conv_geom.h b/dspnet_amd/csrc/conv_geom.h
--- a/dspnet_amd/csrc/conv_geom.h
+++ b/dspnet_amd/csrc/conv_geom.h
@@ -30,6 +30,8 @@
   float *bn_sums;
   int bn_relu, bn_tile_base;
   unsigned *bn_dy_absmax;
+  int bn_mode;
+  const float *bn_coef;
   const float *a_absmax, *b_absmax;
   int a_planes;
   const void *w_planes;
diff --git a/dspnet_amd/csrc/conv_wide.h b/dspnet_amd/csrc/conv_wide.h
--- a/dspnet_amd/csrc/conv_wide.h
+++ b/dspnet_amd/csrc/conv_wide.h
@@ -256,7 +256,7 @@
   const unsigned obytes = (unsigned)M * (unsigned)g.ldc * 4u;
   const __amdgpu_buffer_rsrc_t rs_o = __builtin_amdgcn_make_buffer_rsrc(out, 0, obytes, 0x00020000);
   const __amdgpu_buffer_rsrc_t rs_a = __builtin_amdgcn_make_buffer_rsrc(const_cast<float *>(addsrc ? addsrc : out), 0, addsrc ? obytes : 0u, 0x00020000);
-  const __amdgpu_buffer_rsrc_t rs_x = __builtin_amdgcn_make_buffer_rsrc(const_cast<float *>(EPI == 2 ? g.bn_x : out), 0, EPI == 2 ? obytes : 0u, 0x00020000);
+  const __amdgpu_buffer_rsrc_t rs_x = __builtin_amdgcn_make_buffer_rsrc(const_cast<float *>(EPI >= 2 ? g.bn_x : out), 0, EPI >= 2 ? obytes : 0u, 0x00020000);
   constexpr unsigned kOOB = 0x80000000u;
   constexpr float kInf = __builtin_huge_valf();
   int col[TN];
@@ -270,8 +270,17 @@
     cbyte[j] = cv[j] ? (unsigned)col[j] * 4u : kOOB;
     bv[j] = (has_bias && cv[j]) ? bias[col[j]] : 0.f;
     bsc[j] = bsh[j] = bmu[j] = brs[j] = 0.f;
-    if (EPI == 2 && cv[j]) {
+    if ((EPI == 2 || EPI == 3) && cv[j]) {
       bmu[j] = g.bn_mean[col[j]]; brs[j] = g.bn_rstd[col[j]];
+      if (g.bn_relu) { bsc[j] = g.bn_scale[col[j]]; bsh[j] = g.bn_shift[col[j]]; }
+    }
+  }
+  float ka[TN], kc1[TN], kc0[TN];
+#pragma unroll
+  for (int j = 0; j < TN; ++j) {
+    ka[j] = kc1[j] = kc0[j] = 0.f;
+    if (EPI == 4 && cv[j]) {
+      ka[j] = g.bn_coef[col[j]]; kc1[j] = g.bn_coef[g.Cout + col[j]]; kc0[j] = g.bn_coef[2 * g.Cout + col[j]];
       if (g.bn_relu) { bsc[j] = g.bn_scale[col[j]]; bsh[j] = g.bn_shift[col[j]]; }
     }
   }
@@ -284,8 +293,45 @@
   for (int j = 0; j < TN; ++j) { sK[j] = 0.f; s1[j] = 0.f; s2[j] = 0.f; vmn[j] = kInf; vmx[j] = -kInf; gs[j] = 0.f; gss[j] = 0.f; }
   const bool both = has_res && accum;
   constexpr int NB = TM * 16 / RB;
-  const bool need_rows = addsrc != nullptr || EPI == 2;
-  if constexpr (EPI == 2) {
+  const bool need_rows = addsrc != nullptr || EPI >= 2;
+  if constexpr (EPI == 4) {
+    float rq[2][RB][TN], xq[2][RB][TN];
+    auto request = [&](const int bb, const int s_) __attribute__((always_inline)) {
+      const int i = bb / (16 / RB), r0 = (bb % (16 / RB)) * RB;
+#pragma unroll
+      for (int rr = 0; rr < RB; ++rr) {
+        const int r = r0 + rr;
+        const unsigned rb = (unsigned)(row0 + 32 * i + (r & 3) + 8 * (r >> 2)) * pitch;
+#pragma unroll
+        for (int j = 0; j < TN; ++j) {
+          const unsigned off = rb + cbyte[j];
+          rq[s_][rr][j] = accum ? __builtin_bit_cast(float, __builtin_amdgcn_raw_buffer_load_b32(rs_a, (int)off, 0, 0)) : 0.f;
+          xq[s_][rr][j] = __builtin_bit_cast(float, __builtin_amdgcn_raw_buffer_load_b32(rs_x, (int)off, 0, 0));
+        }
+      }
+    };
+    const bool brelu = g.bn_relu != 0;
+    request(0, 0);
+#pragma unroll
+    for (int bb = 0; bb < NB; ++bb) {
+      const int i = bb / (16 / RB), r0 = (bb % (16 / RB)) * RB, s_ = bb & 1;
+      if (bb + 1 < NB) request(bb + 1, s_ ^ 1);
+#pragma unroll
+      for (int rr = 0; rr < RB; ++rr) {
+        const int r = r0 + rr;
+        const unsigned rb = (unsigned)(row0 + 32 * i + (r & 3) + 8 * (r >> 2)) * pitch;
+#pragma unroll
+        for (int j = 0; j < TN; ++j) {
+          float v = acc[i][j][r] * inv_a * inv_b + bv[j];
+          v += 0.f;
+          float o = dspn::bn_bwd_elem(xq[s_][rr][j], v, brelu, bsc[j], bsh[j], ka[j], kc1[j], kc0[j]);
+          if (accum) o += rq[s_][rr][j];
+          __builtin_amdgcn_raw_buffer_store_b32(__builtin_bit_cast(unsigned, o), rs_o, (int)(rb + cbyte[j]), 0, 0);
+          gmx = fmaxf(gmx, fabsf(o));
+        }
+      }
+    }
+  } else if constexpr (EPI == 2 || EPI == 3) {
     float rq[2][RB][TN], xq[2][RB][TN], oq[2][RB][TN];
     auto request = [&](const int bb, const int s_) __attribute__((always_inline)) {
       const int i = bb / (16 / RB), r0 = (bb % (16 / RB)) * RB;
@@ -296,9 +342,9 @@
 #pragma unroll
         for (int j = 0; j < TN; ++j) {
           const unsigned off = rb + cbyte[j];
-          rq[s_][rr][j] = addsrc ? __builtin_bit_cast(float, __builtin_amdgcn_raw_buffer_load_b32(rs_a, (int)off, 0, 0)) : 0.f;
+          rq[s_][rr][j] = (EPI == 2 && addsrc) ? __builtin_bit_cast(float, __builtin_amdgcn_raw_buffer_load_b32(rs_a, (int)off, 0, 0)) : 0.f;
           xq[s_][rr][j] = __builtin_bit_cast(float, __builtin_amdgcn_raw_buffer_load_b32(rs_x, (int)off, 0, 0));
-          oq[s_][rr][j] = both ? __builtin_bit_cast(float, __builtin_amdgcn_raw_buffer_load_b32(rs_o, (int)off, 0, 0)) : 0.f;
+          oq[s_][rr][j] = (EPI == 2 && both) ? __builtin_bit_cast(float, __builtin_amdgcn_raw_buffer_load_b32(rs_o, (int)off, 0, 0)) : 0.f;
         }
       }
     };
@@ -315,9 +361,9 @@
         for (int j = 0; j < TN; ++j) {
           float v = acc[i][j][r] * inv_a * inv_b + bv[j];
           v += rq[s_][rr][j];
-          if (both) v += oq[s_][rr][j];
+          if (EPI == 2 && both) v += oq[s_][rr][j];
           if (relu) v = v > 0.f ? v : 0.f;
-          __builtin_amdgcn_raw_buffer_store_b32(__builtin_bit_cast(unsigned, v), rs_o, (int)(rb + cbyte[j]), 0, 0);
+          if constexpr (EPI == 2) __builtin_amdgcn_raw_buffer_store_b32(__builtin_bit_cast(unsigned, v), rs_o, (int)(rb + cbyte[j]), 0, 0);
           const float xv = xq[s_][rr][j];
           const float gd = (!g.bn_relu || fmaf(xv, bsc[j], bsh[j]) > 0.f) ? v : 0.f;
           gs[j] += gd;
@@ -388,8 +434,8 @@
     for (int j = 0; j < TN; ++j) { s1[j] = s1p[j].x + s1p[j].y; s2[j] = s2p[j].x + s2p[j].y; }
   }
   if constexpr (EPI == 0) gmx_all = fmaxf(gmx_all, gmx);
-  if constexpr (EPI == 2) gmx_all = fmaxf(gmx_all, gmx);
-  if constexpr (EPI != 0) {
+  if constexpr (EPI == 2 || EPI == 4) gmx_all = fmaxf(gmx_all, gmx);
+  if constexpr (EPI != 0 && EPI != 4) {
     float *red = reinterpret_cast<float *>(exch);
     float *red2 = red + PARTS * BN * 4;
     const bool mmx = EPI == 1 && g.minmax != nullptr;
@@ -677,9 +723,9 @@
       char *exch = wsm + STAGES * STG;
       if constexpr (EXCH_IN_RING) {
         exch = wsm + last_slot * STG;
-        if constexpr (EPI != 0) { asm volatile("s_waitcnt lgkmcnt(0)" ::: "memory"); __builtin_amdgcn_s_barrier(); }
-      }
-      if constexpr (!kHalf) direct_epilogue<WAVES_M, WAVES_N, EPI, (EPI == 2 ? 4 : 8), SR>(g, exch, acc, inv_a, inv_b, m0, n0, M, tid, wave, bias, out, residual, gmx_all);
+        if constexpr (EPI != 0 && EPI != 4) { asm volatile("s_waitcnt lgkmcnt(0)" ::: "memory"); __builtin_amdgcn_s_barrier(); }
+      }
+      if constexpr (!kHalf) direct_epilogue<WAVES_M, WAVES_N, EPI, (EPI >= 2 ? 4 : 8), SR>(g, exch, acc, inv_a, inv_b, m0, n0, M, tid, wave, bias, out, residual, gmx_all);
       DSPN_STAMP(5);
     }
     DSPN_STAMP_FLUSH;
@@ -727,7 +773,7 @@
             st[(wm + i * 32 + (r & 3) + 8 * (r >> 2) + 4 * (lane >> 5)) * SLD + wn + j * 32 + (lane & 31)] = acc[i][j][r] * inv_a * inv_b;
     }
     DSPN_STAMP(3);
-    wide_epilogue<BM, BN, NTHR, EPI, SR>(g, wsm, m0, n0, M, tid, bias, out, residual, gmx_all, NoStage() DSPN_STAMP_ARG);
+    if constexpr (EPI <= 2) wide_epilogue<BM, BN, NTHR, EPI, SR>(g, wsm, m0, n0, M, tid, bias, out, residual, gmx_all, NoStage() DSPN_STAMP_ARG);
   }
   DSPN_STAMP_FLUSH;
   if constexpr (EPI != 1) wide_publish_absmax<NWV>(g, wsm, gmx_all, tid);
@@ -1168,12 +1214,17 @@
     const int nk = g.TR * g.TS * (g.Cin / 32);
     if (xt_enabled() && nk >= STAGES && xt_output_ok(g, WAVES_M * 64) &&
         (WAVES_M == 4 ? xt_c64_enabled() : (WAVES_N == 2 || xt_wide8_enabled()))) {
+      if (g.bn_mode == 1) return launch_ntw_impl<WAVES_M, WAVES_N, STAGES, 3, SR, true>(in, w, bias, out, g, s, residual);
+      if (g.bn_mode == 2) return launch_ntw_impl<WAVES_M, WAVES_N, STAGES, 4, SR, true>(in, w, bias, out, g, s, residual);
       if (g.bn_sums) return launch_ntw_impl<WAVES_M, WAVES_N, STAGES, 2, SR, true>(in, w, bias, out, g, s, residual);
       if (g.stats) return launch_ntw_impl<WAVES_M, WAVES_N, STAGES, 1, SR, true>(in, w, bias, out, g, s, residual);
       return launch_ntw_impl<WAVES_M, WAVES_N, STAGES, 0, SR, true>(in, w, bias, out, g, s, residual);
     }
   }
 #endif
+  if (g.bn_mode)
+    return dspn::fail(DSPN_ERR_ARG_, "conv2d_dgrad: the recomputed BatchNorm backward (bn_mode %d) needs the tile-spanning loop's direct "
+                      "epilogue, which this layer does not run on", g.bn_mode);
   if (g.bn_sums) return launch_ntw_impl<WAVES_M, WAVES_N, STAGES, 2, SR>(in, w, bias, out, g, s, residual);
   if (g.stats) return launch_ntw_impl<WAVES_M, WAVES_N, STAGES, 1, SR>(in, w, bias, out, g, s, residual);
   return launch_ntw_impl<WAVES_M, WAVES_N, STAGES, 0, SR>(in, w, bias, out, g, s, residual);
diff --git a/dspnet_amd/csrc/dspn_common.h b/dspnet_amd/csrc/dspn_common.h
--- a/dspnet_amd/csrc/dspn_common.h
+++ b/dspnet_amd/csrc/dspn_common.h
@@ -79,6 +79,18 @@
 inline size_t align_up(size_t v, size_t a) { return (v + a - 1) / a * a; }
 inline int cdiv(long a, long b) { return (int)((a + b - 1) / b); }
 
+__device__ __forceinline__ float bn_bwd_elem(const float x, const float dy, const bool relu, const float sa, const float sb,
+                                             const float a, const float c1, const float c0) {
+#pragma clang fp contract(off)
+  const float g = (!relu || __builtin_fmaf(x, sa, sb) > 0.f) ? dy : 0.f;
+  return __builtin_fmaf(c1, x, a * g) + c0;
+}
+__device__ __forceinline__ float4 bn_bwd_elem4(const float4 x, const float4 dy, const bool relu, const float4 sa, const float4 sb,
+                                               const float4 a, const float4 c1, const float4 c0) {
+  return make_float4(bn_bwd_elem(x.x, dy.x, relu, sa.x, sb.x, a.x, c1.x, c0.x), bn_bwd_elem(x.y, dy.y, relu, sa.y, sb.y, a.y, c1.y, c0.y),
+                     bn_bwd_elem(x.z, dy.z, relu, sa.z, sb.z, a.z, c1.z, c0.z), bn_bwd_elem(x.w, dy.w, relu, sa.w, sb.w, a.w, c1.w, c0.w));
+}
+
 }
 
 #define DSPN_REQUIRE(cond, ...) \
diff --git a/dspnet_amd/csrc/nn.hip b/dspnet_amd/csrc/nn.hip
--- a/dspnet_amd/csrc/nn.hip
+++ b/dspnet_amd/csrc/nn.hip
@@ -578,14 +578,9 @@
                                     long long n4, int C4, int relu, int accumulate, unsigned *__restrict__ absmax,
                                     int fixed_c) {
   float mx = 0.f;
-  auto one = [&](const float4 xv, float4 g, const float4 d, const float4 sa, const float4 sb, const float4 a,
+  auto one = [&](const float4 xv, const float4 g, const float4 d, const float4 sa, const float4 sb, const float4 a,
                  const float4 c1, const float4 c0) __attribute__((always_inline)) {
-    if (relu) {
-      g.x = fmaf(xv.x, sa.x, sb.x) > 0.f ? g.x : 0.f; g.y = fmaf(xv.y, sa.y, sb.y) > 0.f ? g.y : 0.f;
-      g.z = fmaf(xv.z, sa.z, sb.z) > 0.f ? g.z : 0.f; g.w = fmaf(xv.w, sa.w, sb.w) > 0.f ? g.w : 0.f;
-    }
-    float4 o = make_float4(a.x * g.x + c1.x * xv.x + c0.x, a.y * g.y + c1.y * xv.y + c0.y,
-                           a.z * g.z + c1.z * xv.z + c0.z, a.w * g.w + c1.w * xv.w + c0.w);
+    float4 o = dspn::bn_bwd_elem4(xv, g, relu, sa, sb, a, c1, c0);
     if (accumulate) { o.x += d.x; o.y += d.y; o.z += d.z; o.w += d.w; }
     mx = fmaxf(mx, fmaxf(fmaxf(fabsf(o.x), fabsf(o.y)), fmaxf(fabsf(o.z), fabsf(o.w))));
     return o;
diff --git a/dspnet_amd/engine.py b/dspnet_amd/engine.py
--- a/dspnet_amd/engine.py
+++ b/dspnet_amd/engine.py
@@ -369,6 +369,31 @@
             n.x_ext = fn.zeros(2, x.shape[3], device=self.device)
             n.am_dyin = self.new_scalar(backward=True)
 
+    def _plan_bn_recompute(self):
+        if not BN_RECOMPUTE or self.math != "f16x2" or self.device.type != "cuda":
+            return
+        readers = {}
+        for m in self.nodes:
+            for k, v in vars(m).items():
+                if k in ("out", "x_raw"):
+                    continue
+                for t in (v if isinstance(v, (list, tuple)) else [v]):
+                    if isinstance(t, Tensor):
+                        readers.setdefault(id(t), set()).add(id(m))
+        planes_in = {id(n.x) for n in self.nodes if isinstance(n, BatchNorm) and n.dx_planes}
+        for c in self.nodes:
+            bn = getattr(c, "bn_bwd_node", None) if isinstance(c, Conv) else None
+            if bn is None or bn.defer_apply is not True or bn.conv_consumers != [c] or readers.get(id(bn.out), set()) - {id(c)}:
+                continue
+            if (bn.dx_planes or not bn.x.requires_grad or bn.x.dtype != torch.float32 or bn.x.data is None
+                    or c.math != "f16x2" or c.wtp is None or c.stride != 1 or c.tap_expand or c.input_sum_grad is not None
+                    or id(c.out) not in planes_in or c.cout > BN_RECOMPUTE_MAX_K):
+                continue
+            sums, tiles = bn.bwd_sums
+            bn.rc_ws = torch.empty(fn.bn_backward_from_sums_workspace_bytes(tiles, bn.x.shape[3]), dtype=torch.uint8,
+                                   device=self.device)
+            c.bn_recompute = True
+
     def _plan_input_planes(self):
         if self.math != "f16x2" or self.device.type != "cuda":
             return
@@ -396,6 +421,7 @@
         self._plan_gradient_magnitudes()
         if _os.environ.get("DSPN_DY_PLANES", "1") != "0":
             self._plan_gradient_planes()
+        self._plan_bn_recompute()
         self._wt_pairs_nodes = [n for n in self.nodes if isinstance(n, Conv) and (n.wt is not None or n.wh is not None)]
         off = 0
         for p in self.param_order:
@@ -893,6 +919,16 @@
         self._g = g
         self.completes_x_grad = False
         self._pending = None
+        self.rc_ws, self._rc_done = None, False
+
+    def _input_grad_target(self):
+        dx, acc = self.x.grad_target()
+        prod, g, am = getattr(self.x, "producer", None), self._g, None
+        if (isinstance(prod, Conv) and prod.am_dy is not None and g.scalars is not None and dx.dtype == torch.float32
+                and self.completes_x_grad):
+            am = g.scalar(prod.am_dy)
+            g._am_done.add(prod.am_dy)
+        return dx, acc, am
 
     def _moving(self):
         if self.use_global_stats:
@@ -952,6 +988,9 @@
         self._pending = (args, kw)
 
     def backward(self, beside=False):
+        if self._rc_done:
+            self._rc_done = False
+            return
         if self._pending is not None:
             args, kw = self._pending
             self._pending = None
@@ -960,13 +999,9 @@
         if not self.out._gw:
             return
         am = None
+        prod, g = getattr(self.x, "producer", None), self._g
         if self.x.requires_grad:
-            dx, acc = self.x.grad_target()
-            prod, g = getattr(self.x, "producer", None), self._g
-            if (isinstance(prod, Conv) and prod.am_dy is not None and g.scalars is not None and dx.dtype == torch.float32
-                    and self.completes_x_grad):
-                am = g.scalar(prod.am_dy)
-                g._am_done.add(prod.am_dy)
+            dx, acc, am = self._input_grad_target()
         else:
             dx, acc = (self.out.grad if self.pool_grad is None else self.out.own_grad()), False
         if self.pool_grad is not None:
@@ -1008,6 +1043,9 @@
 WGRAD_SIDE_MIN_US = float(_os.environ.get("DSPN_WGRAD_SIDE_MIN_US", "30"))
 
 FINALIZE_BESIDE = _os.environ.get("DSPN_FINALIZE_BESIDE", "1") != "0"
+
+BN_RECOMPUTE = _os.environ.get("DSPN_BN_RECOMPUTE", "1") != "0"
+BN_RECOMPUTE_MAX_K = int(_os.environ.get("DSPN_BN_RECOMPUTE_MAX_K", "128"))
 
 FUSE_CONV_MAGNITUDES = _os.environ.get("DSPN_CONV_MAGNITUDES", "1") != "0"
 
@@ -1071,6 +1109,7 @@
         if self.am_x is not None and self.in_affine is None:
             g.want_magnitude(self.x_raw)
         self.x_planes_bn = None
+        self.bn_recompute = False
         self.guard_fb = False
         self.wp = self.wtp = None
         if g.device.type == "cuda":
@@ -1214,7 +1253,7 @@
             self._g._am_done.add(self.am_dy)
         bn = getattr(self, "bn_bwd_node", None) if self.x.requires_grad else None
         early = (bn is not None and FINALIZE_BESIDE and not self.guard_fb and self._g.device.type == "cuda"
-                 and bn.pool_grad is None)
+                 and bn.pool_grad is None and not self.bn_recompute)
         if (WGRAD_SIDE and self._g.wgrad_side_allowed and self._g.device.type == "cuda" and (bn is not None or self._g.batchnorm_chain()) and self._wgrad_worth_a_stream()
                 and self._g.wgrad_beside(self, dy, planes, xa, dya)):
             early = False
@@ -1276,14 +1315,37 @@
                             dy_absmax=dya, dy_planes=planes, x_planes=xp is not None)
         self.slabs_fresh = self.slabs is not None
 
+    def _bn_recompute(self, bn, dy, planes, dya, wa):
+        if not (self.bn_recompute and planes and not self.guard_fb and bn.pool_grad is None):
+            return False
+        sums, tiles = bn.bwd_sums
+        dact = self.x.own_grad()
+        if not fn.conv2d_dgrad_bn_sums(dy, self.wtp, self.x.shape, self.wt_shape,
+                                       (bn.x.data, bn.scale, bn.shift, bn.mean, bn.rstd, bn.relu, sums), dya, wa, dact,
+                                       pad=self.pad, dil=self.dil):
+            self.bn_recompute = False
+            return False
+        self.x.grad_target()
+        gamma = None if bn.gamma is None else bn.gamma.data
+        fn.bn_backward_from_sums(bn.x.data, bn.scale, bn.shift, dact, bn.mean, bn.rstd, gamma, sums, tiles, relu=bn.relu,
+                                 dx=dact, dgamma=None if bn.gamma is None else bn.gamma.grad, dbeta=bn.beta.grad, phase=1,
+                                 ws=bn.rc_ws)
+        dx, acc, am = bn._input_grad_target()
+        fn.conv2d_dgrad_bn_apply(dy, self.wtp, self.x.shape, self.wt_shape, bn.x.data, bn.scale, bn.shift, bn.relu, bn.rc_ws,
+                                 dya, wa, dx, accumulate=acc, dx_absmax=am, pad=self.pad, dil=self.dil)
+        bn.bwd_sums_ready, bn._rc_done = False, True
+        return True
+
     def _data_gradient(self, dy, planes, dya, wa):
         if self.wtp is not None and self._g.wp_table is None:
             fn.weight_planes(self.w.data, transposed=True, cols=self.wtp.shape[2] * 32, out=self.wtp, math=self.math,
                              w_absmax=wa)
         elif self.wtp is None and not self._g.wt_batched:
             fn.weight_transpose(self.w.data, out=self.wt, copy=self.wh)
+        bn = getattr(self, "bn_bwd_node", None)
+        if bn is not None and self._bn_recompute(bn, dy, planes, dya, wa):
+            return
         dx, acc = self.x.grad_target()
-        bn = getattr(self, "bn_bwd_node", None)
         bn_bwd, bn_dya = None, None
         if bn is not None:
             bn_bwd = (bn.x.data, bn.scale, bn.shift, bn.mean, bn.rstd, bn.relu, bn.bwd_sums[0])
diff --git a/dspnet_amd/functional.py b/dspnet_amd/functional.py
--- a/dspnet_amd/functional.py
+++ b/dspnet_amd/functional.py
@@ -41,6 +41,8 @@
     "dspn_conv2d_dgrad_bn_tiles": (_i, [_i, _i, _i, _i, _i]),
     "dspn_conv2d_dgrad_bn_f32": (_i, [_vp, _vp, _vp, _vp, _i, _i, _i, _i, _i, _i, _i, _i, _i, _i, _i, _i, _i, _i, _i,
                                       _vp, _vp, _vp, _vp, _vp, _i, _vp, _sz, _vp, _i, _vp, _vp, _vp, _sz, _vp]),
+    "dspn_conv2d_dgrad_bn_apply_f32": (_i, [_vp, _vp, _vp, _vp, _i, _i, _i, _i, _i, _i, _i, _i, _i, _i, _i, _i, _i, _i, _i,
+                                            _vp, _vp, _vp, _i, _vp, _vp, _i, _vp, _vp, _vp, _sz, _vp]),
     "dspn_bn_backward_from_sums_f32": (_i, [_vp, _vp, _vp, _vp, _vp, _vp, _vp, _vp, _i, _vp, _vp, _vp, _ll, _i, _i, _i,
                                             _vp, _vp, _vp, _vp, _i, _vp, _sz, _vp]),
     "dspn_absmin_rows_batch_f32": (_i, [_vp, _i, _ll, _vp]),
@@ -465,6 +467,7 @@
 
 MATH_DY_PLANES = 0x200
 MATH_X_PLANES = 0x400
+MATH_NO_STORE = 0x800
 
 
 def conv2d_dgrad(dy, wt, x_shape, stride=1, pad=0, dil=1, out=None, accumulate=False, bn_bwd=None, wt_planes=None,
@@ -501,6 +504,37 @@
     return out
 
 
+def conv2d_dgrad_bn_sums(dy, wt_planes, x_shape, wt_shape, bn_bwd, dy_absmax, w_absmax, dx, pad=0, dil=1):
+    N, H, W, Cx = x_shape
+    Cin, R, S, ldy = wt_shape
+    bx, bsc, bsh, bmu, brs, brelu, bsums = bn_bwd
+    ws = workspace(L().dspn_conv2d_split_workspace_bytes(N * H * W, Cin), dy.device, "split")
+    ph, pw = _hw(pad)
+    rc = L().dspn_conv2d_dgrad_bn_f32(ptr(dy), None, ptr(wt_planes), ptr(dx), N, H, W, Cin, ldy, R, S, 1, ph, pw, dil,
+                                      dy.shape[1], dy.shape[2], dx.shape[3], 0, ptr(bx), ptr(bsc), ptr(bsh), ptr(bmu), ptr(brs),
+                                      int(brelu), ptr(bsums), bsums.numel() * 4, None, 3 | MATH_DY_PLANES | MATH_NO_STORE,
+                                      ptr(dy_absmax), ptr(w_absmax), ptr(ws), ws.numel(), stream())
+    if rc == -1:
+        return False
+    check(rc, "conv2d_dgrad (BatchNorm sums only)")
+    return True
+
+
+def conv2d_dgrad_bn_apply(dy, wt_planes, x_shape, wt_shape, bn_x, scale, shift, relu, coef, dy_absmax, w_absmax, out,
+                          accumulate=False, dx_absmax=None, pad=0, dil=1):
+    N, H, W, Cx = x_shape
+    Cin, R, S, ldy = wt_shape
+    ws = workspace(L().dspn_conv2d_split_workspace_bytes(N * H * W, Cin), dy.device, "split")
+    ph, pw = _hw(pad)
+    assert out.dtype == bn_x.dtype == torch.float32 and out.shape == bn_x.shape
+    check(L().dspn_conv2d_dgrad_bn_apply_f32(ptr(dy), None, ptr(wt_planes), ptr(out), N, H, W, Cin, ldy, R, S, 1, ph, pw, dil,
+                                             dy.shape[1], dy.shape[2], out.shape[3], int(accumulate), ptr(bn_x), ptr(scale),
+                                             ptr(shift), int(relu), ptr(coef), ptr(dx_absmax), 3 | MATH_DY_PLANES,
+                                             ptr(dy_absmax), ptr(w_absmax), ptr(ws), ws.numel(), stream()),
+          "conv2d_dgrad_bn_apply")
+    return out
+
+
 def _wgrad_absmax(x, dy, in_affine, math, x_absmax, dy_absmax):
     if math == 3 and x.dtype == torch.float32:
         return (absmax(x, in_affine) if x_absmax is None else x_absmax, absmax(dy) if dy_absmax is None else dy_absmax)
@@ -677,9 +711,13 @@
     return dx, dgamma, dbeta
 
 
+def bn_backward_from_sums_workspace_bytes(tiles, C):
+    return 12 * C + L().dspn_bn_tiles_workspace_bytes(tiles, C)
+
+
 def bn_backward_from_sums(x, scale, shift, dy, mean, rstd, gamma, sums, tiles, relu=False, dx=None, dgamma=None,
                           dbeta=None, accumulate=False, dx_absmax=None, dy_absmax=None, x_chan_minmax=None, dx_planes=False,
-                          dx_absmin=None, phase=0, park=False):
+                          dx_absmin=None, phase=0, park=False, ws=None):
     assert phase in (0, 1, 2) and (not park or phase == 1)
     C = x.shape[-1]
     rows = _rows(x)
@@ -687,7 +725,9 @@
     dbeta = empty(C, device=x.device) if dbeta is None else dbeta
     if gamma is not None and dgamma is None:
         dgamma = empty(C, device=x.device)
-    ws = workspace(12 * C + L().dspn_bn_tiles_workspace_bytes(tiles, C), x.device, "bn")
+    if ws is None:
+        ws = workspace(bn_backward_from_sums_workspace_bytes(tiles, C), x.device, "bn")
+    assert ws.numel() >= bn_backward_from_sums_workspace_bytes(tiles, C)
     assert dy.dtype == x.dtype == dx.dtype
     check(_f("dspn_bn_backward_from_sums", x)(ptr(x), ptr(scale), ptr(shift), ptr(dy), ptr(mean), ptr(rstd), ptr(gamma),
                                              ptr(sums), tiles, ptr(dx), ptr(dgamma), ptr(dbeta), rows, C, int(relu),
diff --git a/include/dspn_nn.h b/include/dspn_nn.h
--- a/include/dspn_nn.h
+++ b/include/dspn_nn.h
@@ -16,6 +16,7 @@
 #define DSPN_MATH_UNSCALED_OK 0x100
 #define DSPN_MATH_DY_PLANES 0x200
 #define DSPN_MATH_X_PLANES 0x400
+#define DSPN_MATH_NO_STORE 0x800
 
 int dspn_conv2d_forward_f32(const float *x, const float *w, const float *bias, const float *residual, float *y,
                             int N, int H, int W, int Cin, int Cout, int R, int S,
@@ -54,6 +55,11 @@
                              const float *bn_mean, const float *bn_rstd, int bn_relu, float *bn_sums,
                              size_t bn_sums_bytes, float *bn_dy_absmax, int math, const float *dy_absmax, const float *w_absmax,
                              void *workspace, size_t workspace_bytes, void *stream);
+int dspn_conv2d_dgrad_bn_apply_f32(const float *dy, const float *wt, const void *wt_planes, float *dx, int N, int H, int W, int Cin,
+                                   int ldy, int R, int S, int stride, int pad_h, int pad_w, int dil, int Ho, int Wo, int dx_ldc,
+                                   int accumulate, const float *bn_x, const float *bn_scale, const float *bn_shift, int bn_relu,
+                                   const float *coef, float *dx_absmax, int math, const float *dy_absmax, const float *w_absmax,
+                                   void *workspace, size_t workspace_bytes, void *stream);
 
 size_t dspn_conv2d_input_sum_grad_workspace_bytes(int Ho, int Wo, int ldy, int R, int S);
 int dspn_conv2d_input_sum_grad_f32(const float *dy, const float *w, float *out, int N, int H, int W,
```

New measurement: 984.8 images/s (median of 6 runs). 1.1% higher.
